# sinamalakouti/CDDMSL

Measured on AMD Instinct MI355X. Metric: images/sec (train step) VOC+Clipart RN50-C4, higher is better.
Workload: dtype bf16

## Files before the change

cddmsl_amd/csrc/elementwise.hip:

```cpp
#include "common.h"
#include <stdlib.h>

namespace {

template <typename T> struct Elt;
template <> struct Elt<__bf16> {
  static constexpr int ES = 2, VEC = 8;
  __device__ static __forceinline__ void unpack(const u32x4& v, float* f) {
#pragma unroll
    for (int j = 0; j < 4; ++j) { f[2 * j] = bf2f(v[j] & 0xffff); f[2 * j + 1] = bf2f(v[j] >> 16); }
  }
  __device__ static __forceinline__ u32x4 pack(const float* f) {
    u32x4 v;
#pragma unroll
    for (int j = 0; j < 4; ++j) v[j] = pack2bf(f[2 * j], f[2 * j + 1]);
    return v;
  }
  __device__ static __forceinline__ float ld(const char* p) { return bf2f(*(const unsigned short*)p); }
  __device__ static __forceinline__ void st(char* p, float v) { *(unsigned short*)p = f2bf(v); }
};
template <> struct Elt<float> {
  static constexpr int ES = 4, VEC = 4;
  __device__ static __forceinline__ void unpack(const u32x4& v, float* f) {
    const f32x4 x = __builtin_bit_cast(f32x4, v);
// ... 119 lines not shown
template <typename T>
__global__ void k_avgpool2_bwd(const char* dy, const char* mask, const char* add, char* dx, int N, int H, int W, int cch) {
  int Ho = H / 2, Wo = W / 2;
  long total = (long)N * H * W * cch;
  for (long i = (long)blockIdx.x * blockDim.x + threadIdx.x; i < total; i += (long)gridDim.x * blockDim.x) {
    int c = i % cch; long q = i / cch;
    int xx = q % W; q /= W;
    int yy = q % H; int n = q / H;
    float g[8], m[8], a[8], o[8];
    bool in = (yy >> 1) < Ho && (xx >> 1) < Wo;
    if (in) Elt<T>::unpack(((const u32x4*)dy)[(((long)n * Ho + (yy >> 1)) * Wo + (xx >> 1)) * cch + c], g);
    if (mask) Elt<T>::unpack(((const u32x4*)mask)[i], m);
    if (add) Elt<T>::unpack(((const u32x4*)add)[i], a);
#pragma unroll
    for (int j = 0; j < Elt<T>::VEC; ++j) {
      float v = in ? g[j] * 0.25f : 0.f;
      if (add) v += a[j];
      if (mask && !(m[j] > 0.f)) v = 0.f;
      o[j] = v;
    }
    ((u32x4*)dx)[i] = Elt<T>::pack(o);
  }
}

__global__ __launch_bounds__(256) void k_avgpool2_bwd_q8(const char* dy, const char* mask, const char* add, char* dx, int N, int H, int W, int cch,
                                                         char* y8, const float* q8, unsigned* amax8) {
  using T = __bf16;
  const int Ho = H / 2, Wo = W / 2;
  const long total = (long)N * H * W * cch;
  const float s = q8[0];
  unsigned mx = 0u;
  for (long i = (long)blockIdx.x * blockDim.x + threadIdx.x; i < total; i += (long)gridDim.x * blockDim.x) {
    int c = i % cch; long q = i / cch;
    int xx = q % W; q /= W;
    int yy = q % H; int n = q / H;
    float g[8], m[8], a[8], o[8];
    bool in = (yy >> 1) < Ho && (xx >> 1) < Wo;
    if (in) Elt<T>::unpack(((const u32x4*)dy)[(((long)n * Ho + (yy >> 1)) * Wo + (xx >> 1)) * cch + c], g);
    if (mask) Elt<T>::unpack(((const u32x4*)mask)[i], m);
    if (add) Elt<T>::unpack(((const u32x4*)add)[i], a);
#pragma unroll
    for (int j = 0; j < 8; ++j) {
      float v = in ? g[j] * 0.25f : 0.f;
      if (add) v += a[j];
      if (mask && !(m[j] > 0.f)) v = 0.f;
      o[j] = v;
      mx = absmax_bits(mx, v);
    }
    ((u32x4*)dx)[i] = Elt<T>::pack(o);
    const u32x2 o8 = {e4m3x4(o[0] * s, o[1] * s, o[2] * s, o[3] * s), e4m3x4(o[4] * s, o[5] * s, o[6] * s, o[7] * s)};
    ((u32x2*)y8)[i] = o8;
  }
  __shared__ unsigned sm[4];
  mx = wave_max_u(mx);
  if ((threadIdx.x & 63) == 0) sm[threadIdx.x >> 6] = mx;
  __syncthreads();
  if (threadIdx.x == 0) {
    const unsigned a = sm[0] > sm[1] ? sm[0] : sm[1], b = sm[2] > sm[3] ? sm[2] : sm[3];
    atomicMax(amax8 + (blockIdx.x & 63), a > b ? a : b);
  }
}

template <typename T>
__global__ void k_maxpool3s2(const char* x, char* y, int N, int H, int W, int Ho, int Wo, int cch) {
  long total = (long)N * Ho * Wo * cch;
  for (long i = (long)blockIdx.x * blockDim.x + threadIdx.x; i < total; i += (long)gridDim.x * blockDim.x) {
    int c = i % cch; long q = i / cch;
    int ox = q % Wo; q /= Wo;
    int oy = q % Ho; int n = q / Ho;
    float m[8], v[8];
#pragma unroll
    for (int j = 0; j < 8; ++j) m[j] = -INFINITY;
    for (int dy = 0; dy < 3; ++dy) {
      int iy = 2 * oy - 1 + dy;
      if (iy < 0 || iy >= H) continue;
      for (int dx = 0; dx < 3; ++dx) {
        int ix = 2 * ox - 1 + dx;
        if (ix < 0 || ix >= W) continue;
        Elt<T>::unpack(((const u32x4*)x)[(((long)n * H + iy) * W + ix) * cch + c], v);
#pragma unroll
        for (int j = 0; j < Elt<T>::VEC; ++j) m[j] = fmaxf(m[j], v[j]);
      }
    }
    ((u32x4*)y)[i] = Elt<T>::pack(m);
  }
}
template <typename T>
__global__ void k_upsample_zero2(const char* t, const char* mask, const char* add, char* dx, int N, int H, int W, int Ho, int Wo, int cch) {
  long total = (long)N * H * W * cch;
  for (long i = (long)blockIdx.x * blockDim.x + threadIdx.x; i < total; i += (long)gridDim.x * blockDim.x) {
    int c = i % cch; long q = i / cch;
    int xx = q % W; q /= W;
    int yy = q % H; int n = q / H;
    float g[8], m[8], a[8], o[8];
    bool in = !(yy & 1) && !(xx & 1) && (yy >> 1) < Ho && (xx >> 1) < Wo;
    if (in) Elt<T>::unpack(((const u32x4*)t)[(((long)n * Ho + (yy >> 1)) * Wo + (xx >> 1)) * cch + c], g);
    if (mask) Elt<T>::unpack(((const u32x4*)mask)[i], m);
    if (add) Elt<T>::unpack(((const u32x4*)add)[i], a);
#pragma unroll
    for (int j = 0; j < Elt<T>::VEC; ++j) {
      float v = in ? g[j] : 0.f;
      if (add) v += a[j];
      if (mask && !(m[j] > 0.f)) v = 0.f;
      o[j] = v;
    }
    ((u32x4*)dx)[i] = Elt<T>::pack(o);
  }
}
template <typename T>
__global__ void k_meanpool_fwd(const char* x, float* y, long K, int P, int C) {
  long i = (long)blockIdx.x * blockDim.x + threadIdx.x;
  if (i >= K * C) return;
  long k = i / C; int c = i % C;
  float s = 0.f;
  for (int p = 0; p < P; ++p) s += Elt<T>::ld(x + ((k * P + p) * C + c) * Elt<T>::ES);
  y[i] = s / (float)P;
}
template <typename T>
__global__ void k_meanpool_bwd(const float* dy, char* dx, long K, int P, int C) {
  long i = (long)blockIdx.x * blockDim.x + threadIdx.x;
  if (i >= K * P * C) return;
  int c = i % C; long k = i / ((long)P * C);
  Elt<T>::st(dx + i * Elt<T>::ES, dy[k * C + c] / (float)P);
}

template <typename T>
__global__ void k_attn_tokens_fwd(const char* x, const float* pos, char* tok, unsigned long long* mbits, int K, int P, int TP, int cch) {
  long total = (long)K * cch;
  for (long i = (long)blockIdx.x * blockDim.x + threadIdx.x; i < total; i += (long)gridDim.x * blockDim.x) {
    int c = i % cch; long k = i / cch;
    float s[8] = {0, 0, 0, 0, 0, 0, 0, 0}, v[8], o[8];
    unsigned long long mb[8] = {0, 0, 0, 0, 0, 0, 0, 0};
    const int VEC = Elt<T>::VEC;
    for (int p = 0; p < P; ++p) {
      Elt<T>::unpack(((const u32x4*)x)[(k * P + p) * cch + c], v);
      const float* pe = pos + (long)(p + 1) * cch * VEC + c * VEC;
#pragma unroll
      for (int j = 0; j < VEC; ++j) { s[j] += v[j]; o[j] = v[j] + pe[j]; mb[j] |= (unsigned long long)(v[j] > 0.f) << p; }
      ((u32x4*)tok)[(k * TP + p + 1) * cch + c] = Elt<T>::pack(o);
    }
    if (mbits) {
#pragma unroll
      for (int j = 0; j < VEC; ++j) mbits[(k * cch + c) * VEC + j] = mb[j];
    }
    const float* pe = pos + c * VEC;
#pragma unroll
    for (int j = 0; j < VEC; ++j) o[j] = s[j] / (float)P + pe[j];
    ((u32x4*)tok)[(k * TP) * cch + c] = Elt<T>::pack(o);
    const u32x4 z = {0u, 0u, 0u, 0u};
    for (int p = P + 1; p < TP; ++p) ((u32x4*)tok)[(k * TP + p) * cch + c] = z;
  }
}
template <typename T>
__global__ __launch_bounds__(256) void k_attn_tokens_bwd(const char* __restrict__ dtok, const char* __restrict__ relu_mask, char* __restrict__ dx, float* __restrict__ gpos, int K,
                                                         int P, int TP, int cch, int slab) {
  constexpr int V = Elt<T>::VEC;
  const int c = blockIdx.x * 256 + threadIdx.x;
  const int t = blockIdx.y;
  if (c >= cch || (t == 0 && !gpos)) return;
  const int k0 = blockIdx.z * slab, k1 = min(K, k0 + slab);
  float acc[V];
#pragma unroll
  for (int j = 0; j < V; ++j) acc[j] = 0.f;
  const u32x4* src = (const u32x4*)dtok;
#pragma unroll 4
  for (int k = k0; k < k1; ++k) {
    float a[8];
    Elt<T>::unpack(src[((long)k * TP + t) * cch + c], a);
#pragma unroll
    for (int j = 0; j < V; ++j) acc[j] += a[j];
    if (t > 0 && dx) {
      float b[8], m[8], o[8];
      const long oi = ((long)k * P + t - 1) * cch + c;
      Elt<T>::unpack(src[(long)k * TP * cch + c], b);
      if (relu_mask) Elt<T>::unpack(((const u32x4*)relu_mask)[oi], m);
#pragma unroll
      for (int j = 0; j < V; ++j) {
        o[j] = a[j] + b[j] / (float)P;
        if (relu_mask && !(m[j] > 0.f)) o[j] = 0.f;
      }
      ((u32x4*)dx)[oi] = Elt<T>::pack(o);
    }
  }
  if (gpos) {
#pragma unroll
    for (int j = 0; j < V; ++j) atomicAdd(gpos + (long)t * cch * V + (long)c * V + j, acc[j]);
  }
}

template <typename T>
__global__ void k_attnpool_softmax_fwd(const float* S, float* p, char* pT, long rows, int H, int P1, int TP, float scale) {
  const long r = (long)blockIdx.x * blockDim.x + threadIdx.x;
  if (r >= rows) return;
  const long k = r / H; const int h = (int)(r - k * H);
  const float* s = S + r * TP;
  float mx = -INFINITY;
  for (int t = 0; t < P1; ++t) mx = fmaxf(mx, s[t] * scale);
  float sum = 0.f;
  for (int t = 0; t < P1; ++t) sum += expf(s[t] * scale - mx);
  const float inv = 1.f / sum;
  for (int t = 0; t < TP; ++t) {
    float v = 0.f;
    if (t < P1) { v = expf(s[t] * scale - mx) * inv; p[r * P1 + t] = v; }
    Elt<T>::st(pT + ((k * TP + t) * H + h) * Elt<T>::ES, v);
  }
}
template <typename T>
__global__ void k_attnpool_softmax_bwd(const float* p, const float* dP, char* dsT, char* pds, long rows, int H, int P1, int TP,
                                       float scale) {
  const long r = (long)blockIdx.x * blockDim.x + threadIdx.x;
  if (r >= rows) return;
  const long k = r / H; const int h = (int)(r - k * H);
  const float* pr = p + r * P1;
  const float* dp = dP + r * TP;
  float dot = 0.f;
  for (int t = 0; t < P1; ++t) dot += pr[t] * dp[t];
  char* prow = pds + ((k * 2 * H + h) * TP) * Elt<T>::ES;
  char* drow = pds + ((k * 2 * H + H + h) * TP) * Elt<T>::ES;
  for (int t = 0; t < TP; ++t) {
    float pv = 0.f, ds = 0.f;
    if (t < P1) { pv = pr[t]; ds = pv * (dp[t] - dot) * scale; }
    Elt<T>::st(dsT + ((k * TP + t) * H + h) * Elt<T>::ES, ds);
    Elt<T>::st(prow + t * Elt<T>::ES, pv);
    Elt<T>::st(drow + t * Elt<T>::ES, ds);
  }
}

template <typename T>
__global__ __launch_bounds__(256) void k_attnpool_softmax_fwd_w(const float* __restrict__ S, float* __restrict__ p, char* __restrict__ pT,
                                                                long K, int H, int P1, int TP, float scale) {
  const long k = (long)blockIdx.x * 4 + (threadIdx.x >> 6);
  const int t = threadIdx.x & 63;
  if (k >= K) return;
  float v[32];
#pragma unroll
  for (int h = 0; h < 32; ++h) {
    v[h] = 0.f;
    if (h < H) {
      const bool in = t < P1;
      const float x = in ? S[(k * H + h) * TP + t] * scale : -INFINITY;
      const float mx = wave_max(x);
      const float e = in ? expf(x - mx) : 0.f;
      const float sum = wave_sum(e);
      v[h] = e * (1.f / sum);
      if (in) p[(k * H + h) * P1 + t] = v[h];
    }
  }
  if (t < TP) {
    char* dst = pT + ((k * TP + t) * H) * Elt<T>::ES;
    if (H % Elt<T>::VEC == 0) {
#pragma unroll
      for (int g = 0; g < 32 / Elt<T>::VEC; ++g)
        if (g * Elt<T>::VEC < H) ((u32x4*)dst)[g] = Elt<T>::pack(v + g * Elt<T>::VEC);
    } else {
#pragma unroll
      for (int h = 0; h < 32; ++h)
        if (h < H) Elt<T>::st(dst + h * Elt<T>::ES, v[h]);
    }
  }
}
template <typename T>
__global__ __launch_bounds__(256) void k_attnpool_softmax_bwd_w(const float* __restrict__ p, const float* __restrict__ dP,
                                                                char* __restrict__ dsT, char* __restrict__ pds, long K, int H, int P1,
                                                                int TP, float scale) {
  const long k = (long)blockIdx.x * 4 + (threadIdx.x >> 6);
  const int t = threadIdx.x & 63;
  if (k >= K) return;
  float dsv[32];
#pragma unroll
  for (int h = 0; h < 32; ++h) {
    dsv[h] = 0.f;
    if (h < H) {
      const bool in = t < P1;
      const float pv = in ? p[(k * H + h) * P1 + t] : 0.f;
      const float dp = in ? dP[(k * H + h) * TP + t] : 0.f;
      const float dot = wave_sum(pv * dp);
      dsv[h] = in ? pv * (dp - dot) * scale : 0.f;
      if (t < TP) {
        Elt<T>::st(pds + ((k * 2 * H + h) * TP + t) * Elt<T>::ES, pv);
        Elt<T>::st(pds + ((k * 2 * H + H + h) * TP + t) * Elt<T>::ES, dsv[h]);
      }
    }
  }
  if (t < TP) {
    char* dst = dsT + ((k * TP + t) * H) * Elt<T>::ES;
    if (H % Elt<T>::VEC == 0) {
#pragma unroll
      for (int g = 0; g < 32 / Elt<T>::VEC; ++g)
        if (g * Elt<T>::VEC < H) ((u32x4*)dst)[g] = Elt<T>::pack(dsv + g * Elt<T>::VEC);
    } else {
#pragma unroll
      for (int h = 0; h < 32; ++h)
        if (h < H) Elt<T>::st(dst + h * Elt<T>::ES, dsv[h]);
    }
  }
}

template <typename T>
__global__ void k_relu_bwd(const char* g, const char* y, char* dx, long nchunks, int g_f32) {
  for (long i = (long)blockIdx.x * blockDim.x + threadIdx.x; i < nchunks; i += (long)gridDim.x * blockDim.x) {
    float a[8], m[8], o[8];
    Elt<T>::unpack(((const u32x4*)y)[i], m);
    if (g_f32 && Elt<T>::VEC == 8) {
      Elt<float>::unpack(((const u32x4*)g)[2 * i], a);
      Elt<float>::unpack(((const u32x4*)g)[2 * i + 1], a + 4);
    } else Elt<T>::unpack(((const u32x4*)g)[i], a);
// ... 114 lines not shown
  return (unsigned)(g < 1 ? 1 : (g > cap ? cap : g));
}

}

#define DISPATCH(dtype, KERNEL, ...)                                   \
  do {                                                                 \
    if ((dtype) == 0) { KERNEL<__bf16> __VA_ARGS__; }                  \
    else if ((dtype) == 1) { KERNEL<float> __VA_ARGS__; }              \
    else return CDDMSL_ERR_ARG;                                        \
  } while (0)

extern "C" int cddmsl_preprocess(const unsigned char* img, void* out, int n, int h, int w, int Hp, int Wp, int Cp,
                                 const float* mean3, const float* std3, int div255, int dtype, void* stream) {
  if (h <= 0 || w <= 0 || h > Hp || w > Wp || Cp < 3) return CDDMSL_ERR_ARG;
  hipStream_t st = (hipStream_t)stream;
  long px = (long)Hp * Wp;
  DISPATCH(dtype, k_preprocess, <<<dim3((unsigned)((px + 255) / 256)), dim3(256), 0, st>>>(
      img, (char*)out, n, h, w, Hp, Wp, Cp, mean3[0], mean3[1], mean3[2], std3[0], std3[1], std3[2], div255 ? 255.0f : 1.0f));
  return launch_status();
}

extern "C" int cddmsl_preprocess224(const unsigned char* img, void* out, int n, int h, int w, int Hp, int Wp, int RH,
                                    int RW, int top, int left, int S, int Cp, const float* mean3, const float* std3,
                                    int dtype, void* stream) {
  if (h <= 0 || w <= 0 || h > Hp || w > Wp || Cp < 3 || S <= 0 || top < 0 || left < 0 || top + S > RH || left + S > RW)
    return CDDMSL_ERR_ARG;
  hipStream_t st = (hipStream_t)stream;
  DISPATCH(dtype, k_preprocess224, <<<dim3((unsigned)((S * S + 255) / 256)), dim3(256), 0, st>>>(
      img, (char*)out, n, h, w, Hp, Wp, RH, RW, top, left, S, Cp, mean3[0], mean3[1], mean3[2], std3[0], std3[1], std3[2]));
  return launch_status();
}

extern "C" int cddmsl_preprocess_batch(const unsigned char* const* imgs, const int* hs, const int* ws, int N, void* out, int Hp, int Wp,
                                       int Cp, const float* mean3, const float* std3, int div255, int dtype, void* stream) {
  if (N < 0 || Cp < 3 || !imgs || !hs || !ws) return CDDMSL_ERR_ARG;
  for (int j = 0; j < N; ++j) if (hs[j] <= 0 || ws[j] <= 0 || hs[j] > Hp || ws[j] > Wp || !imgs[j]) return CDDMSL_ERR_ARG;
  hipStream_t st = (hipStream_t)stream;
  const long px = (long)Hp * Wp;
  for (int n0 = 0; n0 < N; n0 += PRE_MAX) {
    const int c = N - n0 < PRE_MAX ? N - n0 : PRE_MAX;
    PreBatch b;
    for (int j = 0; j < PRE_MAX; ++j) { const int q = j < c ? j : 0; b.img[j] = imgs[n0 + q]; b.h[j] = hs[n0 + q]; b.w[j] = ws[n0 + q]; }
    DISPATCH(dtype, k_preprocess_batch, <<<dim3((unsigned)((px + 255) / 256), (unsigned)c), dim3(256), 0, st>>>(
        b, (char*)out, n0, Hp, Wp, Cp, mean3[0], mean3[1], mean3[2], std3[0], std3[1], std3[2], div255 ? 255.0f : 1.0f));
  }
  return launch_status();
}
extern "C" int cddmsl_preprocess224_batch(const unsigned char* const* imgs, const int* hs, const int* ws, int N, void* out, int Hp, int Wp,
                                          int RH, int RW, int top, int left, int S, int Cp, const float* mean3, const float* std3,
                                          int dtype, void* stream) {
  if (N < 0 || Cp < 3 || !imgs || !hs || !ws || S <= 0 || top < 0 || left < 0 || top + S > RH || left + S > RW) return CDDMSL_ERR_ARG;
  for (int j = 0; j < N; ++j) if (hs[j] <= 0 || ws[j] <= 0 || hs[j] > Hp || ws[j] > Wp || !imgs[j]) return CDDMSL_ERR_ARG;
  hipStream_t st = (hipStream_t)stream;
  for (int n0 = 0; n0 < N; n0 += PRE_MAX) {
    const int c = N - n0 < PRE_MAX ? N - n0 : PRE_MAX;
    PreBatch b;
    for (int j = 0; j < PRE_MAX; ++j) { const int q = j < c ? j : 0; b.img[j] = imgs[n0 + q]; b.h[j] = hs[n0 + q]; b.w[j] = ws[n0 + q]; }
    DISPATCH(dtype, k_preprocess224_batch, <<<dim3((unsigned)((S * S + 255) / 256), (unsigned)c), dim3(256), 0, st>>>(
        b, (char*)out, n0, Hp, Wp, RH, RW, top, left, S, Cp, mean3[0], mean3[1], mean3[2], std3[0], std3[1], std3[2]));
  }
  return launch_status();
}

extern "C" int cddmsl_avgpool2_fwd(const void* x, void* y, int N, int H, int W, int C, int dtype, void* stream) {
  int es = dtype == 0 ? 2 : 4;
  if ((C * es) % 16 || H < 2 || W < 2) return CDDMSL_ERR_ARG;
  int cch = C * es / 16;
  long total = (long)N * (H / 2) * (W / 2) * cch;
  if (total == 0) return CDDMSL_OK;
  DISPATCH(dtype, k_avgpool2_fwd, <<<dim3(gsz(total)), dim3(256), 0, (hipStream_t)stream>>>((const char*)x, (char*)y, N, H, W, cch));
  return launch_status();
}

extern "C" int cddmsl_avgpool2_bwd(const void* dy, const void* mask, const void* add, void* dx, int N, int H, int W,
                                   int C, int dtype, void* stream) {
  int es = dtype == 0 ? 2 : 4;
  if ((C * es) % 16 || H < 2 || W < 2) return CDDMSL_ERR_ARG;
  int cch = C * es / 16;
  long total = (long)N * H * W * cch;
  if (total == 0) return CDDMSL_OK;
  DISPATCH(dtype, k_avgpool2_bwd, <<<dim3(gsz(total)), dim3(256), 0, (hipStream_t)stream>>>(
      (const char*)dy, (const char*)mask, (const char*)add, (char*)dx, N, H, W, cch));
  return launch_status();
}

extern "C" int cddmsl_avgpool2_bwd_q8(const void* dy, const void* mask, const void* add, void* dx, int N, int H, int W, int C, void* y8,
                                      const float* q8, float* amax8, void* stream) {
  if ((C * 2) % 16 || !y8 || !q8 || !amax8) return CDDMSL_ERR_ARG;
  const int cch = C * 2 / 16;
  const long total = (long)N * H * W * cch;
  if (total == 0) return CDDMSL_OK;
  hipLaunchKernelGGL(k_avgpool2_bwd_q8, dim3(gsz(total, 256, 8192)), dim3(256), 0, (hipStream_t)stream, (const char*)dy, (const char*)mask, (const char*)add,
                     (char*)dx, N, H, W, cch, (char*)y8, q8, (unsigned*)amax8);
  return launch_status();
}

extern "C" int cddmsl_maxpool3s2_fwd(const void* x, void* y, int N, int H, int W, int C, int dtype, void* stream) {
  int es = dtype == 0 ? 2 : 4;
  if ((C * es) % 16 || H < 1 || W < 1) return CDDMSL_ERR_ARG;
  int cch = C * es / 16, Ho = (H - 1) / 2 + 1, Wo = (W - 1) / 2 + 1;
  long total = (long)N * Ho * Wo * cch;
  if (total == 0) return CDDMSL_OK;
  DISPATCH(dtype, k_maxpool3s2, <<<dim3(gsz(total)), dim3(256), 0, (hipStream_t)stream>>>((const char*)x, (char*)y, N, H, W, Ho, Wo, cch));
  return launch_status();
}
extern "C" int cddmsl_upsample_zero2(const void* t, const void* mask, const void* add, void* dx, int N, int H, int W, int C,
                                     int dtype, void* stream) {
  int es = dtype == 0 ? 2 : 4;
  if ((C * es) % 16 || H < 1 || W < 1) return CDDMSL_ERR_ARG;
  int cch = C * es / 16, Ho = (H - 1) / 2 + 1, Wo = (W - 1) / 2 + 1;
  long total = (long)N * H * W * cch;
  if (total == 0) return CDDMSL_OK;
  DISPATCH(dtype, k_upsample_zero2, <<<dim3(gsz(total)), dim3(256), 0, (hipStream_t)stream>>>(
      (const char*)t, (const char*)mask, (const char*)add, (char*)dx, N, H, W, Ho, Wo, cch));
  return launch_status();
}
extern "C" int cddmsl_meanpool_fwd(const void* x, float* y, long K, int P, int C, int dtype, void* stream) {
  if (K < 0 || P <= 0 || C <= 0) return CDDMSL_ERR_ARG;
  if (K == 0) return CDDMSL_OK;
  long n = K * C;
  DISPATCH(dtype, k_meanpool_fwd, <<<dim3((unsigned)((n + 255) / 256)), dim3(256), 0, (hipStream_t)stream>>>((const char*)x, y, K, P, C));
  return launch_status();
}
extern "C" int cddmsl_meanpool_bwd(const float* dy, void* dx, long K, int P, int C, int dtype, void* stream) {
  if (K < 0 || P <= 0 || C <= 0) return CDDMSL_ERR_ARG;
  if (K == 0) return CDDMSL_OK;
  long n = K * P * C;
  DISPATCH(dtype, k_meanpool_bwd, <<<dim3((unsigned)((n + 255) / 256)), dim3(256), 0, (hipStream_t)stream>>>(dy, (char*)dx, K, P, C));
  return launch_status();
}

extern "C" int cddmsl_attn_tokens_fwd(const void* x, const float* pos, void* tok, int K, int P, int TP, int C, int dtype, void* stream) {
  int es = dtype == 0 ? 2 : 4;
  if ((C * es) % 16 || P <= 0 || TP < P + 1) return CDDMSL_ERR_ARG;
  int cch = C * es / 16;
  long total = (long)K * cch;
  if (total == 0) return CDDMSL_OK;
  DISPATCH(dtype, k_attn_tokens_fwd, <<<dim3(gsz(total, 64)), dim3(64), 0, (hipStream_t)stream>>>((const char*)x, pos, (char*)tok, nullptr, K, P, TP, cch));
  return launch_status();
}

extern "C" int cddmsl_attn_tokens_fwd_mask(const void* x, const float* pos, void* tok, unsigned long long* mbits, int K, int P, int TP, int C,
                                           int dtype, void* stream) {
  int es = dtype == 0 ? 2 : 4;
  if ((C * es) % 16 || P <= 0 || P > 64 || TP < P + 1 || K < 0 || !mbits) return CDDMSL_ERR_ARG;
  int cch = C * es / 16;
  long total = (long)K * cch;
  if (total == 0) return CDDMSL_OK;
  DISPATCH(dtype, k_attn_tokens_fwd, <<<dim3(gsz(total, 64)), dim3(64), 0, (hipStream_t)stream>>>((const char*)x, pos, (char*)tok, mbits, K, P, TP, cch));
  return launch_status();
}

extern "C" int cddmsl_attn_tokens_bwd(const void* dtok, const void* relu_mask, void* dx, float* gpos, int K, int P, int TP, int C,
                                      int dtype, void* stream) {
  int es = dtype == 0 ? 2 : 4;
  if ((C * es) % 16 || P <= 0 || TP < P + 1 || K < 0 || (!dx && !gpos)) return CDDMSL_ERR_ARG;
  int cch = C * es / 16;
  if (K == 0) return CDDMSL_OK;
  int slab = 128;
  while ((K + slab - 1) / slab > 65535) slab *= 2;
  dim3 grid((unsigned)((cch + 255) / 256), (unsigned)(P + 1), (unsigned)((K + slab - 1) / slab));
  DISPATCH(dtype, k_attn_tokens_bwd, <<<grid, dim3(256), 0, (hipStream_t)stream>>>((const char*)dtok, (const char*)relu_mask, (char*)dx, gpos, K, P, TP, cch, slab));
  return launch_status();
}

extern "C" int cddmsl_attnpool_softmax_fwd(const float* S, float* p, void* pT, long K, int H, int P1, int TP, float scale, int dtype,
                                           void* stream) {
  if (K < 0 || H <= 0 || P1 <= 0 || TP < P1) return CDDMSL_ERR_ARG;
  const long rows = K * H;
  if (rows == 0) return CDDMSL_OK;
  if (H <= 32 && TP <= 64) {
    DISPATCH(dtype, k_attnpool_softmax_fwd_w, <<<dim3((unsigned)((K + 3) / 4)), dim3(256), 0, (hipStream_t)stream>>>(S, p, (char*)pT, K, H, P1, TP, scale));
    return launch_status();
  }
  DISPATCH(dtype, k_attnpool_softmax_fwd, <<<dim3((unsigned)((rows + 255) / 256)), dim3(256), 0, (hipStream_t)stream>>>(S, p, (char*)pT, rows, H, P1, TP, scale));
  return launch_status();
}
extern "C" int cddmsl_attnpool_softmax_bwd(const float* p, const float* dP, void* dsT, void* pds, long K, int H, int P1, int TP,
                                           float scale, int dtype, void* stream) {
  if (K < 0 || H <= 0 || P1 <= 0 || TP < P1) return CDDMSL_ERR_ARG;
  const long rows = K * H;
  if (rows == 0) return CDDMSL_OK;
  if (H <= 32 && TP <= 64) {
    DISPATCH(dtype, k_attnpool_softmax_bwd_w, <<<dim3((unsigned)((K + 3) / 4)), dim3(256), 0, (hipStream_t)stream>>>(p, dP, (char*)dsT, (char*)pds, K, H, P1, TP, scale));
    return launch_status();
  }
  DISPATCH(dtype, k_attnpool_softmax_bwd, <<<dim3((unsigned)((rows + 255) / 256)), dim3(256), 0, (hipStream_t)stream>>>(p, dP, (char*)dsT, (char*)pds, rows, H, P1, TP, scale));
  return launch_status();
}

extern "C" int cddmsl_relu_bwd(const void* g, const void* y, void* dx, long numel, int g_f32, int dtype, void* stream) {
  int vec = dtype == 0 ? 8 : 4;
  if (numel < 0 || numel % vec) return CDDMSL_ERR_ARG;
  if (numel == 0) return CDDMSL_OK;
  long nch = numel / vec;
  DISPATCH(dtype, k_relu_bwd, <<<dim3(gsz(nch)), dim3(256), 0, (hipStream_t)stream>>>((const char*)g, (const char*)y, (char*)dx, nch, g_f32));
  return launch_status();
}

extern "C" int cddmsl_colsum(const void* x, float* out, long rows, int cols, int period, int dtype, void* stream) {
  if (rows < 0 || cols <= 0 || period <= 0) return CDDMSL_ERR_ARG;
  if (rows == 0) return CDDMSL_OK;
  if (period > 65535) return CDDMSL_ERR_ARG;
  long nj = (rows + period - 1) / period;
  int slab = 256;
  while ((nj + slab - 1) / slab > 2048) slab *= 2;
  const int vec = dtype == 0 ? 8 : 4;
  if (cols % vec == 0) {
    dim3 gridv((unsigned)((cols / vec + 63) / 64), (unsigned)((nj + slab - 1) / slab), (unsigned)period);
    DISPATCH(dtype, k_colsum_vec, <<<gridv, dim3(256), 0, (hipStream_t)stream>>>((const char*)x, out, rows, cols, period, slab));
    return launch_status();
  }
  dim3 grid((unsigned)((cols + 63) / 64), (unsigned)((nj + slab - 1) / slab), (unsigned)period);
  DISPATCH(dtype, k_colsum, <<<grid, dim3(256), 0, (hipStream_t)stream>>>((const char*)x, out, rows, cols, period, slab));
  return launch_status();
}

extern "C" int cddmsl_sgd_clip_step(float** params, const float** grads, float** moms, const long* sizes, int count,
                                    float* norm_ws, float lr, float momentum, float wd, float clip, int first_step,
                                    void* stream) {
  hipStream_t st = (hipStream_t)stream;
  if (count < 0) return CDDMSL_ERR_ARG;
  for (int base = 0; base < count; base += SGD_MAX) {
    SgdBatch b;
    b.count = count - base < SGD_MAX ? count - base : SGD_MAX;
    long mx = 0;
    for (int i = 0; i < b.count; ++i) {
      b.it[i].p = params[base + i]; b.it[i].g = grads[base + i]; b.it[i].m = moms[base + i]; b.it[i].n = sizes[base + i];
      if (sizes[base + i] > mx) mx = sizes[base + i];
    }
    if (hipMemsetAsync(norm_ws + base, 0, sizeof(float) * b.count, st) != hipSuccess) return CDDMSL_ERR_LAUNCH;
    unsigned gx = gsz(mx, 256 * 8, 256);
    k_sqnorm<<<dim3(gx, b.count), dim3(256), 0, st>>>(b, norm_ws + base);
    k_sgd<<<dim3(gx, b.count), dim3(256), 0, st>>>(b, norm_ws + base, lr, momentum, wd, clip, first_step);
  }
  return launch_status();
}

extern "C" int cddmsl_abi_version() { return 3; }
```

cddmsl_amd/csrc/gemm_conv.hip:

```cpp
#include "common.h"
#include <cstdlib>
#include <type_traits>

namespace {

constexpr int BM = 128, BN = 128, KCH = 8;

struct FastDiv {
  unsigned mul, shr, d;
};
static inline FastDiv make_fastdiv(unsigned d) {
  FastDiv f;
  f.d = d;
  unsigned s = 0;
  while ((1ull << s) < d) ++s;
  f.shr = s;
  f.mul = (unsigned)(((1ull << 32) * ((1ull << s) - d)) / d + 1);
  return f;
}
__device__ __forceinline__ unsigned fdiv(unsigned n, const FastDiv& f) { return (__umulhi(n, f.mul) + n) >> f.shr; }

template <typename T> __device__ __forceinline__ float affine(float v, float sc, float bi) {
  return sizeof(T) <= 2 ? __builtin_fmaf(v, sc, bi) : v * sc + bi;
}

__device__ __forceinline__ unsigned pack4_e4m3(float a, float b, float c, float d) {
  a = __builtin_amdgcn_fmed3f(a, -448.f, 448.f); b = __builtin_amdgcn_fmed3f(b, -448.f, 448.f);
  c = __builtin_amdgcn_fmed3f(c, -448.f, 448.f); d = __builtin_amdgcn_fmed3f(d, -448.f, 448.f);
  int w = __builtin_amdgcn_cvt_pk_fp8_f32(a, b, 0, false);
  w = __builtin_amdgcn_cvt_pk_fp8_f32(c, d, w, true);
  return (unsigned)w;
}

#ifndef CDDMSL_STORE_AUX
#define CDDMSL_STORE_AUX 2
#endif
#ifndef CDDMSL_LOAD_AUX
#define CDDMSL_LOAD_AUX 0
#endif

struct ConvArgs {
  const char* x;
  const char* w;
  char* y;
  const float* scale;
  const float* bias;
  const char* residual;
  const char* relu_mask;
  int Nimg, Hi, Wi, Cin, Ho, Wo, Cout, KH, KW, stride, pad;
  int ldy, ldr, ldm;
  int relu, out_f32, pool;
  int res_f32;
  int res_pool;
  int M, Kc, cpp;
  FastDiv dWo, dHo, dcpp, dKW;
  int xrs, wrs;
  long bx, bw, by;
  char* y8 = nullptr;
  const float* q8 = nullptr;
  unsigned* amax8 = nullptr;
  float* partial = nullptr;
  int tile0 = 0, ksplits = 1, kper = 0, tile_limit = 0;
  int nt_out = 1;
#ifdef CDDMSL_STAMPS
  unsigned long long* stamps;
#endif
#ifdef CDDMSL_TILE_STAMPS
  unsigned long long* tstamps = nullptr;
#endif
};

template <typename T> struct Mma;
template <> struct Mma<__bf16> {
  static constexpr int ES = 2;
  __device__ static __forceinline__ void step(f32x16& acc, const u32x4& a, const u32x4& b) {
    acc = __builtin_amdgcn_mfma_f32_32x32x16_bf16(__builtin_bit_cast(bf16x8, a), __builtin_bit_cast(bf16x8, b), acc, 0, 0, 0);
  }
  __device__ static __forceinline__ float load(const char* p) { return bf2f(*(const unsigned short*)p); }
  __device__ static __forceinline__ void store(char* p, float v) { *(unsigned short*)p = f2bf(v); }
};
template <> struct Mma<float> {
  static constexpr int ES = 4;
  __device__ static __forceinline__ void step(f32x16& acc, const u32x4& a, const u32x4& b) {
    const f32x4 fa = __builtin_bit_cast(f32x4, a), fb = __builtin_bit_cast(f32x4, b);
    acc = __builtin_amdgcn_mfma_f32_32x32x2f32(fa[0], fb[0], acc, 0, 0, 0);
    acc = __builtin_amdgcn_mfma_f32_32x32x2f32(fa[1], fb[1], acc, 0, 0, 0);
    acc = __builtin_amdgcn_mfma_f32_32x32x2f32(fa[2], fb[2], acc, 0, 0, 0);
    acc = __builtin_amdgcn_mfma_f32_32x32x2f32(fa[3], fb[3], acc, 0, 0, 0);
  }
  __device__ static __forceinline__ float load(const char* p) { return *(const float*)p; }
  __device__ static __forceinline__ void store(char* p, float v) { *(float*)p = v; }
};

struct fp8e4 { unsigned char v; };
typedef __attribute__((ext_vector_type(8))) int i32x8;
template <> struct Mma<fp8e4> {
  static constexpr int ES = 2;
  __device__ static __forceinline__ void step2(f32x16& acc, const u32x4& a0, const u32x4& a1, const u32x4& b0, const u32x4& b1) {
    const i32x8 a = {(int)a0[0], (int)a0[1], (int)a0[2], (int)a0[3], (int)a1[0], (int)a1[1], (int)a1[2], (int)a1[3]};
    const i32x8 b = {(int)b0[0], (int)b0[1], (int)b0[2], (int)b0[3], (int)b1[0], (int)b1[1], (int)b1[2], (int)b1[3]};
    acc = __builtin_amdgcn_mfma_scale_f32_32x32x64_f8f6f4(a, b, acc, 0, 0, 0, 0x7f7f7f7f, 0, 0x7f7f7f7f);
  }
};
template <typename T> struct MmaQuad {
  __device__ static __forceinline__ void run(f32x16& c0, f32x16& c1, const u32x4 (*fa)[4], const u32x4* fb) {
#pragma unroll
    for (int ks = 0; ks < 4; ++ks) {
      Mma<T>::step(c0, fa[0][ks], fb[ks]);
      Mma<T>::step(c1, fa[1][ks], fb[ks]);
    }
  }
};
template <> struct MmaQuad<fp8e4> {
  __device__ static __forceinline__ void run(f32x16& c0, f32x16& c1, const u32x4 (*fa)[4], const u32x4* fb) {
#pragma unroll
    for (int s = 0; s < 2; ++s) {
      Mma<fp8e4>::step2(c0, fa[0][2 * s], fa[0][2 * s + 1], fb[2 * s], fb[2 * s + 1]);
      Mma<fp8e4>::step2(c1, fa[1][2 * s], fa[1][2 * s + 1], fb[2 * s], fb[2 * s + 1]);
    }
  }
};

template <typename T> __device__ __forceinline__ void load8(const char* p, float* f);
template <> __device__ __forceinline__ void load8<__bf16>(const char* p, float* f) {
  const u32x4 v = *(const u32x4*)p;
#pragma unroll
  for (int j = 0; j < 4; ++j) { f[2 * j] = bf2f(v[j] & 0xffff); f[2 * j + 1] = bf2f(v[j] >> 16); }
}
template <> __device__ __forceinline__ void load8<float>(const char* p, float* f) {
  const f32x4 a = ((const f32x4*)p)[0], b = ((const f32x4*)p)[1];
  f[0] = a[0]; f[1] = a[1]; f[2] = a[2]; f[3] = a[3]; f[4] = b[0]; f[5] = b[1]; f[6] = b[2]; f[7] = b[3];
}

__device__ __forceinline__ int xcd_remap(int bid, int nblk) {
  const int q = nblk >> 3, rem = nblk & 7, x = bid & 7, j = bid >> 3;
  return (x < rem ? x * (q + 1) : rem * (q + 1) + (x - rem) * q) + j;
}

__device__ __forceinline__ int swz(int row, int chunk) { return row * KCH + (chunk ^ ((row >> 1) & 7)); }

template <typename T> __device__ __forceinline__ u32x4 avg4(const u32x4& a, const u32x4& b, const u32x4& c, const u32x4& d);
template <> __device__ __forceinline__ u32x4 avg4<float>(const u32x4& a, const u32x4& b, const u32x4& c, const u32x4& d) {
  const f32x4 fa = __builtin_bit_cast(f32x4, a), fb = __builtin_bit_cast(f32x4, b);
  const f32x4 fc = __builtin_bit_cast(f32x4, c), fd = __builtin_bit_cast(f32x4, d);
  f32x4 r = ((fa + fb) + (fc + fd)) * 0.25f;
  return __builtin_bit_cast(u32x4, r);
}
template <> __device__ __forceinline__ u32x4 avg4<__bf16>(const u32x4& a, const u32x4& b, const u32x4& c, const u32x4& d) {
  u32x4 r;
#pragma unroll
  for (int j = 0; j < 4; ++j) {
    float lo = (bf2f(a[j] & 0xffff) + bf2f(b[j] & 0xffff)) + (bf2f(c[j] & 0xffff) + bf2f(d[j] & 0xffff));
    float hi = (bf2f(a[j] >> 16) + bf2f(b[j] >> 16)) + (bf2f(c[j] >> 16) + bf2f(d[j] >> 16));
    r[j] = pack2bf(lo * 0.25f, hi * 0.25f);
  }
  return r;
}

template <typename T>
__global__ __launch_bounds__(256, 2) void k_conv_fwd_reg(ConvArgs p) {
  __shared__ __attribute__((aligned(16))) u32x4 lds[2][BM * KCH];
  const int t = threadIdx.x;
  const int ntn = (p.Cout + BN - 1) / BN;
  const int tile_n = blockIdx.x % ntn, tile_m = blockIdx.x / ntn;
  const int m0 = tile_m * BM, n0 = tile_n * BN;
  const int cc = t & 7, rb = t >> 3;

  long pix[4];
  int iy0[4], ix0[4];
  bool vm[4];
#pragma unroll
  for (int i = 0; i < 4; ++i) {
    int m = m0 + rb + 32 * i;
    vm[i] = m < p.M;
    int mm = vm[i] ? m : 0;
    int ox = mm % p.Wo, tq = mm / p.Wo;
    int oy = tq % p.Ho, img = tq / p.Ho;
    int s = p.pool ? 2 * p.stride : p.stride;
    iy0[i] = oy * s - p.pad;
    ix0[i] = ox * s - p.pad;
    pix[i] = ((long)img * p.Hi + iy0[i]) * p.Wi + ix0[i];
  }
  const int nkt = (p.Kc + KCH - 1) / KCH;
  u32x4 ra[4], rbv[4];
  const u32x4 zero = {0u, 0u, 0u, 0u};

  auto gload = [&](int kt) {
    int kc = kt * KCH + cc;
    bool vk = kc < p.Kc;
    int pp = vk ? kc / p.cpp : 0;
    int coff = vk ? kc - pp * p.cpp : 0;
    int ky = pp / p.KW, kx = pp - ky * p.KW;
#pragma unroll
    for (int i = 0; i < 4; ++i) {
      int iy = iy0[i] + ky, ix = ix0[i] + kx;
      if (!p.pool) {
        bool ok = vk && vm[i] && iy >= 0 && iy < p.Hi && ix >= 0 && ix < p.Wi;
        const u32x4* src = (const u32x4*)(p.x + ((pix[i] + (long)ky * p.Wi + kx) * p.cpp + coff) * 16);
        ra[i] = ok ? *src : zero;
      } else {
        bool ok = vk && vm[i];
        if (ok) {
          const char* b0 = p.x + (pix[i] * p.cpp + coff) * 16;
          long rs = (long)p.Wi * p.cpp * 16, cs = (long)p.cpp * 16;
          ra[i] = avg4<T>(*(const u32x4*)b0, *(const u32x4*)(b0 + cs), *(const u32x4*)(b0 + rs), *(const u32x4*)(b0 + rs + cs));
        } else ra[i] = zero;
      }
      int n = n0 + rb + 32 * i;
      bool okb = vk && n < p.Cout;
      rbv[i] = okb ? *(const u32x4*)(p.w + ((long)n * p.Kc + kc) * 16) : zero;
    }
  };

  f32x16 acc[2][2];
#pragma unroll
  for (int a = 0; a < 2; ++a)
#pragma unroll
    for (int b = 0; b < 2; ++b)
#pragma unroll
      for (int r = 0; r < 16; ++r) acc[a][b][r] = 0.f;

  const int lane = t & 63, wv = t >> 6;
  const int wm = wv >> 1, wn = wv & 1;
  const int r = lane & 31, h = lane >> 5;

  gload(0);
  for (int kt = 0; kt < nkt; ++kt) {
#pragma unroll
    for (int i = 0; i < 4; ++i) {
      int row = rb + 32 * i;
      lds[0][swz(row, cc)] = ra[i];
      lds[1][swz(row, cc)] = rbv[i];
    }
    __syncthreads();
    if (kt + 1 < nkt) gload(kt + 1);
#pragma unroll
    for (int ks = 0; ks < KCH / 2; ++ks) {
      u32x4 fa[2], fb[2];
#pragma unroll
      for (int i = 0; i < 2; ++i) {
        fa[i] = lds[0][swz(wm * 64 + i * 32 + r, 2 * ks + h)];
        fb[i] = lds[1][swz(wn * 64 + i * 32 + r, 2 * ks + h)];
      }
#pragma unroll
      for (int a = 0; a < 2; ++a)
#pragma unroll
        for (int b = 0; b < 2; ++b) Mma<T>::step(acc[a][b], fa[a], fb[b]);
    }
    __syncthreads();
  }

  const bool vec_ok = (p.Cout % 8 == 0) && (p.ldy % 8 == 0) && (!p.residual || p.ldr % 8 == 0) && (!p.relu_mask || p.ldm % 8 == 0);
  if (vec_ok) {
    float* ep = (float*)&lds[0][0] + wv * 2048;
    const int cg = lane & 7, rr = lane >> 3;
    const int n = n0 + wn * 64 + cg * 8;
    float sc[8], bi[8];
#pragma unroll
    for (int j = 0; j < 8; ++j) {
      sc[j] = (p.scale && n + j < p.Cout) ? p.scale[n + j] : 1.f;
      bi[j] = (p.bias && n + j < p.Cout) ? p.bias[n + j] : 0.f;
    }
#pragma unroll
    for (int a = 0; a < 2; ++a) {
      __syncthreads();
#pragma unroll
      for (int b = 0; b < 2; ++b)
#pragma unroll
        for (int g = 0; g < 16; ++g) {
          int row = (g & 3) + 8 * (g >> 2) + 4 * h, col = b * 32 + r;
          ep[row * 64 + ((((col >> 3) ^ (row & 7)) << 3) | (col & 7))] = acc[a][b][g];
        }
      __syncthreads();
      if (n < p.Cout) {
#pragma unroll
        for (int i = 0; i < 4; ++i) {
          int row = rr + 8 * i;
          int m = m0 + wm * 64 + a * 32 + row;
          if (m >= p.M) continue;
          const f32x4* src = (const f32x4*)(ep + row * 64 + ((cg ^ (row & 7)) << 3));
          f32x4 v0 = src[0], v1 = src[1];
          float v[8] = {v0[0], v0[1], v0[2], v0[3], v1[0], v1[1], v1[2], v1[3]};
#pragma unroll
          for (int j = 0; j < 8; ++j) v[j] = affine<T>(v[j], sc[j], bi[j]);
          if (p.residual) {
            float rv[8];
            load8<T>(p.residual + ((long)m * p.ldr + n) * Mma<T>::ES, rv);
#pragma unroll
            for (int j = 0; j < 8; ++j) v[j] += rv[j];
          }
          if (p.relu) {
#pragma unroll
            for (int j = 0; j < 8; ++j) v[j] = fmaxf(v[j], 0.f);
          }
          if (p.relu_mask) {
            float mv[8];
            load8<T>(p.relu_mask + ((long)m * p.ldm + n) * Mma<T>::ES, mv);
#pragma unroll
            for (int j = 0; j < 8; ++j) if (!(mv[j] > 0.f)) v[j] = 0.f;
          }
          if (p.out_f32 || Mma<T>::ES == 4) {
            f32x4* dst = (f32x4*)(p.y + ((long)m * p.ldy + n) * 4);
            f32x4 o0 = {v[0], v[1], v[2], v[3]}, o1 = {v[4], v[5], v[6], v[7]};
            dst[0] = o0; dst[1] = o1;
          } else {
            u32x4 o = {pack2bf(v[0], v[1]), pack2bf(v[2], v[3]), pack2bf(v[4], v[5]), pack2bf(v[6], v[7])};
            *(u32x4*)(p.y + ((long)m * p.ldy + n) * 2) = o;
          }
        }
      }
    }
    return;
  }
#pragma unroll
  for (int b = 0; b < 2; ++b) {
    int n = n0 + wn * 64 + b * 32 + r;
    if (n >= p.Cout) continue;
    float sc = p.scale ? p.scale[n] : 1.f;
    float bi = p.bias ? p.bias[n] : 0.f;
#pragma unroll
    for (int a = 0; a < 2; ++a) {
#pragma unroll
      for (int g = 0; g < 16; ++g) {
        int m = m0 + wm * 64 + a * 32 + (g & 3) + 8 * (g >> 2) + 4 * h;
        if (m >= p.M) continue;
        float v = affine<T>(acc[a][b][g], sc, bi);
        if (p.residual) v += Mma<T>::load(p.residual + ((long)m * p.ldr + n) * Mma<T>::ES);
        if (p.relu) v = fmaxf(v, 0.f);
        if (p.relu_mask && !(Mma<T>::load(p.relu_mask + ((long)m * p.ldm + n) * Mma<T>::ES) > 0.f)) v = 0.f;
        if (p.out_f32) *(float*)(p.y + ((long)m * p.ldy + n) * 4) = v;
        else Mma<T>::store(p.y + ((long)m * p.ldy + n) * Mma<T>::ES, v);
      }
    }
  }
}

__device__ __attribute__((aligned(16))) unsigned int g_zero_page[4] = {0u, 0u, 0u, 0u};

__device__ __forceinline__ void glds16(const void* g, void* l) {
  __builtin_amdgcn_global_load_lds((const __attribute__((address_space(1))) void*)g,
                                   (__attribute__((address_space(3))) void*)l, 16, 0, 0);
}

__device__ __forceinline__ long pooled_row(const ConvArgs& p, int m) {
  const unsigned tq = fdiv((unsigned)m, p.dWo), ox = m - tq * p.Wo;
  const unsigned img = fdiv(tq, p.dHo), oy = tq - img * p.Ho;
  const unsigned hp = p.Ho >> 1, wp = p.Wo >> 1;
  return ((oy >> 1) < hp && (ox >> 1) < wp) ? ((long)img * hp + (oy >> 1)) * wp + (ox >> 1) : -1L;
}

template <typename T>
__global__ __launch_bounds__(256, 2) void k_conv_fwd(ConvArgs p) {
  __shared__ __attribute__((aligned(16))) u32x4 lds[2][2][BM * KCH];
  const int t = threadIdx.x;
  p.x += (long)blockIdx.y * p.bx; p.w += (long)blockIdx.y * p.bw; p.y += (long)blockIdx.y * p.by;
  const int wvu = __builtin_amdgcn_readfirstlane(t >> 6);
  const int ntn = (p.Cout + BN - 1) / BN;
  const int lbid = xcd_remap(blockIdx.x, gridDim.x);
  const int tile_n = lbid % ntn, tile_m = lbid / ntn;
  const int m0 = tile_m * BM, n0 = tile_n * BN;
  const int cc = t & 7, rb = t >> 3;
  const int cl = cc ^ ((rb >> 1) & 7);

  long rowoff[4], wrow[4];
  int iy0[4], ix0[4];
  bool vm[4], vn[4];
#pragma unroll
  for (int i = 0; i < 4; ++i) {
    int m = m0 + rb + 32 * i;
    vm[i] = m < p.M;
    unsigned mm = vm[i] ? m : 0;
    unsigned tq = fdiv(mm, p.dWo), ox = mm - tq * p.Wo;
    unsigned img = fdiv(tq, p.dHo), oy = tq - img * p.Ho;
    iy0[i] = (int)oy * p.stride - p.pad;
    ix0[i] = (int)ox * p.stride - p.pad;
    rowoff[i] = ((((long)img * p.Hi + iy0[i]) * p.Wi + ix0[i]) * p.xrs) * 16;
    int n = n0 + rb + 32 * i;
    vn[i] = n < p.Cout;
    wrow[i] = (long)(vn[i] ? n : 0) * p.wrs * 16;
  }
  const int nkt = (p.Kc + KCH - 1) / KCH;
  const char* zp = (const char*)g_zero_page;
  const bool taps = !(p.KH == 1 && p.KW == 1 && p.pad == 0);
  int kc = cl;
  int pp0 = (int)fdiv((unsigned)kc, p.dcpp);
  int coff = kc - pp0 * p.cpp;
  int ky = (int)fdiv((unsigned)pp0, p.dKW), kx = pp0 - ky * p.KW;

  const bool fast = (p.cpp & 7) == 0;
  const char* pa[4];
  const char* pb[4];
  int inca[4], incb[4];
  int tiles_left_in_tap = 0;
  auto retap = [&]() {
    const int delta = ((ky * p.Wi + kx) * p.xrs + coff) * 16;
#pragma unroll
    for (int i = 0; i < 4; ++i) {
      bool ok = vm[i];
      if (taps) {
        int iy = iy0[i] + ky, ix = ix0[i] + kx;
        ok = ok && iy >= 0 && iy < p.Hi && ix >= 0 && ix < p.Wi;
      }
      pa[i] = ok ? p.x + rowoff[i] + delta : zp;
      inca[i] = ok ? KCH * 16 : 0;
    }
  };
  if (fast) {
#pragma unroll
    for (int i = 0; i < 4; ++i) {
      pb[i] = vn[i] ? p.w + wrow[i] + (long)kc * 16 : zp;
      incb[i] = vn[i] ? KCH * 16 : 0;
    }
    retap();
    tiles_left_in_tap = p.cpp >> 3;
  }

  auto stage = [&](int buf) {
    if (fast) {
#pragma unroll
      for (int i = 0; i < 4; ++i) glds16(pa[i], &lds[buf][0][(8 * wvu + 32 * i) * KCH]);
#pragma unroll
      for (int i = 0; i < 4; ++i) glds16(pb[i], &lds[buf][1][(8 * wvu + 32 * i) * KCH]);
#pragma unroll
      for (int i = 0; i < 4; ++i) pb[i] += incb[i];
      if (--tiles_left_in_tap == 0) {
        tiles_left_in_tap = p.cpp >> 3;
        coff = cl;
        if (++kx == p.KW) { kx = 0; ++ky; }
        retap();
      } else {
#pragma unroll
        for (int i = 0; i < 4; ++i) pa[i] += inca[i];
      }
      return;
    }
    const bool vk = kc < p.Kc;
    const int delta = ((ky * p.Wi + kx) * p.xrs + coff) * 16;
#pragma unroll
    for (int i = 0; i < 4; ++i) {
      bool ok = vk && vm[i];
      if (taps) {
        int iy = iy0[i] + ky, ix = ix0[i] + kx;
        ok = ok && iy >= 0 && iy < p.Hi && ix >= 0 && ix < p.Wi;
      }
      const char* src = ok ? p.x + rowoff[i] + delta : zp;
      glds16(src, &lds[buf][0][(8 * wvu + 32 * i) * KCH]);
    }
#pragma unroll
    for (int i = 0; i < 4; ++i) {
      const char* src = (vk && vn[i]) ? p.w + wrow[i] + (long)kc * 16 : zp;
      glds16(src, &lds[buf][1][(8 * wvu + 32 * i) * KCH]);
    }
    kc += KCH;
    coff += KCH;
    while (coff >= p.cpp) {
      coff -= p.cpp;
      if (++kx == p.KW) { kx = 0; ++ky; }
    }
  };

  f32x16 acc[2][2];
#pragma unroll
  for (int a = 0; a < 2; ++a)
#pragma unroll
    for (int b = 0; b < 2; ++b)
#pragma unroll
      for (int r = 0; r < 16; ++r) acc[a][b][r] = 0.f;

  const int lane = t & 63, wv = t >> 6;
  const int wm = wv >> 1, wn = wv & 1;
  const int r = lane & 31, h = lane >> 5;

  const bool vec_ok = (p.Cout % 8 == 0) && (p.ldy % 8 == 0) && (!p.residual || p.ldr % 8 == 0) && (!p.relu_mask || p.ldm % 8 == 0);
  constexpr bool PRE = Mma<T>::ES == 2;
  u32x4 rres[2][4], rmsk[2][4];
  const bool rf32 = PRE && p.res_f32;
  if (PRE && vec_ok && ((p.residual && !rf32) || p.relu_mask)) {
    const int n = n0 + wn * 64 + (lane & 7) * 8;
#pragma unroll
    for (int a = 0; a < 2; ++a)
#pragma unroll
      for (int i = 0; i < 4; ++i) {
        int m = m0 + wm * 64 + a * 32 + (lane >> 3) + 8 * i;
        bool ok = m < p.M && n < p.Cout;
        const u32x4 z = {0u, 0u, 0u, 0u};
        if (p.res_pool) {
          const long po = pooled_row(p, m);
          rres[a][i] = (ok && po >= 0) ? *(const u32x4*)(p.residual + (po * p.ldr + n) * 2) : z;
        } else
        rres[a][i] = (ok && p.residual && !rf32) ? *(const u32x4*)(p.residual + ((long)m * p.ldr + n) * 2) : z;
        rmsk[a][i] = (ok && p.relu_mask) ? *(const u32x4*)(p.relu_mask + ((long)m * p.ldm + n) * 2) : z;
      }
  }

  stage(0);
  for (int kt = 0; kt < nkt; ++kt) {
    const int cur = kt & 1;
    if (kt + 1 < nkt) {
      stage(cur ^ 1);
      asm volatile("s_waitcnt vmcnt(8)" ::: "memory");
    } else {
      asm volatile("s_waitcnt vmcnt(0)" ::: "memory");
    }
    __builtin_amdgcn_s_barrier();
    u32x4 fa[2][2], fb[2][2];
#pragma unroll
    for (int i = 0; i < 2; ++i) {
      fa[0][i] = lds[cur][0][swz(wm * 64 + i * 32 + r, h)];
      fb[0][i] = lds[cur][1][swz(wn * 64 + i * 32 + r, h)];
    }
#pragma unroll
    for (int ks = 0; ks < KCH / 2; ++ks) {
      if (ks + 1 < KCH / 2) {
#pragma unroll
        for (int i = 0; i < 2; ++i) {
          fa[(ks + 1) & 1][i] = lds[cur][0][swz(wm * 64 + i * 32 + r, 2 * (ks + 1) + h)];
          fb[(ks + 1) & 1][i] = lds[cur][1][swz(wn * 64 + i * 32 + r, 2 * (ks + 1) + h)];
        }
      }
#pragma unroll
      for (int a = 0; a < 2; ++a)
#pragma unroll
        for (int b = 0; b < 2; ++b) Mma<T>::step(acc[a][b], fa[ks & 1][a], fb[ks & 1][b]);
    }
    asm volatile("s_waitcnt lgkmcnt(0)" ::: "memory");
    __builtin_amdgcn_s_barrier();
  }

  if (vec_ok) {
    float* ep = (float*)&lds[0][0][0] + wv * 2048;
    const int cg = lane & 7, rr = lane >> 3;
    const int n = n0 + wn * 64 + cg * 8;
    float sc[8], bi[8];
#pragma unroll
    for (int j = 0; j < 8; ++j) {
      sc[j] = (p.scale && n + j < p.Cout) ? p.scale[n + j] : 1.f;
      bi[j] = (p.bias && n + j < p.Cout) ? p.bias[n + j] : 0.f;
    }
#pragma unroll
    for (int a = 0; a < 2; ++a) {
      __syncthreads();
#pragma unroll
      for (int b = 0; b < 2; ++b)
#pragma unroll
        for (int g = 0; g < 16; ++g) {
          int row = (g & 3) + 8 * (g >> 2) + 4 * h, col = b * 32 + r;
          ep[row * 64 + ((((col >> 3) ^ (row & 7)) << 3) | (col & 7))] = acc[a][b][g];
        }
      __syncthreads();
      if (n < p.Cout) {
#pragma unroll
        for (int i = 0; i < 4; ++i) {
          int row = rr + 8 * i;
          int m = m0 + wm * 64 + a * 32 + row;
          if (m >= p.M) continue;
          const f32x4* src = (const f32x4*)(ep + row * 64 + ((cg ^ (row & 7)) << 3));
          f32x4 v0 = src[0], v1 = src[1];
          float v[8] = {v0[0], v0[1], v0[2], v0[3], v1[0], v1[1], v1[2], v1[3]};
#pragma unroll
          for (int j = 0; j < 8; ++j) v[j] = affine<T>(v[j], sc[j], bi[j]);
          if (p.residual) {
            float rv[8];
            if (rf32) load8<float>(p.residual + ((long)m * p.ldr + n) * 4, rv);
            else if (PRE) {
#pragma unroll
              for (int j = 0; j < 4; ++j) { rv[2 * j] = bf2f(rres[a][i][j] & 0xffff); rv[2 * j + 1] = bf2f(rres[a][i][j] >> 16); }
            } else if (p.res_pool) {
              const long po = pooled_row(p, m);
#pragma unroll
              for (int j = 0; j < 8; ++j) rv[j] = 0.f;
              if (po >= 0) load8<T>(p.residual + (po * p.ldr + n) * Mma<T>::ES, rv);
            } else load8<T>(p.residual + ((long)m * p.ldr + n) * Mma<T>::ES, rv);
            if (p.res_pool) {
#pragma unroll
              for (int j = 0; j < 8; ++j) rv[j] *= 0.25f;
            }
#pragma unroll
            for (int j = 0; j < 8; ++j) v[j] += rv[j];
          }
          if (p.relu) {
#pragma unroll
            for (int j = 0; j < 8; ++j) v[j] = fmaxf(v[j], 0.f);
          }
          if (p.relu_mask) {
            float mv[8];
            if (PRE) {
#pragma unroll
              for (int j = 0; j < 4; ++j) { mv[2 * j] = bf2f(rmsk[a][i][j] & 0xffff); mv[2 * j + 1] = bf2f(rmsk[a][i][j] >> 16); }
            } else load8<T>(p.relu_mask + ((long)m * p.ldm + n) * Mma<T>::ES, mv);
#pragma unroll
            for (int j = 0; j < 8; ++j) if (!(mv[j] > 0.f)) v[j] = 0.f;
          }
          if (p.out_f32 || Mma<T>::ES == 4) {
            f32x4* dst = (f32x4*)(p.y + ((long)m * p.ldy + n) * 4);
            f32x4 o0 = {v[0], v[1], v[2], v[3]}, o1 = {v[4], v[5], v[6], v[7]};
            dst[0] = o0; dst[1] = o1;
          } else {
            u32x4 o = {pack2bf(v[0], v[1]), pack2bf(v[2], v[3]), pack2bf(v[4], v[5]), pack2bf(v[6], v[7])};
            *(u32x4*)(p.y + ((long)m * p.ldy + n) * 2) = o;
          }
        }
      }
    }
    return;
  }
#pragma unroll
  for (int b = 0; b < 2; ++b) {
    int n = n0 + wn * 64 + b * 32 + r;
    if (n >= p.Cout) continue;
    float sc = p.scale ? p.scale[n] : 1.f;
    float bi = p.bias ? p.bias[n] : 0.f;
#pragma unroll
    for (int a = 0; a < 2; ++a) {
#pragma unroll
      for (int g = 0; g < 16; ++g) {
        int m = m0 + wm * 64 + a * 32 + (g & 3) + 8 * (g >> 2) + 4 * h;
        if (m >= p.M) continue;
        float v = affine<T>(acc[a][b][g], sc, bi);
        if (p.residual) v += Mma<T>::load(p.residual + ((long)m * p.ldr + n) * Mma<T>::ES);
        if (p.relu) v = fmaxf(v, 0.f);
        if (p.relu_mask && !(Mma<T>::load(p.relu_mask + ((long)m * p.ldm + n) * Mma<T>::ES) > 0.f)) v = 0.f;
        if (p.out_f32) *(float*)(p.y + ((long)m * p.ldy + n) * 4) = v;
        else Mma<T>::store(p.y + ((long)m * p.ldy + n) * Mma<T>::ES, v);
      }
    }
  }
}

struct WgradArgs {
  const char* x;
  const char* dy;
  float* dw;
  const float* scale;
  int Nimg, Hi, Wi, Cin, Ho, Wo, Cout, KH, KW, stride, pad, ldd, pool;
  int M, Kc, cpp, K, ncc;
  int mtiles_per_split;
  FastDiv dWo, dHo;
  int xrs;
  int ldo;
  int direct;
  long bx, bd, bo;
  const float* g0 = nullptr;
  const unsigned long long* mbits = nullptr;
  float* gpos = nullptr;
  float* ws = nullptr;
#ifdef CDDMSL_TILE_STAMPS
  unsigned long long* tstamps = nullptr;
#endif
};

constexpr int WM = 64;
constexpr int WROW = 16 + 4;

template <typename T> struct TrFrag;
template <> struct TrFrag<__bf16> {
  __device__ static __forceinline__ u32x4 read(const u32x4* base, int mrow0, int col0, int lane) {
    int g = lane >> 4, li = lane & 15, q = li >> 2, pp = li & 3;
    int hh = g >> 1;
    int col = col0 + 16 * (g & 1) + 4 * pp;
    const char* b = (const char*)base;
    const char* a0 = b + (long)(mrow0 + 8 * hh + q) * (WROW * 16) + col * 2;
    const char* a1 = a0 + 4 * (WROW * 16);
    i16x4 v0 = __builtin_amdgcn_ds_read_tr16_b64_v4i16((__attribute__((address_space(3))) i16x4*)a0);
    i16x4 v1 = __builtin_amdgcn_ds_read_tr16_b64_v4i16((__attribute__((address_space(3))) i16x4*)a1);
    u32x2 p0 = __builtin_bit_cast(u32x2, v0), p1 = __builtin_bit_cast(u32x2, v1);
    u32x4 r = {p0[0], p0[1], p1[0], p1[1]};
    return r;
  }
  static constexpr int MSTEP = 16;
};
template <> struct TrFrag<float> {
  __device__ static __forceinline__ u32x4 read(const u32x4* base, int mrow0, int col0, int lane) {
    int r = lane & 31, hh = lane >> 5;
    const char* b = (const char*)base;
    u32x4 v;
#pragma unroll
    for (int j = 0; j < 4; ++j) v[j] = *(const unsigned int*)(b + (long)(mrow0 + 4 * hh + j) * (WROW * 16) + (col0 + r) * 4);
    return v;
  }
  static constexpr int MSTEP = 8;
};

template <typename T>
__global__ __launch_bounds__(256, 2) void k_conv_wgrad(WgradArgs p) {
  constexpr int ES = Mma<T>::ES;
  constexpr int TC = 128 * ES / 16;
  constexpr int COLS = 256 / ES;
  __shared__ __attribute__((aligned(16))) u32x4 lds[2][WM * WROW];
  const int t = threadIdx.x, lane = t & 63, wv = t >> 6;
  const int ntn = (p.Cout + COLS - 1) / COLS, ntk = (p.K + COLS - 1) / COLS;
  int bid = xcd_remap(blockIdx.x, gridDim.x);
  const int tile_k = bid % ntk; bid /= ntk;
  const int tile_n = bid % ntn; bid /= ntn;
  const int split = bid;
  const int n0 = tile_n * COLS, k0 = tile_k * COLS;
  const int mt0 = split * p.mtiles_per_split;
  const int total_mt = (p.M + WM - 1) / WM;
  const int mt1 = min(mt0 + p.mtiles_per_split, total_mt);
  (void)TC;

  const int cc = t & 15, rb = t >> 4;
  const int kc = k0 * ES / 16 + cc;
  const bool vk = kc < p.Kc;
  const int pp = vk ? kc / p.cpp : 0, coff = vk ? kc - pp * p.cpp : 0;
  const int ky = pp / p.KW, kx = pp - ky * p.KW;
  const int nc = n0 * ES / 16 + cc;
  const bool vn = nc < p.ncc;
  const u32x4 zero = {0u, 0u, 0u, 0u};
  u32x4 rx[4], rd[4];

  auto gload = [&](int mt) {
#pragma unroll
    for (int i = 0; i < 4; ++i) {
      int m = mt * WM + rb + 16 * i;
      bool vmm = m < p.M;
      unsigned mm = vmm ? m : 0;
      unsigned tq = fdiv(mm, p.dWo);
      int ox = (int)(mm - tq * p.Wo);
      unsigned img = fdiv(tq, p.dHo);
      int oy = (int)(tq - img * p.Ho);
      if (!p.pool) {
        int iy = oy * p.stride - p.pad + ky, ix = ox * p.stride - p.pad + kx;
        bool ok = vmm && vk && iy >= 0 && iy < p.Hi && ix >= 0 && ix < p.Wi;
        rx[i] = ok ? *(const u32x4*)(p.x + ((((long)img * p.Hi + iy) * p.Wi + ix) * p.cpp + coff) * 16) : zero;
      } else {
        if (vmm && vk) {
          const char* b0 = p.x + ((((long)img * p.Hi + 2 * oy) * p.Wi + 2 * ox) * p.cpp + coff) * 16;
          long rs = (long)p.Wi * p.cpp * 16, cs = (long)p.cpp * 16;
          rx[i] = avg4<T>(*(const u32x4*)b0, *(const u32x4*)(b0 + cs), *(const u32x4*)(b0 + rs), *(const u32x4*)(b0 + rs + cs));
        } else rx[i] = zero;
      }
      rd[i] = (vmm && vn) ? *(const u32x4*)(p.dy + ((long)m * p.ldd) * ES + (long)nc * 16) : zero;
    }
  };

  constexpr int WT = COLS / 2;
  constexpr int NT = WT / 32;
  const int wn = wv >> 1, wk = wv & 1;
  f32x16 acc[NT][NT];
#pragma unroll
  for (int a = 0; a < NT; ++a)
#pragma unroll
    for (int b = 0; b < NT; ++b)
#pragma unroll
      for (int r = 0; r < 16; ++r) acc[a][b][r] = 0.f;

  if (mt0 < mt1) gload(mt0);
  for (int mt = mt0; mt < mt1; ++mt) {
#pragma unroll
    for (int i = 0; i < 4; ++i) {
      int row = rb + 16 * i;
      lds[0][row * WROW + cc] = rd[i];
      lds[1][row * WROW + cc] = rx[i];
    }
    __syncthreads();
    if (mt + 1 < mt1) gload(mt + 1);
#pragma unroll
    for (int ms = 0; ms < WM; ms += TrFrag<T>::MSTEP) {
      u32x4 fa[NT], fb[NT];
#pragma unroll
      for (int i = 0; i < NT; ++i) {
        fa[i] = TrFrag<T>::read(lds[0], ms, wn * WT + i * 32, lane);
        fb[i] = TrFrag<T>::read(lds[1], ms, wk * WT + i * 32, lane);
      }
#pragma unroll
      for (int a = 0; a < NT; ++a)
#pragma unroll
        for (int b = 0; b < NT; ++b) Mma<T>::step(acc[a][b], fa[a], fb[b]);
    }
    __syncthreads();
  }

  const int r = lane & 31, h = lane >> 5;
#pragma unroll
  for (int a = 0; a < NT; ++a)
#pragma unroll
    for (int b = 0; b < NT; ++b) {
      int k = k0 + wk * WT + b * 32 + r;
      if (k >= p.K) continue;
#pragma unroll
      for (int g = 0; g < 16; ++g) {
        int n = n0 + wn * WT + a * 32 + (g & 3) + 8 * (g >> 2) + 4 * h;
        if (n >= p.Cout) continue;
        float v = acc[a][b][g] * (p.scale ? p.scale[n] : 1.f);
        atomicAdd(p.dw + (long)n * p.K + k, v);
      }
    }
}

__device__ __forceinline__ int fsw(int row) { return ((row & 3) << 2) | ((row >> 2) & 3); }

template <typename T> struct TrFragS;
template <> struct TrFragS<__bf16> {
  struct Off { int o0, o1; };
  __device__ static __forceinline__ Off prep(int col0, int lane) {
    int g = lane >> 4, li = lane & 15, q = li >> 2, pp = li & 3;
    int hh = g >> 1;
// ... 34 lines not shown
    for (int j = 0; j < 4; ++j) {
      int off = o.o[j] + ms * 256;
      int row = off >> 8, ch = (off >> 4) & 15;
      v[j] = *(const unsigned int*)(b + (off & ~0xf0) + 16 * (ch ^ fsw(row)));
    }
    return v;
  }
  static constexpr int MSTEP = 8;
};

template <typename T>
__global__ __launch_bounds__(256, 2) void k_conv_wgrad_dma(WgradArgs p) {
  constexpr int ES = Mma<T>::ES;
  constexpr int COLS = 256 / ES;
  __shared__ __attribute__((aligned(16))) u32x4 lds[2][2][WM * 16];
  const int t = threadIdx.x, lane = t & 63, wv = t >> 6;
  p.x += (long)blockIdx.y * p.bx; p.dy += (long)blockIdx.y * p.bd;
  char* outp = (char*)p.dw + (long)blockIdx.y * p.bo;
  const int wvu = __builtin_amdgcn_readfirstlane(t >> 6);
  const int ntn = (p.Cout + COLS - 1) / COLS, ntk = (p.K + COLS - 1) / COLS;
  int bid = xcd_remap(blockIdx.x, gridDim.x);
  const int tile_k = bid % ntk; bid /= ntk;
  const int tile_n = bid % ntn; bid /= ntn;
  const int split = bid;
  const int n0 = tile_n * COLS, k0 = tile_k * COLS;
  const int mt0 = split * p.mtiles_per_split;
  const int total_mt = (p.M + WM - 1) / WM;
  const int mt1 = min(mt0 + p.mtiles_per_split, total_mt);

  const int cc = t & 15, rb = t >> 4;
  const int cl = cc ^ fsw(rb);
  const int kc = k0 * ES / 16 + cl;
  const bool vk = kc < p.Kc;
  const int pp = vk ? kc / p.cpp : 0, coff = vk ? kc - pp * p.cpp : 0;
  const int ky = pp / p.KW, kx = pp - ky * p.KW;
  const int nc = n0 * ES / 16 + cl;
  const bool vn = nc < p.ncc;
  const bool taps = !(p.KH == 1 && p.KW == 1);
  const char* zp = (const char*)g_zero_page;

  int m[4];
  const char* pd[4];
  const char* px[4];
#pragma unroll
  for (int i = 0; i < 4; ++i) {
    m[i] = mt0 * WM + rb + 16 * i;
    pd[i] = p.dy + ((long)m[i] * p.ldd) * ES + (long)nc * 16;
    px[i] = p.x + (((long)m[i] + (long)(ky - p.pad) * p.Wi + (kx - p.pad)) * p.xrs) * 16 + (long)coff * 16;
  }
  const long dstep = (long)WM * p.ldd * ES, xstep = (long)WM * p.xrs * 16;

  auto stage = [&](int buf) {
#pragma unroll
    for (int i = 0; i < 4; ++i) {
      bool vmm = m[i] < p.M;
      glds16((vmm && vn) ? pd[i] : zp, &lds[buf][0][(4 * wvu + 16 * i) * 16]);
    }
#pragma unroll
    for (int i = 0; i < 4; ++i) {
      bool ok = (m[i] < p.M) & vk;
      if (taps) {
        unsigned mm = min((unsigned)m[i], (unsigned)(p.M - 1));
        unsigned tq = fdiv(mm, p.dWo);
        unsigned ox = mm - tq * p.Wo;
        unsigned oy = tq - fdiv(tq, p.dHo) * p.Ho;
        ok = ok & ((unsigned)((int)oy - p.pad + ky) < (unsigned)p.Hi) & ((unsigned)((int)ox - p.pad + kx) < (unsigned)p.Wi);
      }
      glds16(ok ? px[i] : zp, &lds[buf][1][(4 * wvu + 16 * i) * 16]);
    }
#pragma unroll
    for (int i = 0; i < 4; ++i) { m[i] += WM; pd[i] += dstep; px[i] += xstep; }
  };

  constexpr int WT = COLS / 2;
  constexpr int NT = WT / 32;
  const int wn = wv >> 1, wk = wv & 1;
  f32x16 acc[NT][NT];
#pragma unroll
  for (int a = 0; a < NT; ++a)
#pragma unroll
    for (int b = 0; b < NT; ++b)
#pragma unroll
      for (int r = 0; r < 16; ++r) acc[a][b][r] = 0.f;

  typename TrFragS<T>::Off offa[NT], offb[NT];
#pragma unroll
  for (int i = 0; i < NT; ++i) {
    offa[i] = TrFragS<T>::prep(wn * WT + i * 32, lane);
    offb[i] = TrFragS<T>::prep(wk * WT + i * 32, lane);
  }

  if (mt0 < mt1) stage(0);
  for (int mt = mt0; mt < mt1; ++mt) {
    const int cur = (mt - mt0) & 1;
    if (mt + 1 < mt1) {
      stage(cur ^ 1);
      asm volatile("s_waitcnt vmcnt(8)" ::: "memory");
    } else {
      asm volatile("s_waitcnt vmcnt(0)" ::: "memory");
    }
    __builtin_amdgcn_s_barrier();
#pragma unroll
    for (int ms = 0; ms < WM; ms += TrFragS<T>::MSTEP) {
      u32x4 fa[NT], fb[NT];
#pragma unroll
      for (int i = 0; i < NT; ++i) {
        fa[i] = TrFragS<T>::read(lds[cur][0], ms, offa[i]);
        fb[i] = TrFragS<T>::read(lds[cur][1], ms, offb[i]);
      }
      asm volatile("s_waitcnt lgkmcnt(0)" ::: "memory");
      __builtin_amdgcn_sched_barrier(0);
#pragma unroll
      for (int a = 0; a < NT; ++a)
#pragma unroll
        for (int b = 0; b < NT; ++b) Mma<T>::step(acc[a][b], fa[a], fb[b]);
    }
    asm volatile("s_waitcnt lgkmcnt(0)" ::: "memory");
    __builtin_amdgcn_s_barrier();
  }

  const int r = lane & 31, h = lane >> 5;
  if (p.ws) {
    f32x4* dst = (f32x4*)p.ws + ((long)(split * ntn + tile_n) * ntk + tile_k) * (4 * NT * NT * 4 * 64) + (wv * NT * NT * 4) * 64 + lane;
#pragma unroll
    for (int a = 0; a < NT; ++a)
#pragma unroll
      for (int b = 0; b < NT; ++b)
#pragma unroll
        for (int g4 = 0; g4 < 4; ++g4) {
          const f32x4 v = {acc[a][b][4 * g4], acc[a][b][4 * g4 + 1], acc[a][b][4 * g4 + 2], acc[a][b][4 * g4 + 3]};
          dst[((a * NT + b) * 4 + g4) * 64] = v;
        }
    return;
  }
#pragma unroll
  for (int a = 0; a < NT; ++a)
#pragma unroll
    for (int b = 0; b < NT; ++b) {
      int k = k0 + wk * WT + b * 32 + r;
      if (k >= p.K) continue;
#pragma unroll
      for (int g = 0; g < 16; ++g) {
        int n = n0 + wn * WT + a * 32 + (g & 3) + 8 * (g >> 2) + 4 * h;
        if (n >= p.Cout) continue;
        float v = acc[a][b][g] * (p.scale ? p.scale[n] : 1.f);
        long o = (long)n * p.ldo + k;
        if (p.direct == 0) atomicAdd((float*)outp + o, v);
        else if (p.direct == 1) ((float*)outp)[o] = v;
        else Mma<T>::store(outp + o * ES, v);
      }
    }
}

template <typename T>
__global__ __launch_bounds__(256, 2) void k_gemm_tn_stream(WgradArgs p, int nbatch, int bpb) {
  constexpr int ES = Mma<T>::ES;
  constexpr int COLS = 256 / ES;
  __shared__ __attribute__((aligned(16))) u32x4 lds[2][2][WM * 16];
  const int t = threadIdx.x, lane = t & 63, wv = t >> 6;
  const int wvu = __builtin_amdgcn_readfirstlane(t >> 6);
  const int ntk = (p.K + COLS - 1) / COLS;
  const int tile_k = blockIdx.x % ntk, tile_n = blockIdx.x / ntk;
  const int n0 = tile_n * COLS, k0 = tile_k * COLS;
  const int b0 = blockIdx.y * bpb, nb = min(bpb, nbatch - b0);
  const int nmt = (p.M + WM - 1) / WM;
  const int nit = nb * nmt;

  const int cc = t & 15, rb = t >> 4;
  const int cl = cc ^ fsw(rb);
  const int kc = k0 * ES / 16 + cl, nc = n0 * ES / 16 + cl;
  const bool vk = kc < p.Kc, vn = nc < p.ncc;
  const char* zp = (const char*)g_zero_page;
  int sb = 0, smt = 0;
  auto stage = [&](int buf) {
    const char* db = p.dy + (long)(b0 + sb) * p.bd + (long)nc * 16;
    const char* xb = p.x + (long)(b0 + sb) * p.bx + (long)kc * 16;
#pragma unroll
    for (int i = 0; i < 4; ++i) {
      const int m = smt * WM + rb + 16 * i;
      const bool vm = m < p.M;
      glds16((vm && vn) ? db + ((long)m * p.ldd) * ES : zp, &lds[buf][0][(4 * wvu + 16 * i) * 16]);
    }
#pragma unroll
    for (int i = 0; i < 4; ++i) {
      const int m = smt * WM + rb + 16 * i;
      const bool vm = m < p.M;
      glds16((vm && vk) ? xb + ((long)m * p.xrs) * 16 : zp, &lds[buf][1][(4 * wvu + 16 * i) * 16]);
    }
    if (++smt == nmt) { smt = 0; ++sb; }
  };

  constexpr int WT = COLS / 2;
  constexpr int NT = WT / 32;
  const int wn = wv >> 1, wk = wv & 1;
  f32x16 acc[NT][NT];
#pragma unroll
  for (int a = 0; a < NT; ++a)
#pragma unroll
    for (int b = 0; b < NT; ++b)
#pragma unroll
      for (int r = 0; r < 16; ++r) acc[a][b][r] = 0.f;
  typename TrFragS<T>::Off offa[NT], offb[NT];
#pragma unroll
  for (int i = 0; i < NT; ++i) {
    offa[i] = TrFragS<T>::prep(wn * WT + i * 32, lane);
    offb[i] = TrFragS<T>::prep(wk * WT + i * 32, lane);
  }
  const int r = lane & 31, h = lane >> 5;

  if (nit > 0) stage(0);
  int cb = 0, cmt = 0;
  for (int it = 0; it < nit; ++it) {
    const int cur = it & 1;
    if (it + 1 < nit) {
      stage(cur ^ 1);
      asm volatile("s_waitcnt vmcnt(8)" ::: "memory");
    } else {
      asm volatile("s_waitcnt vmcnt(0)" ::: "memory");
    }
    __builtin_amdgcn_s_barrier();
#pragma unroll
    for (int ms = 0; ms < WM; ms += TrFragS<T>::MSTEP) {
      u32x4 fa[NT], fb[NT];
#pragma unroll
      for (int i = 0; i < NT; ++i) {
        fa[i] = TrFragS<T>::read(lds[cur][0], ms, offa[i]);
        fb[i] = TrFragS<T>::read(lds[cur][1], ms, offb[i]);
      }
      asm volatile("s_waitcnt lgkmcnt(0)" ::: "memory");
      __builtin_amdgcn_sched_barrier(0);
#pragma unroll
      for (int a = 0; a < NT; ++a)
#pragma unroll
        for (int b = 0; b < NT; ++b) Mma<T>::step(acc[a][b], fa[a], fb[b]);
    }
    asm volatile("s_waitcnt lgkmcnt(0)" ::: "memory");
    __builtin_amdgcn_s_barrier();
    if (++cmt == nmt) {
      char* outp = (char*)p.dw + (long)(b0 + cb) * p.bo;
#pragma unroll
      for (int a = 0; a < NT; ++a)
#pragma unroll
        for (int b = 0; b < NT; ++b) {
          const int k = k0 + wk * WT + b * 32 + r;
#pragma unroll
          for (int g = 0; g < 16; ++g) {
            const int n = n0 + wn * WT + a * 32 + (g & 3) + 8 * (g >> 2) + 4 * h;
            if (k < p.K && n < p.Cout) {
              const float v = acc[a][b][g];
              const long o = (long)n * p.ldo + k;
              if (p.direct == 0) atomicAdd((float*)outp + o, v);
              else if (p.direct == 1) ((float*)outp)[o] = v;
              else Mma<T>::store(outp + o * ES, v);
            }
            acc[a][b][g] = 0.f;
          }
        }
      cmt = 0; ++cb;
    }
  }
}

template <int N>
__device__ __forceinline__ void wait_vm() { asm volatile("s_waitcnt vmcnt(%0)" :: "n"(N) : "memory"); }

template <int NG, int P>
constexpr int tn_small_stores3() {
  int n = 0;
  for (int a = 0; a < (NG + 3) / 4; ++a)
    for (int g = 0; g < 16; ++g) {
      if (a * 4 + (g >> 2) >= NG) continue;
      const int n0 = a * 32 + (g & 3) + 8 * (g >> 2);
      if ((n0 >= 1 && n0 <= P) || (n0 + 4 >= 1 && n0 + 4 <= P)) ++n;
    }
  return n;
}
template <int NG, int MODE, int P = 0>
__global__ __launch_bounds__(256, 2) void k_gemm_tn_small(WgradArgs p, int nbatch, int bpb) {
  constexpr int NTN = (NG + 3) / 4, NSTORE = MODE == 3 ? tn_small_stores3<NG, P>() : 4 * NG, NML = MODE == 3 ? 2 : 0;
  constexpr int STAGE = 8192 + 16384, NST = 3;
  __shared__ __attribute__((aligned(16))) char lds[NST * STAGE];
  const int t = threadIdx.x, lane = t & 63;
  const int wvu = __builtin_amdgcn_readfirstlane(t >> 6);
  const int k0 = blockIdx.x * 128;
  const int b0 = blockIdx.y * bpb, nit = min(bpb, nbatch - b0);
  const char* zp = (const char*)g_zero_page;
  const int ar = t >> 3, ac = t & 7;
  const bool va = ac * 8 < p.Cout;
  const int xr = t >> 4, xc = (t & 15) ^ fsw(t >> 4);
  const int kc = (k0 >> 3) + xc;
  const bool vk = kc < p.Kc;
  int sb = 0;
  auto stage = [&](int slot) {
    char* base = lds + slot * STAGE;
    const char* db = p.dy + (long)(b0 + sb) * p.bd + ac * 16;
    const char* xb = p.x + (long)(b0 + sb) * p.bx + (long)kc * 16;
#pragma unroll
    for (int i = 0; i < 2; ++i) {
      const int m = ar + 32 * i;
      glds16((va && m < p.M) ? db + ((long)m * p.ldd) * 2 : zp, base + (i * 256 + wvu * 64) * 16);
    }
#pragma unroll
    for (int i = 0; i < 4; ++i) {
      const int m = xr + 16 * i;
      glds16((vk && m < p.M) ? xb + ((long)m * p.xrs) * 16 : zp, base + 8192 + (i * 256 + wvu * 64) * 16);
    }
    ++sb;
  };
  f32x16 acc[NTN];
#pragma unroll
  for (int a = 0; a < NTN; ++a)
#pragma unroll
    for (int r = 0; r < 16; ++r) acc[a][r] = 0.f;
  const unsigned lbase = (unsigned)(size_t)(__attribute__((address_space(3))) char*)lds;
  unsigned aoff[NTN][2], xoff[2];
  {
    const int g = lane >> 4, li = lane & 15, q = li >> 2, pp = li & 3, hh = g >> 1;
#pragma unroll
    for (int a = 0; a < NTN; ++a) {
      const int col = a * 32 + 16 * (g & 1) + 4 * pp;
      aoff[a][0] = (8 * hh + q) * 128 + col * 2;
      aoff[a][1] = aoff[a][0] + 4 * 128;
    }
    const TrFragS<__bf16>::Off o = TrFragS<__bf16>::prep(wvu * 32, lane);
    xoff[0] = 8192 + o.o0; xoff[1] = 8192 + o.o1;
  }
  const int r = lane & 31, h = lane >> 5;
  f32x16 gacc[MODE == 3 ? NTN : 1];
  if (MODE == 3) {
#pragma unroll
    for (int a = 0; a < NTN; ++a)
#pragma unroll
      for (int g = 0; g < 16; ++g) gacc[a][g] = 0.f;
  }
  if (nit > 0) stage(0);
  if (nit > 1) stage(1);
  auto item = [&](int it, auto KIND) {
    constexpr int kind = decltype(KIND)::value;
    const int slot = it % NST;
    float g0v = 0.f;
    u32x2 mbv = {~0u, ~0u};
    if (MODE == 3) {
      const long ci = (long)(b0 + it) * p.K + k0 + wvu * 32 + r;
      const char* gp = (const char*)(p.g0 + ci);
      const char* mp = (const char*)(p.mbits + ci);
      asm volatile("global_load_dword %0, %1, off" : "=v"(g0v) : "v"(gp) : "memory");
      asm volatile("global_load_dwordx2 %0, %1, off" : "=v"(mbv) : "v"(mp) : "memory");
    }
    if (kind == 2) {
      stage((it + 2) % NST);
      if (it) wait_vm<12 + NML + NSTORE>(); else wait_vm<12 + NML>();
    } else if (kind == 1) {
      if (it) wait_vm<6 + NML + NSTORE>(); else wait_vm<6 + NML>();
    } else {
      wait_vm<0>();
    }
    __builtin_amdgcn_s_barrier();
    const unsigned sbase = lbase + slot * STAGE;
#define CDDMSL_TRS(DST, A0, A1, IMM)                                                             \
  { u32x2 q0_, q1_;                                                                              \
    asm volatile("ds_read_b64_tr_b16 %0, %1 offset:%2" : "=v"(q0_) : "v"(A0), "i"(IMM));         \
    asm volatile("ds_read_b64_tr_b16 %0, %1 offset:%2" : "=v"(q1_) : "v"(A1), "i"(IMM));         \
    DST = u32x4{q0_[0], q0_[1], q1_[0], q1_[1]}; }
    u32x4 fa[NTN][4], fb[4];
    const unsigned x0 = sbase + xoff[0], x1 = sbase + xoff[1];
    CDDMSL_TRS(fb[0], x0, x1, 0) CDDMSL_TRS(fb[1], x0, x1, 4096) CDDMSL_TRS(fb[2], x0, x1, 8192) CDDMSL_TRS(fb[3], x0, x1, 12288)
#pragma unroll
    for (int a = 0; a < NTN; ++a) {
      const unsigned a0 = sbase + aoff[a][0], a1 = sbase + aoff[a][1];
      CDDMSL_TRS(fa[a][0], a0, a1, 0) CDDMSL_TRS(fa[a][1], a0, a1, 2048) CDDMSL_TRS(fa[a][2], a0, a1, 4096) CDDMSL_TRS(fa[a][3], a0, a1, 6144)
    }
#undef CDDMSL_TRS
    if (NTN == 1) asm volatile("s_waitcnt lgkmcnt(0)" : "+v"(fb[0]), "+v"(fb[1]), "+v"(fb[2]), "+v"(fb[3]), "+v"(fa[0][0]), "+v"(fa[0][1]),
                               "+v"(fa[0][2]), "+v"(fa[0][3]) :: "memory");
    else asm volatile("s_waitcnt lgkmcnt(0)" : "+v"(fb[0]), "+v"(fb[1]), "+v"(fb[2]), "+v"(fb[3]), "+v"(fa[0][0]), "+v"(fa[0][1]), "+v"(fa[0][2]),
                      "+v"(fa[0][3]), "+v"(fa[NTN - 1][0]), "+v"(fa[NTN - 1][1]), "+v"(fa[NTN - 1][2]), "+v"(fa[NTN - 1][3]) :: "memory");
    __builtin_amdgcn_sched_barrier(0);
#pragma unroll
    for (int ms = 0; ms < 4; ++ms)
#pragma unroll
      for (int a = 0; a < NTN; ++a) Mma<__bf16>::step(acc[a], fa[a][ms], fb[ms]);
    __builtin_amdgcn_s_barrier();
    char* outp = (char*)p.dw + (long)(b0 + it) * p.bo;
    const int k = k0 + wvu * 32 + r;
    if (MODE == 3) {
      if (kind == 2) asm volatile("s_waitcnt vmcnt(6)" : "+v"(g0v), "+v"(mbv) :: "memory");
      else asm volatile("s_waitcnt vmcnt(0)" : "+v"(g0v), "+v"(mbv) :: "memory");
      const unsigned a00 = __builtin_bit_cast(unsigned, acc[0][0]);
      const float t0 = __builtin_bit_cast(float, __builtin_amdgcn_permlane32_swap(a00, a00, false, false)[0]) + g0v;
      const float base = t0 * (1.0f / (float)(P > 0 ? P : 1));
      const unsigned mlo = mbv[0], mhi = mbv[1];
#pragma unroll
      for (int a = 0; a < NTN; ++a)
#pragma unroll
        for (int g = 0; g < 16; ++g) {
          const int n0 = a * 32 + (g & 3) + 8 * (g >> 2);
          const bool exists = a * 4 + (g >> 2) < NG;
          const bool lo_ok = n0 >= 1 && n0 <= P, hi_ok = n0 + 4 >= 1 && n0 + 4 <= P;
          if (exists) {
            const int n = n0 + 4 * h;
            const float v = acc[a][g];
            gacc[a][g] += (n == 0) ? t0 : v;
            if (lo_ok || hi_ok) {
              if (h ? hi_ok : lo_ok) {
                const unsigned word = (n - 1) < 32 ? mlo : mhi;
                const bool keep = (word >> ((n - 1) & 31)) & 1u;
                Mma<__bf16>::store(outp + ((long)(n - 1) * p.ldo + k) * 2, keep ? v + base : 0.f);
              }
            }
          }
          acc[a][g] = 0.f;
        }
      return;
    }
#pragma unroll
    for (int a = 0; a < NTN; ++a)
#pragma unroll
      for (int g = 0; g < 16; ++g) {
        if (a * 4 + (g >> 2) < NG) {
          const int n = a * 32 + (g & 3) + 8 * (g >> 2) + 4 * h;
          const float v = acc[a][g];
          const long o = (long)n * p.ldo + k;
          if (MODE == 0) atomicAdd((float*)outp + o, v);
          else if (MODE == 1) ((float*)outp)[o] = v;
          else Mma<__bf16>::store(outp + o * 2, v);
        }
        acc[a][g] = 0.f;
      }
  };
  {
    int it = 0;
    for (; it + 2 < nit; ++it) item(it, std::integral_constant<int, 2>{});
    if (it + 1 < nit) { item(it, std::integral_constant<int, 1>{}); ++it; }
    if (it < nit) item(it, std::integral_constant<int, 0>{});
  }
  if (MODE == 3 && p.gpos) {
    const int k = k0 + wvu * 32 + r;
#pragma unroll
    for (int a = 0; a < NTN; ++a)
#pragma unroll
      for (int g = 0; g < 16; ++g) {
        const int n = a * 32 + (g & 3) + 8 * (g >> 2) + 4 * h;
        if (a * 4 + (g >> 2) < NG && n <= P) atomicAdd(p.gpos + (long)n * p.K + k, gacc[a][g]);
      }
  }
}

__global__ __launch_bounds__(512) void k_wgrad256(WgradArgs p) {
  __shared__ __attribute__((aligned(16))) u32x4 lds[2 * 2 * 2 * 64 * 16];
  const int t = threadIdx.x, lane = t & 63;
#ifdef CDDMSL_TILE_STAMPS
  const unsigned long long ts_entry = __builtin_amdgcn_s_memrealtime();
  unsigned long long ts_loop = ts_entry;
#endif
  p.x += (long)blockIdx.y * p.bx; p.dy += (long)blockIdx.y * p.bd;
  char* outp = (char*)p.dw + (long)blockIdx.y * p.bo;
  const int wvu = __builtin_amdgcn_readfirstlane(t >> 6);
  const int wn = wvu >> 2, wk = wvu & 3;
  const int ntn = p.Cout >> 8, ntk = p.K >> 8;
  int bid = xcd_remap(blockIdx.x, gridDim.x);
  const int tile_k = bid % ntk; bid /= ntk;
  const int tile_n = bid % ntn; bid /= ntn;
  const int n0 = tile_n * 256, k0 = tile_k * 256;
  const int mt0 = bid * p.mtiles_per_split;
  const int nmt = min(p.mtiles_per_split, (p.M + WM - 1) / WM - mt0);
  const bool taps = !(p.KH == 1 && p.KW == 1);

  const int rb = t >> 4, cl = (t & 15) ^ fsw(rb);
  const int gd = (cl >> 3) * 16 + (cl & 7);
  const int gx = (cl >> 2) * 8 + (cl & 3);
  const int kc = (k0 >> 3) + gx;
  const int pp = kc / p.cpp, coff = kc - pp * p.cpp;
  const int ky = pp / p.KW, kx = pp - ky * p.KW;
  unsigned vd[2], vx[2];
#pragma unroll
  for (int i = 0; i < 2; ++i) {
    vd[i] = (unsigned)((i * 32 + rb) * p.ldd * 2 + gd * 16);
    vx[i] = (unsigned)((((i * 32 + rb) + ky * p.Wi + kx) * p.xrs + coff) * 16);
  }
  const __amdgpu_buffer_rsrc_t rd = __builtin_amdgcn_make_buffer_rsrc((void*)(p.dy + ((long)mt0 * WM * p.ldd + n0) * 2), 0, 0x80000000u, 0x00020000);
  const __amdgpu_buffer_rsrc_t rx = __builtin_amdgcn_make_buffer_rsrc((void*)(p.x + ((long)mt0 * WM - p.pad * p.Wi - p.pad) * p.xrs * 16), 0, 0x80000000u, 0x00020000);
  const unsigned dstep = (unsigned)(WM * p.ldd * 2), xstep = (unsigned)(WM * p.xrs * 16);
  const int mrow = mt0 * WM + rb;

  char* const L = (char*)lds;
  auto stageD = [&](auto H, int buf, int T) {
    constexpr int h = decltype(H)::value;
    char* dst = L + (buf << 16) + (h << 14) + wvu * 1024;
#pragma unroll
    for (int i = 0; i < 2; ++i) {
      const unsigned inv = (mrow + T * WM + i * 32 < p.M) ? 0u : 0x80000000u;
      __builtin_amdgcn_raw_ptr_buffer_load_lds(rd, (__attribute__((address_space(3))) void*)(dst + i * 8192 - h * 128), 16,
                                               (int)(vd[i] | inv), (int)(T * dstep), h * 128, 0);
    }
  };
  unsigned xinv[2];
  auto validX = [&](int T) {
#pragma unroll
    for (int i = 0; i < 2; ++i) {
      const int m = mrow + T * WM + i * 32;
      bool ok = m < p.M;
      if (taps) {
        const unsigned mm = min((unsigned)m, (unsigned)(p.M - 1));
        const unsigned tq = fdiv(mm, p.dWo);
        const unsigned ox = mm - tq * p.Wo;
        const unsigned oy = tq - fdiv(tq, p.dHo) * p.Ho;
        ok = ok & ((unsigned)((int)oy - p.pad + ky) < (unsigned)p.Hi) & ((unsigned)((int)ox - p.pad + kx) < (unsigned)p.Wi);
      }
      xinv[i] = ok ? 0u : 0x80000000u;
    }
  };
  auto stageX = [&](auto J, int buf, int T) {
    constexpr int j = decltype(J)::value;
    char* dst = L + (buf << 16) + (1 << 15) + (j << 14) + wvu * 1024;
#pragma unroll
    for (int i = 0; i < 2; ++i)
      __builtin_amdgcn_raw_ptr_buffer_load_lds(rx, (__attribute__((address_space(3))) void*)(dst + i * 8192 - j * 64), 16,
                                               (int)(vx[i] | xinv[i]), (int)(T * xstep), j * 64, 0);
  };
  using I0 = std::integral_constant<int, 0>;
  using I1 = std::integral_constant<int, 1>;

  f32x16 acc[4][2];
#pragma unroll
  for (int a = 0; a < 4; ++a)
#pragma unroll
    for (int b = 0; b < 2; ++b)
#pragma unroll
      for (int r = 0; r < 16; ++r) acc[a][b][r] = 0.f;

  const unsigned lbase = (unsigned)(size_t)(__attribute__((address_space(3))) char*)L;
  unsigned adA[2][2], adB[2];
  {
#pragma unroll
// ... 1573 lines not shown
      }
      hipLaunchKernelGGL(k_wgrad256, dim3((unsigned)(tiles2 * sp)), dim3(512), 0, (hipStream_t)stream, a);
      return launch_status();
    }
    a.mtiles_per_split = keep;
  }
  g_last_kernel = same ? 5 : 4;
  if (g_plan_only) return CDDMSL_OK;
  if (same && dtype == 0 && splits > 1 && use_workspace(grid, 16384)) {
    a.ws = (float*)g_ws;
    hipLaunchKernelGGL(k_conv_wgrad_dma<__bf16>, dim3((unsigned)grid), dim3(256), 0, (hipStream_t)stream, a);
    hipLaunchKernelGGL((k_wgrad_reduce<4, 16>), dim3((unsigned)(tiles * 16)), dim3(256), 0, (hipStream_t)stream, (const f32x4*)g_ws, dw, scale,
                       (Cout + 127) / 128, (a.K + 127) / 128, (int)splits, Cout, a.K, a.ldo);
  } else if (same) {
    if (dtype == 0) hipLaunchKernelGGL(k_conv_wgrad_dma<__bf16>, dim3((unsigned)grid), dim3(256), 0, (hipStream_t)stream, a);
    else hipLaunchKernelGGL(k_conv_wgrad_dma<float>, dim3((unsigned)grid), dim3(256), 0, (hipStream_t)stream, a);
  } else {
    if (dtype == 0) hipLaunchKernelGGL(k_conv_wgrad<__bf16>, dim3((unsigned)grid), dim3(256), 0, (hipStream_t)stream, a);
    else hipLaunchKernelGGL(k_conv_wgrad<float>, dim3((unsigned)grid), dim3(256), 0, (hipStream_t)stream, a);
  }
  return launch_status();
}

extern "C" int cddmsl_conv_wgrad_fp8_ok(int Cin, int Cout, int KH, int KW, int pad, int ldd) {
  return (Cin % 256 == 0 && Cout % 256 == 0 && KH == KW && (KH & 1) && 2 * pad == KH - 1 && ldd % 16 == 0) ? 1 : 0;
}
extern "C" int cddmsl_conv_wgrad_fp8(const void* x8, const void* dy8, float* dw, const float* scale, int Nimg, int Hi, int Wi, int Cin,
                                     int Cout, int KH, int KW, int pad, int ldd, void* stream) {
  if (Nimg < 0 || Hi <= 0 || Wi <= 0 || !cddmsl_conv_wgrad_fp8_ok(Cin, Cout, KH, KW, pad, ldd) || ldd < Cout) return CDDMSL_ERR_ARG;
  WgradArgs a;
  a.x = (const char*)x8; a.dy = (const char*)dy8; a.dw = dw; a.scale = scale;
  a.Nimg = Nimg; a.Hi = Hi; a.Wi = Wi; a.Cin = Cin; a.Cout = Cout; a.KH = KH; a.KW = KW; a.stride = 1; a.pad = pad;
  a.ldd = ldd; a.pool = 0; a.Ho = Hi; a.Wo = Wi;
  const long M = (long)Nimg * Hi * Wi;
  if (M > 0x7fffff00L) return CDDMSL_ERR_ARG;
  a.M = (int)M; a.cpp = Cin / 16; a.Kc = KH * KW * a.cpp; a.K = KH * KW * Cin; a.ncc = Cout / 16;
  a.dWo = make_fastdiv((unsigned)a.Wo); a.dHo = make_fastdiv((unsigned)a.Ho);
  a.xrs = a.cpp; a.ldo = a.K; a.direct = 0; a.bx = a.bd = a.bo = 0;
  if (a.M == 0) return CDDMSL_OK;
  const int total_mt = (a.M + WM - 1) / WM;
  const long tiles = (long)(Cout / 256) * (a.K / 256), maxs = (total_mt + 15) / 16;
  long sp = 1;
  double best = -1.0;
  for (int r = 1; r <= 6; ++r) {
    long c = (256L * r) / tiles;
    if (c < 1) continue;
    if (c > maxs) c = maxs;
    const long blocks = tiles * c, rounds = (blocks + 255) / 256;
    const double eff = (double)blocks / (256.0 * rounds);
    if (eff > best + 0.02) { best = eff; sp = c; }
    if (c == maxs) break;
  }
  a.mtiles_per_split = (int)((total_mt + sp - 1) / sp);
  sp = (total_mt + a.mtiles_per_split - 1) / a.mtiles_per_split;
  const long rowb = ldd > a.xrs * 16 ? ldd : a.xrs * 16;
  if (((long)a.mtiles_per_split * WM + WM + 2L * Wi + 2) * rowb + (1L << 20) >= (1L << 31)) return CDDMSL_ERR_ARG;
  g_last_kernel = 12;
  if (g_plan_only) return CDDMSL_OK;
  if (sp > 1 && use_workspace(tiles * sp, 65536)) {
    a.ws = (float*)g_ws;
    hipLaunchKernelGGL(k_wgrad256_f8, dim3((unsigned)(tiles * sp)), dim3(512), 0, (hipStream_t)stream, a);
    hipLaunchKernelGGL((k_wgrad_reduce<8, 32>), dim3((unsigned)(tiles * 64)), dim3(256), 0, (hipStream_t)stream, (const f32x4*)g_ws, dw, scale,
                       Cout / 256, a.K / 256, (int)sp, Cout, a.K, a.ldo);
    return launch_status();
  }
  hipLaunchKernelGGL(k_wgrad256_f8, dim3((unsigned)(tiles * sp)), dim3(512), 0, (hipStream_t)stream, a);
  return launch_status();
}

extern "C" int cddmsl_gemm_nt_batched(const void* a, const void* w, void* c, const float* bias, int M, int N, int K, int lda,
                                      int ldb, int ldc, int batch, long sa, long sw, long sc, int out_f32, int dtype, void* stream) {
  int es = dtype == 0 ? 2 : 4;
  if (dtype != 0 && dtype != 1) return CDDMSL_ERR_ARG;
  if (M < 0 || N <= 0 || K <= 0 || batch < 0 || batch > 65535) return CDDMSL_ERR_ARG;
  if ((K * es) % 16 || (lda * es) % 16 || (ldb * es) % 16 || (sa * es) % 16 || (sw * es) % 16) return CDDMSL_ERR_ARG;
  if (M == 0 || batch == 0) return CDDMSL_OK;
  ConvArgs p;
  p.x = (const char*)a; p.w = (const char*)w; p.y = (char*)c; p.scale = nullptr; p.bias = bias; p.residual = nullptr; p.relu_mask = nullptr;
  p.Nimg = 1; p.Hi = 1; p.Wi = M; p.Cin = K; p.Ho = 1; p.Wo = M; p.Cout = N; p.KH = 1; p.KW = 1; p.stride = 1; p.pad = 0;
  p.ldy = ldc; p.ldr = 0; p.ldm = 0; p.relu = 0; p.out_f32 = out_f32; p.pool = 0; p.res_f32 = 0; p.res_pool = 0;
  p.M = M; p.cpp = K * es / 16; p.Kc = p.cpp;
  p.dWo = make_fastdiv((unsigned)M); p.dHo = make_fastdiv(1u); p.dcpp = make_fastdiv((unsigned)p.cpp); p.dKW = make_fastdiv(1u);
  p.xrs = lda * es / 16; p.wrs = ldb * es / 16;
  p.bx = sa * es; p.bw = sw * es; p.by = sc * (out_f32 ? 4 : es);
  g_batch = batch;
  int st = dtype == 0 ? conv_fwd_launch<__bf16>(p, (hipStream_t)stream) : conv_fwd_launch<float>(p, (hipStream_t)stream);
  g_batch = 1;
  return st;
}

extern "C" int cddmsl_gemm_tn_batched(const void* a, const void* b, void* out, int M, int N, int K, int lda, int ldb, int ldo,
                                      int batch, long sa, long sb, long so, int mode, int dtype, void* stream) {
  int es = dtype == 0 ? 2 : 4;
  if (dtype != 0 && dtype != 1) return CDDMSL_ERR_ARG;
  if (M <= 0 || N <= 0 || K <= 0 || batch <= 0 || batch > 65535 || mode < 0 || mode > 2) return CDDMSL_ERR_ARG;
  if ((K * es) % 16 || (N * es) % 16 || (lda * es) % 16 || (ldb * es) % 16 || (sa * es) % 16 || (sb * es) % 16) return CDDMSL_ERR_ARG;
  WgradArgs p;
  p.x = (const char*)b; p.dy = (const char*)a; p.dw = (float*)out; p.scale = nullptr;
  p.Nimg = 1; p.Hi = 1; p.Wi = M; p.Cin = K; p.Ho = 1; p.Wo = M; p.Cout = N; p.KH = 1; p.KW = 1; p.stride = 1; p.pad = 0;
  p.ldd = lda; p.pool = 0; p.M = M; p.cpp = K * es / 16; p.Kc = p.cpp; p.K = K; p.ncc = N * es / 16;
  p.dWo = make_fastdiv((unsigned)M); p.dHo = make_fastdiv(1u);
  p.xrs = ldb * es / 16; p.ldo = ldo; p.direct = mode;
  p.bx = sb * es; p.bd = sa * es; p.bo = so * (mode == 2 ? es : 4);
  int cols = 256 / es;
  long tiles = (long)((N + cols - 1) / cols) * ((K + cols - 1) / cols);
  int total_mt = (M + WM - 1) / WM;
  long splits = 1;
  if (mode == 0) {
    long want = (2048 + tiles * batch - 1) / (tiles * batch);
    long maxs = (total_mt + 7) / 8;
    splits = want < 1 ? 1 : (want > maxs ? maxs : want);
    if (splits < 1) splits = 1;
  }
  if (dtype == 0 && total_mt == 1 && N <= 64 && batch >= 64 && K % 128 == 0 && N % 8 == 0) {
    const long kt = K / 128;
    long bpb = (kt * batch + 4095) / 4096;
    if (bpb < 8) bpb = 8;
    if (bpb > batch) bpb = batch;
    const unsigned gy = (unsigned)((batch + bpb - 1) / bpb);
    g_last_kernel = 9;
    if (g_plan_only) return CDDMSL_OK;
#define CDDMSL_TNS(NG)                                                                                                               \
  case NG:                                                                                                                           \
    if (mode == 0) hipLaunchKernelGGL((k_gemm_tn_small<NG, 0>), dim3((unsigned)kt, gy), dim3(256), 0, (hipStream_t)stream, p, batch, (int)bpb);      \
    else if (mode == 1) hipLaunchKernelGGL((k_gemm_tn_small<NG, 1>), dim3((unsigned)kt, gy), dim3(256), 0, (hipStream_t)stream, p, batch, (int)bpb); \
    else hipLaunchKernelGGL((k_gemm_tn_small<NG, 2>), dim3((unsigned)kt, gy), dim3(256), 0, (hipStream_t)stream, p, batch, (int)bpb);                \
    break;
    switch (N / 8) { CDDMSL_TNS(1) CDDMSL_TNS(2) CDDMSL_TNS(3) CDDMSL_TNS(4) CDDMSL_TNS(5) CDDMSL_TNS(6) CDDMSL_TNS(7) CDDMSL_TNS(8) }
#undef CDDMSL_TNS
    return launch_status();
  }
  if (total_mt <= 4 && batch >= 64) {
    long bpb = (tiles * batch + 4095) / 4096, minb = (8 + total_mt - 1) / total_mt;
    if (bpb < minb) bpb = minb;
    if (bpb > batch) bpb = batch;
    const unsigned gy = (unsigned)((batch + bpb - 1) / bpb);
    g_last_kernel = 7;
    if (g_plan_only) return CDDMSL_OK;
    if (dtype == 0) hipLaunchKernelGGL(k_gemm_tn_stream<__bf16>, dim3((unsigned)tiles, gy), dim3(256), 0, (hipStream_t)stream, p, batch, (int)bpb);
    else hipLaunchKernelGGL(k_gemm_tn_stream<float>, dim3((unsigned)tiles, gy), dim3(256), 0, (hipStream_t)stream, p, batch, (int)bpb);
    return launch_status();
  }
  p.mtiles_per_split = (int)((total_mt + splits - 1) / splits);
  splits = (total_mt + p.mtiles_per_split - 1) / p.mtiles_per_split;
  long grid = tiles * splits;
  if (grid > 0x7fffffffL) return CDDMSL_ERR_ARG;
  g_last_kernel = 5;
  if (g_plan_only) return CDDMSL_OK;
  if (dtype == 0) hipLaunchKernelGGL(k_conv_wgrad_dma<__bf16>, dim3((unsigned)grid, (unsigned)batch), dim3(256), 0, (hipStream_t)stream, p);
  else hipLaunchKernelGGL(k_conv_wgrad_dma<float>, dim3((unsigned)grid, (unsigned)batch), dim3(256), 0, (hipStream_t)stream, p);
  return launch_status();
}

extern "C" int cddmsl_attnpool_dx(const void* pds, const void* zu, const float* g0, const unsigned long long* mbits, void* dx, float* gpos,
                                  int K, int H2, int P, int TP, int C, int dtype, void* stream) {
  if (dtype != 0 || K < 0 || P != 49 || TP != 56 || H2 <= 0 || H2 > 64 || (H2 & 7) || C <= 0 || (C & 127) || !g0 || !mbits || !dx) return CDDMSL_ERR_ARG;
  if (K == 0) return CDDMSL_OK;
  if (K > 65535 * 8) return CDDMSL_ERR_ARG;
  WgradArgs p;
  p.x = (const char*)zu; p.dy = (const char*)pds; p.dw = (float*)dx; p.scale = nullptr;
  p.Nimg = 1; p.Hi = 1; p.Wi = H2; p.Cin = C; p.Ho = 1; p.Wo = H2; p.Cout = TP; p.KH = 1; p.KW = 1; p.stride = 1; p.pad = 0;
  p.ldd = TP; p.pool = 0; p.M = H2; p.cpp = C * 2 / 16; p.Kc = p.cpp; p.K = C; p.ncc = TP * 2 / 16;
  p.dWo = make_fastdiv((unsigned)H2); p.dHo = make_fastdiv(1u);
  p.xrs = C * 2 / 16; p.ldo = C; p.direct = 3;
  p.bx = (long)H2 * C * 2; p.bd = (long)H2 * TP * 2; p.bo = (long)P * C * 2;
  p.g0 = g0; p.mbits = mbits; p.gpos = gpos;
  const long kt = C / 128;
  long bpb = (kt * K + 4095) / 4096;
  if (bpb < 8) bpb = 8;
  if (bpb > K) bpb = K;
  const unsigned gy = (unsigned)((K + bpb - 1) / bpb);
  hipLaunchKernelGGL((k_gemm_tn_small<7, 3, 49>), dim3((unsigned)kt, gy), dim3(256), 0, (hipStream_t)stream, p, K, (int)bpb);
  return launch_status();
}

extern "C" int cddmsl_weight_prep_multi(const long long* table, int count, int dtype, void* stream) {
  if ((dtype != 0 && dtype != 1) || count < 0 || count > 65535) return CDDMSL_ERR_ARG;
  if (count == 0) return CDDMSL_OK;
  if (dtype == 0) hipLaunchKernelGGL(k_weight_prep_multi<__bf16>, dim3(256, (unsigned)count), dim3(256), 0, (hipStream_t)stream, table);
  else hipLaunchKernelGGL(k_weight_prep_multi<float>, dim3(256, (unsigned)count), dim3(256), 0, (hipStream_t)stream, table);
  return launch_status();
}

extern "C" int cddmsl_weight_prep(const float* w, const float* scale, void* w_fwd, void* w_dgrad, int Cout, int KH,
                                  int KW, int Cin, int dtype, void* stream) {
  if (dtype != 0 && dtype != 1) return CDDMSL_ERR_ARG;
  long n = (long)Cout * KH * KW * Cin;
  if (n <= 0) return n == 0 ? CDDMSL_OK : CDDMSL_ERR_ARG;
  const long tiles = (long)((Cout + 31) / 32) * KH * KW * ((Cin + 31) / 32);
  unsigned grid = (unsigned)(tiles > 4096 ? 4096 : tiles);
  if (dtype == 0) hipLaunchKernelGGL(k_weight_prep<__bf16>, dim3(grid), dim3(256), 0, (hipStream_t)stream, w, scale, (char*)w_fwd, (char*)w_dgrad, Cout, KH, KW, Cin);
  else hipLaunchKernelGGL(k_weight_prep<float>, dim3(grid), dim3(256), 0, (hipStream_t)stream, w, scale, (char*)w_fwd, (char*)w_dgrad, Cout, KH, KW, Cin);
  return launch_status();
}
```

cddmsl_amd/hip.py:

```python
import ctypes
import os
from ctypes import c_float, c_int, c_long, c_void_p

import torch

from ._lib import check, lib, ptr, require_cuda, stream_ptr

DT = {torch.bfloat16: 0, torch.float32: 1}

_sigs_done = False


def _L():
    global _sigs_done
    L = lib()
    if not _sigs_done:
        vp, ci, cf = c_void_p, c_int, c_float
        L.cddmsl_last_kernel.argtypes = []
        L.cddmsl_plan_only.argtypes = [ci]
        L.cddmsl_conv_fwd.argtypes = [vp] * 7 + [ci] * 16 + [vp]
        L.cddmsl_conv_wgrad.argtypes = [vp] * 4 + [ci] * 12 + [vp]
        L.cddmsl_set_workspace.argtypes = [vp, c_long]
        L.cddmsl_weight_prep.argtypes = [vp] * 4 + [ci] * 5 + [vp]
        L.cddmsl_weight_prep_multi.argtypes = [vp, ci, ci, vp]
        L.cddmsl_preprocess.argtypes = [vp, vp] + [ci] * 6 + [vp, vp, ci, ci, vp]
        L.cddmsl_maxpool3s2_fwd.argtypes = [vp, vp] + [ci] * 5 + [vp]
        L.cddmsl_upsample_zero2.argtypes = [vp] * 4 + [ci] * 5 + [vp]
        L.cddmsl_meanpool_fwd.argtypes = [vp, vp, c_long, ci, ci, ci, vp]
        L.cddmsl_meanpool_bwd.argtypes = [vp, vp, c_long, ci, ci, ci, vp]
        L.cddmsl_preprocess224.argtypes = [vp, vp] + [ci] * 11 + [vp, vp, ci, vp]
        L.cddmsl_preprocess_batch.argtypes = [vp, vp, vp, ci, vp, ci, ci, ci, vp, vp, ci, ci, vp]
        L.cddmsl_preprocess224_batch.argtypes = [vp, vp, vp, ci, vp] + [ci] * 8 + [vp, vp, ci, vp]
        L.cddmsl_avgpool2_fwd.argtypes = [vp, vp] + [ci] * 5 + [vp]
        L.cddmsl_avgpool2_bwd.argtypes = [vp] * 4 + [ci] * 5 + [vp]
        L.cddmsl_avgpool2_bwd_q8.argtypes = [vp] * 4 + [ci] * 4 + [vp] * 4
        L.cddmsl_attn_tokens_fwd.argtypes = [vp] * 3 + [ci] * 5 + [vp]
        L.cddmsl_attn_tokens_bwd.argtypes = [vp] * 4 + [ci] * 5 + [vp]
        L.cddmsl_attnpool_softmax_fwd.argtypes = [vp] * 3 + [c_long, ci, ci, ci, cf, ci, vp]
        L.cddmsl_attnpool_softmax_bwd.argtypes = [vp] * 4 + [c_long, ci, ci, ci, cf, ci, vp]
        L.cddmsl_gemm_nt_batched.argtypes = [vp] * 4 + [ci] * 7 + [c_long] * 3 + [ci, ci, vp]
        L.cddmsl_gemm_tn_batched.argtypes = [vp] * 3 + [ci] * 7 + [c_long] * 3 + [ci, ci, vp]
        L.cddmsl_relu_bwd.argtypes = [vp, vp, vp, c_long, ci, ci, vp]
        L.cddmsl_colsum.argtypes = [vp, vp, c_long, ci, ci, ci, vp]
        L.cddmsl_sgd_clip_step.argtypes = [vp] * 4 + [ci, vp] + [cf] * 4 + [ci, vp]
        L.cddmsl_roi_align_forward.argtypes = [vp] * 5 + [ci] * 7 + [cf, ci, ci, ci, vp]
        L.cddmsl_roi_align_backward.argtypes = [vp] * 7 + [ci] * 7 + [cf, ci, ci, ci, vp]
        L.cddmsl_nms_anyorder.argtypes = [vp] * 4 + [ci, cf, vp, vp, vp]
        L.cddmsl_roi_align_nchw_anyorder.argtypes = [vp] * 3 + [ci] * 7 + [cf, ci, ci, ci, vp, vp, vp]
        L.cddmsl_roi_align_backward_nchw_anyorder.argtypes = [vp] * 3 + [ci] * 7 + [cf, ci, ci, ci, vp, vp, vp]
        L.cddmsl_quantize_fp8.argtypes = [vp] * 4 + [c_long, ci, vp]
        L.cddmsl_conv_fwd_fp8.argtypes = [vp] * 7 + [ci] * 10 + [vp] * 4
        L.cddmsl_conv_wgrad_fp8_ok.argtypes = [ci] * 6
        L.cddmsl_conv_wgrad_fp8.argtypes = [vp] * 4 + [ci] * 9 + [vp]
        L.cddmsl_conv_fwd_q8.argtypes = [vp] * 7 + [ci] * 10 + [vp] * 4
        L.cddmsl_fp8_dot_nt.argtypes = [vp] * 4 + [ci] * 4 + [vp]
        L.cddmsl_roi_align_forward_affine.argtypes = [vp] * 6 + [ci] * 8 + [cf, ci, ci, ci] + [vp] * 4
        L.cddmsl_roi_align_backward_pooled.argtypes = [vp] * 7 + [ci] * 7 + [cf, ci, ci, ci, vp]
        L.cddmsl_anchors.argtypes = [vp, vp, ci, ci, ci, cf, cf, vp]
        L.cddmsl_sort_desc.argtypes = [vp] * 5 + [ci, ci, vp, vp, vp]
        L.cddmsl_rpn_decode.argtypes = [vp] * 6 + [ci] * 5 + [cf] * 8 + [vp]
        L.cddmsl_nms.argtypes = [vp] * 5 + [ci, ci, cf, ci, vp]
        L.cddmsl_iou_match.argtypes = [vp, ci, vp, ci, vp, vp, vp, ci, cf, cf, ci, ci, ci, ci, vp]
        L.cddmsl_iou_match_batched.argtypes = [vp] * 7 + [ci] * 5 + [cf, cf] + [ci] * 4 + [vp]
        L.cddmsl_l2norm_fwd.argtypes = [vp, vp, vp, c_long, ci, cf, vp]
        L.cddmsl_l2norm_bwd.argtypes = [vp, vp, vp, vp, c_long, ci, vp]
        L.cddmsl_cosine_logits_fwd.argtypes = [vp] * 4 + [c_long, ci, ci, cf, cf, vp]
        L.cddmsl_cosine_logits_bwd.argtypes = [vp] * 5 + [c_long, ci, ci, cf, ci, vp]
        L.cddmsl_layernorm_fwd.argtypes = [vp] * 6 + [c_long, ci, cf, ci, vp]
        L.cddmsl_layernorm_bwd.argtypes = [vp] * 6 + [c_long, ci, ci, ci, vp]
        L.cddmsl_focal_ce_fwd.argtypes = [vp] * 4 + [c_long, ci, cf, ci, cf, vp]
        L.cddmsl_focal_ce_bwd.argtypes = [vp] * 5 + [c_long, ci, cf, ci, cf, vp]
        L.cddmsl_attn_small_fwd.argtypes = [vp] * 4 + [ci] * 8 + [cf, ci, vp]
        L.cddmsl_attn_small_bwd.argtypes = [vp] * 7 + [ci] * 8 + [cf, ci, vp]
        L.cddmsl_attn_tokens_fwd_mask.argtypes = [vp] * 4 + [ci] * 5 + [vp]
        L.cddmsl_attnpool_dx.argtypes = [vp] * 6 + [ci] * 6 + [vp]
        L.cddmsl_rpn_losses.argtypes = [vp, vp, vp, ci, vp, ci, vp, vp, vp, vp, c_long, cf, cf, cf, cf, cf, vp, vp, vp, vp, vp]
        L.cddmsl_box_l1.argtypes = [vp, ci, vp, ci, vp, vp, vp, cf, cf, cf, cf, cf, vp, vp, vp, vp]
        L.cddmsl_attn_last_fwd.argtypes = [vp] * 4 + [ci] * 8 + [cf, ci, vp]
        L.cddmsl_attn_last_bwd.argtypes = [vp] * 6 + [ci] * 8 + [cf, ci, vp]
        L.cddmsl_contrastive_fwd.argtypes = [vp] * 4 + [ci, ci, vp]
        L.cddmsl_contrastive_bwd.argtypes = [vp] * 5 + [ci, ci, vp]
        L.cddmsl_instance_boxes.argtypes = [vp] + [ci] * 4 + [vp, ci, vp, vp, vp, vp]
        _sigs_done = True
    return L


class _Profiler:

    def __init__(self):
        self.on = False
        self.only = None
        self.events = []
        self.shapes = []

    def enable(self, only=None):
        self.on, self.only, self.events, self.shapes = True, (set(only) if only else None), [], []

    def begin(self, name=None, plan=None):
        if not self.on:
            return None
        if self.only is not None:
            if name is None and plan is not None:
                L = _L()
                L.cddmsl_plan_only(1)
                try:
                    plan()
                finally:
                    L.cddmsl_plan_only(0)
                name = _CONV_KERNEL.get(L.cddmsl_last_kernel())
            if name not in self.only:
                return None
        e = torch.cuda.Event(enable_timing=True)
        e.record()
        return e

    def end(self, e0, name, flops=0.0, shape=None, nbytes=0.0):
        if e0 is None:
            return
        e1 = torch.cuda.Event(enable_timing=True)
        e1.record()
        self.events.append((name, flops, e0, e1, nbytes))
        if shape is not None:
            self.shapes.append((name, shape, flops, e0, e1, nbytes))

    def by_shape(self):
        torch.cuda.synchronize()
        out = {}
        for name, shape, flops, e0, e1, nbytes in self.shapes:
            d = out.setdefault((name, shape), [0, 0.0, 0.0, 0.0])
            d[0] += 1
            d[1] += e0.elapsed_time(e1)
            d[2] += flops
            d[3] += nbytes
        return out

    def collect(self):
        torch.cuda.synchronize()
        out = {}
        for name, flops, e0, e1, nbytes in self.events:
            d = out.setdefault(name, {"flops": 0.0, "ms": 0.0, "launches": 0, "bytes": 0.0})
            d["flops"] += flops
            d["bytes"] += nbytes
            d["ms"] += e0.elapsed_time(e1)
            d["launches"] += 1
        self.on, self.only, self.events = False, None, []
        return out


PROFILE = _Profiler()
_CONV_KERNEL = {10: "k_conv_fwd256_fp8", 11: "k_conv_fwd2", 1: "k_conv_fwd", 2: "k_conv_fwd_reg", 3: "k_conv_fwd256", 4: "k_conv_wgrad", 5: "k_conv_wgrad_dma", 6: "k_wgrad256", 7: "k_gemm_tn_stream", 8: "k_conv3x3_small", 9: "k_gemm_tn_small", 12: "k_wgrad256_fp8"}


def _timed(name):
    def deco(fn):
        def wrapper(*a, **k):
            e0 = PROFILE.begin(name)
            r = fn(*a, **k)
            PROFILE.end(e0, name)
            return r
        wrapper.__name__, wrapper.__doc__ = fn.__name__, fn.__doc__
        return wrapper
    return deco


def _dt(t):
    if t.dtype not in DT:
        raise TypeError(f"unsupported dtype {t.dtype}: the kernels compute in bf16 or f32")
    return DT[t.dtype]


def _conv_input_pixels(N, H, W, Ho, Wo, KH, KW, stride, pool):
    if pool:
        return N * min(H, 2 * Ho) * min(W, 2 * Wo)
    rows = min(H, Ho * min(KH, stride) if stride > KH else (Ho - 1) * stride + KH)
    cols = min(W, Wo * min(KW, stride) if stride > KW else (Wo - 1) * stride + KW)
    return N * rows * cols


class OutSpec:

    def __init__(self):
        self.full, self.used = None, 0


def conv_fwd(x, w, scale=None, bias=None, residual=None, relu=False, relu_mask=None, stride=1, pad=0,
             pool=False, out_f32=False, residual_pooled=False, emit8=None, out_spec=None):
    require_cuda(x, w, scale, bias, residual, relu_mask)
    ensure_workspace(x.device)
    assert x.dim() == 4 and w.dim() == 4 and x.is_contiguous() and w.is_contiguous()
    assert x.dtype == w.dtype
    N, H, W, Cin = x.shape
    Cout, KH, KW, Cin2 = w.shape
    assert Cin == Cin2, (x.shape, w.shape)
    if pool:
# ... 151 lines not shown
        return _L().cddmsl_conv_wgrad(ptr(x), ptr(dy), ptr(out), ptr(scale), N, H, W, Cin, Cout, KH, KW, stride, pad,
                                      int(pool), Cout, _dt(x), stream_ptr())
    e0 = PROFILE.begin(plan=launch) if PROFILE.on else None
    st = launch()
    check(st, "cddmsl_conv_wgrad")
    PROFILE.end(e0, _CONV_KERNEL.get(_L().cddmsl_last_kernel(), "conv_wgrad") if e0 is not None else "conv_wgrad",
                2.0 * (dy.numel() // Cout) * Cout * KH * KW * Cin,
                (dy.numel() // Cout, Cout, KH * KW * Cin, KH, int(pool), stride),
                nbytes=float(_conv_input_pixels(N, H, W, (H // 2) if pool else (H + 2 * pad - KH) // stride + 1,
                                                 (W // 2) if pool else (W + 2 * pad - KW) // stride + 1, KH, KW, stride, bool(pool)) * Cin * x.element_size()
                             + dy.numel() * dy.element_size() + out.numel() * 4))
    return out


def conv_wgrad_fp8_ok(M, Cin, Cout, KH, KW, pad, min_m=None, taps_only=True):
    min_m = int(os.environ.get("CDDMSL_FP8_WGRAD_MIN_M", "300000" if min_m is None else str(min_m)))
    return os.environ.get("CDDMSL_FP8_WGRAD", "1") != "0" and (KH * KW > 1 or not taps_only) and M >= min_m \
        and bool(_L().cddmsl_conv_wgrad_fp8_ok(Cin, Cout, KH, KW, pad, Cout))


def conv_wgrad_fp8(x8, dy8, w_shape, scale, pad=0, out=None):
    require_cuda(x8, dy8, scale, out)
    Cout, KH, KW, Cin = w_shape
    N, H, W, Cin2 = x8.shape
    assert Cin == Cin2 and x8.dtype == torch.uint8 and dy8.dtype == torch.uint8 and x8.is_contiguous() and dy8.is_contiguous()
    assert dy8.shape[-1] == Cout and dy8.numel() // Cout == N * H * W and 2 * pad == KH - 1
    assert scale is not None and scale.dtype == torch.float32 and scale.numel() == Cout and scale.is_contiguous()
    if out is None:
        out = torch.zeros(w_shape, device=x8.device, dtype=torch.float32)
    assert out.dtype == torch.float32 and out.is_contiguous() and tuple(out.shape) == tuple(w_shape)
    ensure_workspace(x8.device)
    def launch():
        return _L().cddmsl_conv_wgrad_fp8(ptr(x8), ptr(dy8), ptr(out), ptr(scale), N, H, W, Cin, Cout, KH, KW, pad, Cout, stream_ptr())
    e0 = PROFILE.begin(name="k_wgrad256_fp8") if PROFILE.on else None
    check(launch(), "cddmsl_conv_wgrad_fp8")
    PROFILE.end(e0, "k_wgrad256_fp8", 2.0 * (N * H * W) * Cout * KH * KW * Cin, (N * H * W, Cout, KH * KW * Cin, KH, 0, 1),
                nbytes=float(x8.numel() + dy8.numel() + out.numel() * 4))
    return out


@_timed("weight_prep")
def weight_prep(w_master, scale, dtype, want_fwd=True, want_dgrad=True):
    require_cuda(w_master, scale)
    assert w_master.dtype == torch.float32 and w_master.is_contiguous() and w_master.dim() == 4
    Cout, KH, KW, Cin = w_master.shape
    wf = torch.empty((Cout, KH, KW, Cin), device=w_master.device, dtype=dtype) if want_fwd else None
    wd = torch.empty((Cin, KH, KW, Cout), device=w_master.device, dtype=dtype) if want_dgrad else None
    st = _L().cddmsl_weight_prep(ptr(w_master), ptr(scale), ptr(wf), ptr(wd), Cout, KH, KW, Cin, DT[dtype], stream_ptr())
    check(st, "cddmsl_weight_prep")
    return wf, wd


@_timed("weight_prep")
def weight_prep_multi(table, count, dtype):
    require_cuda(table)
    assert table.dtype == torch.int64 and table.is_contiguous() and table.shape == (count, 8)
    check(_L().cddmsl_weight_prep_multi(ptr(table), count, DT[dtype], stream_ptr()), "cddmsl_weight_prep_multi")


def _f3(v):
    return (c_float * 3)(*[float(x) for x in v])


def _image_table(images_u8):
    import ctypes
    n = len(images_u8)
    ptrs = (ctypes.c_void_p * n)(*[im.data_ptr() for im in images_u8])
    hs = (ctypes.c_int * n)(*[int(im.shape[1]) for im in images_u8])
    ws = (ctypes.c_int * n)(*[int(im.shape[2]) for im in images_u8])
    return ptrs, hs, ws


@_timed("preprocess")
def preprocess(images_u8, Hp, Wp, mean, std, dtype, Cp=None, div255=True):
    require_cuda(*images_u8)
    Cp = Cp or (8 if dtype == torch.bfloat16 else 4)
    out = torch.empty((len(images_u8), Hp, Wp, Cp), device=images_u8[0].device, dtype=dtype)
    m, s = _f3(mean), _f3(std)
    for im in images_u8:
        assert im.dtype == torch.uint8 and im.dim() == 3 and im.shape[0] == 3 and im.is_contiguous()
    ptrs, hs, ws = _image_table(images_u8)
    check(_L().cddmsl_preprocess_batch(ptrs, hs, ws, len(images_u8), ptr(out), Hp, Wp, Cp, m, s, int(div255), DT[dtype], stream_ptr()),
          "cddmsl_preprocess_batch")
    return out


@_timed("preprocess224")
def preprocess224(images_u8, Hp, Wp, mean, std, dtype, size=224, Cp=None):
    require_cuda(*images_u8)
    Cp = Cp or (8 if dtype == torch.bfloat16 else 4)
    if Wp <= Hp:
        RW, RH = size, int(size * Hp / Wp)
    else:
        RH, RW = size, int(size * Wp / Hp)
    top, left = int(round((RH - size) / 2.0)), int(round((RW - size) / 2.0))
    out = torch.empty((len(images_u8), size, size, Cp), device=images_u8[0].device, dtype=dtype)
    m, s = _f3(mean), _f3(std)
    for im in images_u8:
        assert im.dtype == torch.uint8 and im.dim() == 3 and im.is_contiguous()
    ptrs, hs, ws = _image_table(images_u8)
    check(_L().cddmsl_preprocess224_batch(ptrs, hs, ws, len(images_u8), ptr(out), Hp, Wp, RH, RW, top, left, size, Cp,
                                           m, s, DT[dtype], stream_ptr()), "cddmsl_preprocess224_batch")
    return out


@_timed("avgpool2_fwd")
def avgpool2_fwd(x):
    require_cuda(x)
    N, H, W, C = x.shape
    y = torch.empty((N, H // 2, W // 2, C), device=x.device, dtype=x.dtype)
    check(_L().cddmsl_avgpool2_fwd(ptr(x), ptr(y), N, H, W, C, _dt(x), stream_ptr()), "cddmsl_avgpool2_fwd")
    return y


@_timed("avgpool2_bwd")
def avgpool2_bwd(dy, in_shape, mask=None, add=None, emit8=None):
    require_cuda(dy, mask, add)
    N, H, W, C = in_shape
    assert dy.is_contiguous() and tuple(dy.shape) == (N, H // 2, W // 2, C)
    dx = torch.empty(in_shape, device=dy.device, dtype=dy.dtype)
    if emit8 is not None and dy.dtype == torch.bfloat16:
        y8 = torch.empty(in_shape, device=dy.device, dtype=torch.uint8)
        check(_L().cddmsl_avgpool2_bwd_q8(ptr(dy), ptr(mask), ptr(add), ptr(dx), N, H, W, C, ptr(y8), ptr(emit8[0]), ptr(emit8[1]), stream_ptr()),
              "cddmsl_avgpool2_bwd_q8")
        dx._fp8 = (y8, emit8[0].data_ptr())
        return dx
    check(_L().cddmsl_avgpool2_bwd(ptr(dy), ptr(mask), ptr(add), ptr(dx), N, H, W, C, _dt(dy), stream_ptr()), "cddmsl_avgpool2_bwd")
    return dx


@_timed("attn_tokens_fwd")
def attn_tokens_fwd(x, pos, tp=None):
    require_cuda(x, pos)
    K, P, C = x.shape
    tp = tp or P + 1
    assert pos.dtype == torch.float32 and tuple(pos.shape) == (P + 1, C) and x.is_contiguous() and pos.is_contiguous()
    tok = torch.empty((K, tp, C), device=x.device, dtype=x.dtype)
    check(_L().cddmsl_attn_tokens_fwd(ptr(x), ptr(pos), ptr(tok), K, P, tp, C, _dt(x), stream_ptr()), "cddmsl_attn_tokens_fwd")
    return tok


@_timed("attn_tokens_fwd")
def attn_tokens_fwd_mask(x, pos, tp=None):
    require_cuda(x, pos)
    K, P, C = x.shape
    tp = tp or P + 1
    assert pos.dtype == torch.float32 and tuple(pos.shape) == (P + 1, C) and x.is_contiguous() and pos.is_contiguous() and P <= 64
    tok = torch.empty((K, tp, C), device=x.device, dtype=x.dtype)
    mbits = torch.empty((K, C), device=x.device, dtype=torch.int64)
    check(_L().cddmsl_attn_tokens_fwd_mask(ptr(x), ptr(pos), ptr(tok), ptr(mbits), K, P, tp, C, _dt(x), stream_ptr()), "cddmsl_attn_tokens_fwd_mask")
    return tok, mbits


def rpn_losses(logits, deltas, pos, neg, midx, gt, gt_off, anchors, weights, inv_norm, gout=None):
    require_cuda(logits, deltas, pos, neg, midx, gt, gt_off, anchors)
    for t in (logits, deltas, gt, anchors):
        assert t.dtype == torch.float32 and t.is_contiguous()
    for t in (pos, neg, midx, gt_off):
        assert t.dtype == torch.int64 and t.is_contiguous()
    A = anchors.shape[0]
    assert deltas.numel() == 4 * logits.numel() and midx.numel() == logits.numel()
    args = (ptr(logits), ptr(deltas), ptr(pos), pos.numel(), ptr(neg), neg.numel(), ptr(midx), ptr(gt), ptr(gt_off), ptr(anchors), A,
            *[float(w) for w in weights], float(inv_norm))
    if gout is None:
        out = torch.empty(2, device=logits.device, dtype=torch.float32)
        check(_L().cddmsl_rpn_losses(*args, ptr(out), None, None, None, stream_ptr()), "cddmsl_rpn_losses")
        return out
    dl, dd = torch.zeros_like(logits), torch.zeros_like(deltas)
    g = gout.contiguous().float()
    check(_L().cddmsl_rpn_losses(*args, None, ptr(g), ptr(dl), ptr(dd), stream_ptr()), "cddmsl_rpn_losses(backward)")
    return dl, dd


def box_l1(deltas, fg, cls, src, tgt, weights, inv_norm, gout=None):
    require_cuda(deltas, fg, src, tgt)
    assert deltas.dtype == torch.float32 and deltas.dim() == 2 and deltas.is_contiguous() and fg.dtype == torch.int64 and fg.is_contiguous()
    assert src.dtype == tgt.dtype == torch.float32 and src.is_contiguous() and tgt.is_contiguous() and (cls is None or (cls.dtype == torch.int64 and cls.is_contiguous()))
    args = (ptr(deltas), deltas.shape[1], ptr(fg), fg.numel(), ptr(cls), ptr(src), ptr(tgt), *[float(w) for w in weights], float(inv_norm))
    if gout is None:
        out = torch.empty(1, device=deltas.device, dtype=torch.float32)
        check(_L().cddmsl_box_l1(*args, ptr(out), None, None, stream_ptr()), "cddmsl_box_l1")
        return out
    dd = torch.zeros_like(deltas)
    g = gout.contiguous().float().view(1)
    check(_L().cddmsl_box_l1(*args, None, ptr(g), ptr(dd), stream_ptr()), "cddmsl_box_l1(backward)")
    return dd


def attnpool_dx_ok(K, H, P, TP, C, dtype):
    return dtype == torch.bfloat16 and P == 49 and TP == 56 and 2 * H <= 64 and (2 * H) % 8 == 0 and C % 128 == 0 and 0 < K <= 65535 * 8


@_timed("attnpool_dx")
def attnpool_dx(pds, zu, g0, mbits, P, gpos=None):
    require_cuda(pds, zu, g0, mbits)
    K, H2, TP = pds.shape
    C = zu.shape[2]
    assert pds.dtype == zu.dtype == torch.bfloat16 and g0.dtype == torch.float32 and mbits.dtype == torch.int64
    assert pds.is_contiguous() and zu.is_contiguous() and g0.is_contiguous() and mbits.is_contiguous() and tuple(zu.shape) == (K, H2, C)
    assert tuple(g0.shape) == (K, C) and tuple(mbits.shape) == (K, C) and (gpos is None or (gpos.dtype == torch.float32 and tuple(gpos.shape) == (P + 1, C) and gpos.is_contiguous()))
    dx = torch.empty((K, P, C), device=pds.device, dtype=pds.dtype)
    check(_L().cddmsl_attnpool_dx(ptr(pds), ptr(zu), ptr(g0), ptr(mbits), ptr(dx), ptr(gpos), K, H2, P, TP, C, 0, stream_ptr()), "cddmsl_attnpool_dx")
    return dx


@_timed("attn_tokens_bwd")
def attn_tokens_bwd(dtok, P, relu_mask=None, gpos=None, want_dx=True):
    require_cuda(dtok, relu_mask, gpos)
    K, TP, C = dtok.shape
    assert dtok.is_contiguous()
    assert relu_mask is None or (relu_mask.is_contiguous() and relu_mask.dtype == dtok.dtype and relu_mask.numel() == K * P * C)
    assert gpos is None or (gpos.is_contiguous() and gpos.dtype == torch.float32 and tuple(gpos.shape) == (P + 1, C))
    assert want_dx or gpos is not None
    dx = torch.empty((K, P, C), device=dtok.device, dtype=dtok.dtype) if want_dx else None
    check(_L().cddmsl_attn_tokens_bwd(ptr(dtok), ptr(relu_mask), ptr(dx), ptr(gpos), K, P, TP, C, _dt(dtok), stream_ptr()), "cddmsl_attn_tokens_bwd")
    return dx


@_timed("attnpool_softmax")
def attnpool_softmax_fwd(S, P1, scale, dtype):
    require_cuda(S)
    K, H, TP = S.shape
    assert S.dtype == torch.float32 and S.is_contiguous() and P1 <= TP
    p = torch.empty((K, H, P1), device=S.device, dtype=torch.float32)
    pT = torch.empty((K, TP, H), device=S.device, dtype=dtype)
    check(_L().cddmsl_attnpool_softmax_fwd(ptr(S), ptr(p), ptr(pT), K, H, P1, TP, float(scale), DT[dtype], stream_ptr()), "cddmsl_attnpool_softmax_fwd")
    return p, pT


@_timed("attnpool_softmax")
def attnpool_softmax_bwd(p, dP, scale, dtype):
    require_cuda(p, dP)
    K, H, P1 = p.shape
    TP = dP.shape[2]
    assert p.dtype == dP.dtype == torch.float32 and p.is_contiguous() and dP.is_contiguous() and dP.shape[:2] == (K, H)
    dsT = torch.empty((K, TP, H), device=p.device, dtype=dtype)
    pds = torch.empty((K, 2 * H, TP), device=p.device, dtype=dtype)
    check(_L().cddmsl_attnpool_softmax_bwd(ptr(p), ptr(dP), ptr(dsT), ptr(pds), K, H, P1, TP, float(scale), DT[dtype], stream_ptr()), "cddmsl_attnpool_softmax_bwd")
    return dsT, pds


def _eptr(t, elem_offset=0):
    return ctypes.c_void_p(t.data_ptr() + elem_offset * t.element_size())


@_timed("gemm_nt_batched")
def gemm_nt_batched(a, w, c, M, N, K, lda, ldb, ldc, batch, sa, sw, sc, a_off=0, w_off=0, c_off=0, bias=None):
    require_cuda(a, w, c, bias)
    assert a.dtype == w.dtype and c.dtype in (a.dtype, torch.float32)
    out_f32 = int(c.dtype == torch.float32 and a.dtype != torch.float32)
    check(_L().cddmsl_gemm_nt_batched(_eptr(a, a_off), _eptr(w, w_off), _eptr(c, c_off), ptr(bias), M, N, K, lda, ldb, ldc, batch,
                                      sa, sw, sc, out_f32, _dt(a), stream_ptr()), "cddmsl_gemm_nt_batched")


@_timed("gemm_tn_batched")
def gemm_tn_batched(a, b, out, M, N, K, lda, ldb, ldo, batch, sa, sb, so, a_off=0, b_off=0, o_off=0, accumulate=False):
    require_cuda(a, b, out)
    assert a.dtype == b.dtype
    if accumulate:
        assert out.dtype == torch.float32
        mode = 0
    else:
        mode = 1 if (out.dtype == torch.float32 and a.dtype != torch.float32) else (1 if out.dtype == torch.float32 else 2)
        assert out.dtype in (a.dtype, torch.float32)
    check(_L().cddmsl_gemm_tn_batched(_eptr(a, a_off), _eptr(b, b_off), _eptr(out, o_off), M, N, K, lda, ldb, ldo, batch, sa, sb, so,
                                      mode, _dt(a), stream_ptr()), "cddmsl_gemm_tn_batched")


@_timed("relu_bwd")
def relu_bwd(g, y):
    require_cuda(g, y)
    assert g.is_contiguous() and y.is_contiguous() and g.numel() == y.numel()
    g_f32 = int(g.dtype == torch.float32 and y.dtype != torch.float32)
    assert g_f32 or g.dtype == y.dtype
    dx = torch.empty_like(y)
    check(_L().cddmsl_relu_bwd(ptr(g), ptr(y), ptr(dx), y.numel(), g_f32, _dt(y), stream_ptr()), "cddmsl_relu_bwd")
    return dx


@_timed("colsum")
def colsum(x2d, period=1, out=None):
    require_cuda(x2d, out)
    rows, cols = x2d.shape
    assert x2d.is_contiguous()
    if out is None:
        out = torch.zeros((period, cols) if period > 1 else (cols,), device=x2d.device, dtype=torch.float32)
    check(_L().cddmsl_colsum(ptr(x2d), ptr(out), rows, cols, period, _dt(x2d), stream_ptr()), "cddmsl_colsum")
    return out


def same_layout(a, b):
    return a.shape == b.shape and all(sa == sb for sa, sb, n in zip(a.stride(), b.stride(), a.shape) if n > 1)


@_timed("sgd_clip_step")
def sgd_clip_step(params, grads, moms, norm_ws, lr, momentum, wd, clip, first_step):
    n = len(params)
    if n == 0:
        return
    require_cuda(*params, *grads, *moms)
    for p, g, m in zip(params, grads, moms):
        assert p.dtype == g.dtype == m.dtype == torch.float32
        assert same_layout(p, g) and same_layout(p, m), "param/grad/momentum must share a memory layout"
    P = (c_void_p * n)(*[p.data_ptr() for p in params])
    G = (c_void_p * n)(*[g.data_ptr() for g in grads])
    M = (c_void_p * n)(*[m.data_ptr() for m in moms])
# ... 474 lines not shown
```

cddmsl_amd/layers.py:

```python
import os
import weakref

import torch

from . import hip

_STEP = [0]


def bump_weight_version():
    _STEP[0] += 1


_LOAD_GEN = [0]


def note_weights_loaded(*_):
    _LOAD_GEN[0] += 1
    _STEP[0] += 1


def load_generation():
    return _LOAD_GEN[0]

# ... 579 lines not shown
        o1[K:].copy_(hip.conv_fwd(extra, w1, s1, b1, relu=True))
        px[K:].copy_(hip.avgpool2_fwd(extra))
    o2 = conv_fwd_auto(o1, bp.pw[1], s2, b2, f8, relu=True, pad=1)
    p2 = hip.avgpool2_fwd(o2)
    idn = conv_fwd_auto(px, bp.pw[3], bnd[0], bnd[1], f8)
    out_shape = (p2.shape[0], p2.shape[1], p2.shape[2], _ohwi(bp.w[2]).shape[0])
    out = conv_fwd_auto(p2, bp.pw[2], s3, b3, f8, emit8=fp8_emit_for(next_pw, out_shape, 0, f8), residual=idn, relu=True)
    return o1, o2, p2, px, out, (_fp8_made_for(o1, bp.pw[1]) if f8 else None)


class RoIStageFn(torch.autograd.Function):

    @staticmethod
    def forward(ctx, feat, anchor, rois, roi_start, blocks, out_size, scale, sr, out_grad_premasked, extra):
        feat = feat.contiguous()
        nxt = lambda i: blocks[i + 1].pw[0] if i + 1 < len(blocks) else None
        o1, o2, p2, px, cur, o1_8 = _roi_block0_forward(feat, rois, blocks[0], out_size, scale, sr, extra, nxt(0))
        saved, o1_8s = [feat, rois, roi_start, extra, o1, o2, p2, px, cur], [None, o1_8, None]
        for bi, bp in enumerate(blocks[1:], start=1):
            cur, mids = _block_forward(cur, bp, True, None, nxt(bi))
            saved += [mids[0], mids[1], mids[2], mids[3], cur]
            o1_8s += list(mids[4])
        ctx.blocks, ctx.meta = blocks, (out_size, scale, sr, out_grad_premasked)
        ctx.save_for_backward(*saved, *o1_8s)
        return cur

    @staticmethod
    def backward(ctx, g):
        blocks = ctx.blocks
        saved, o1_8s = ctx.saved_tensors[:-3 * len(blocks)], ctx.saved_tensors[-3 * len(blocks):]
        out_size, scale, sr, premasked = ctx.meta
        feat, rois, roi_start, extra = saved[:4]
        st = saved[4:]
        gs = g.contiguous() if premasked else hip.relu_bwd(g.contiguous(), st[-1])
        for i in range(len(blocks) - 1, 0, -1):
            o1, o2, p2, px = st[5 * i: 5 * i + 4]
            gs = _block_backward(gs, st[5 * i - 1], o1, o2, p2, px, blocks[i], True, mask_x=True, prev_bp=blocks[i - 1], c8=tuple(o1_8s[3 * i: 3 * i + 3]))
        bp = blocks[0]
        o1, o2, p2, px = st[0:4]
        T = o1.dtype
        (s1, _), (s2, _), (s3, _), bnd = bp.bn
        w1p, w2p, w3p, wdp = bp.w
        shp = lambda w: _ohwi(w).shape
        K, E = rois.shape[0], (0 if extra is None else extra.shape[0])
        f8 = bp.fp8 and T == torch.bfloat16
        gs_slot = fp8_slot_of(bp, "_fp8_gs") if f8 else None
        d2_slot = fp8_slot_of(bp.pw[1], "_fp8_g") if f8 else None
        hip.conv_wgrad(p2, gs, shp(w3p), s3, out=_ohwi(_grad_buf(w3p)))
        e8 = d2_slot.emit() if f8 and _fp8_dgrad_wanted(bp.pw[1], o2.shape, 1, f8) else None
        dpre2 = hip.avgpool2_bwd(dgrad_auto(gs, bp.pw[2], f8, gs_slot), tuple(o2.shape), mask=o2, emit8=e8)
        dpre1 = dgrad_auto(dpre2, bp.pw[1], f8, d2_slot, pad=1, relu_mask=o1)
        wgrad_auto(o1, dpre2, bp.pw[1], s2, 1, _ohwi(_grad_buf(w2p)), f8, o1_8s[1], d2_slot)
        hip.conv_wgrad(px, gs, shp(wdp), bnd[0], out=_ohwi(_grad_buf(wdp)))
        dxb = dgrad_auto(gs, bp.pw[3], f8, gs_slot)
        N, H, W, C = feat.shape
        dz = hip.roi_align_backward(dpre1[:K], rois, roi_start, (N, H, W, dpre1.shape[-1]), scale, sr, True)
        hip.conv_wgrad(feat, dz, shp(w1p), s1, out=_ohwi(_grad_buf(w1p)))
        _, w1d = bp.pw[0].get(T, True)
        dfeat = dextra = None
        if E:
            hip.conv_wgrad(extra, dpre1[K:], shp(w1p), s1, out=_ohwi(_grad_buf(w1p)))
            if ctx.needs_input_grad[9]:
                dextra = hip.conv_fwd(dpre1[K:], w1d, residual=hip.avgpool2_bwd(dxb[K:].contiguous(), tuple(extra.shape)))
        if ctx.needs_input_grad[0]:
            r = hip.roi_align_backward(dxb[:K], rois, roi_start, (N, H, W, C), scale, sr, True, pooled=True)
            dfeat = hip.conv_fwd(dz, w1d, residual=r)
        return dfeat, None, None, None, None, None, None, None, None, dextra


def roi_stage_supported(blocks):
    bp = blocks[0]
    return bp.stride == 2 and bp.w[3] is not None and tuple(bp.w[0].shape[2:]) == (1, 1) and tuple(bp.w[3].shape[2:]) == (1, 1)


def roi_stage(feat, rois, roi_start, blocks, frozen, out_size, scale, sr, extra=None, out_grad_premasked=False):
    assert rois.dim() == 2 and rois.size(1) == 5 and out_size % 2 == 0
    assert extra is None or tuple(extra.shape[1:]) == (out_size, out_size, feat.shape[3])
    if frozen or not torch.is_grad_enabled():
        nxt = lambda i: blocks[i + 1].pw[0] if i + 1 < len(blocks) else None
        cur = _roi_block0_forward(feat.contiguous(), rois, blocks[0], out_size, scale, sr, extra, nxt(0))[4]
        for bi, bp in enumerate(blocks[1:], start=1):
            cur, _ = _block_forward(cur, bp, False, None, nxt(bi))
        return cur
    return RoIStageFn.apply(feat, blocks[0].w[0], rois, roi_start, blocks, out_size, scale, sr, out_grad_premasked, extra)


def roi_stage_attnpool(feat, rois, roi_start, blocks, frozen, ap, out_size, scale, sr, extra=None):
    fuse = not frozen and torch.is_grad_enabled()
    y = roi_stage(feat, rois, roi_start, blocks, frozen, out_size, scale, sr, extra, out_grad_premasked=fuse)
    return AttnPoolFn.apply(y, None if ap.frozen else ap.q_w, ap, fuse)


class RoIAlignFn(torch.autograd.Function):
    @staticmethod
    def forward(ctx, x, rois, roi_start, out_size, scale, sampling_ratio, aligned, with_pooled=False, extra=None):
        K, E = rois.shape[0], (0 if extra is None else extra.shape[0])
        out = hip.roi_align_forward(x, rois, out_size, out_size, scale, sampling_ratio, aligned, with_pooled=with_pooled, extra_rows=E)
        ctx.save_for_backward(rois, roi_start)
        ctx.meta = (tuple(x.shape), scale, sampling_ratio, aligned, K)
        y = out[0] if with_pooled else out
        if E:
            y[K:].copy_(extra)
            if with_pooled:
                out[1][K:].copy_(hip.avgpool2_fwd(extra.contiguous()))
        if with_pooled:
            ctx.mark_non_differentiable(out[1])
        return out

    @staticmethod
    def backward(ctx, dy, *unused):
        rois, roi_start = ctx.saved_tensors
        shape, scale, sr, aligned, K = ctx.meta
        dy = dy.contiguous()
        dx = hip.roi_align_backward(dy[:K], rois, roi_start, shape, scale, sr, aligned)
        dextra = dy[K:] if (dy.shape[0] > K and ctx.needs_input_grad[8]) else None
        return dx, None, None, None, None, None, None, None, dextra


def roi_align(x, rois, roi_start, out_size, scale, sampling_ratio, aligned=True, with_pooled=False, extra=None):
    assert rois.dim() == 2 and rois.size(1) == 5
    assert extra is None or tuple(extra.shape[1:]) == (out_size, out_size, x.shape[3])
    if with_pooled and out_size % 2 == 0:
        y, yp = RoIAlignFn.apply(x, rois, roi_start, out_size, scale, sampling_ratio, aligned, True, extra)
        y._pooled2 = yp
        return y
    return RoIAlignFn.apply(x, rois, roi_start, out_size, scale, sampling_ratio, aligned, False, extra)


class AttnPoolParams:
    def __init__(self, pos, q_w, q_b, k_w, k_b, v_w, v_b, c_w, c_b, heads, frozen=False):
        self.pos, self.heads, self.frozen = pos, heads, frozen
        self.q_w, self.q_b, self.k_w, self.k_b, self.v_w, self.v_b, self.c_w, self.c_b = q_w, q_b, k_w, k_b, v_w, v_b, c_w, c_b
        self.pq = PreparedWeight(q_w, None, frozen)
        self.pk = PreparedWeight(k_w, None, frozen)
        self.pv = PreparedWeight(v_w, None, frozen)
        self.pc = PreparedWeight(c_w, None, frozen)


class AttnPoolFn(torch.autograd.Function):

    TP = 56

    @staticmethod
    def forward(ctx, x, anchor, ap, premask_input_grad=False):
        ctx.relu_src = x if premask_input_grad else None
        T = x.dtype
        K, h, w, C = x.shape
        P, TP, H = h * w, AttnPoolFn.TP, ap.heads
        D = C // H
        assert ap.pos.shape[0] == P + 1 <= TP, "attention pool needs a 7x7 map (clip_backbone.py:86)"
        dev = x.device
        fused_dx = hip.attnpool_dx_ok(K, H, P, TP, C, T) and bool(ctx.needs_input_grad[0]) and os.environ.get("CDDMSL_ATTNPOOL_DX", "1") != "0"
        mbits = None
        if fused_dx and premask_input_grad:
            tok, mbits = hip.attn_tokens_fwd_mask(x.view(K, P, C), ap.pos.detach(), TP)
        else:
            tok = hip.attn_tokens_fwd(x.view(K, P, C), ap.pos.detach(), TP)
        wq, _ = ap.pq.get(T, False)
        wk, wkT = ap.pk.get(T, True)
        wv, wvT = ap.pv.get(T, True)
        wc, _ = ap.pc.get(T, False)
        q0 = hip.conv_fwd(tok.view(K, 1, TP, C), wq, None, ap.q_b.detach(), stride=TP).view(K, C)
        zu = torch.empty((K, 2 * H, C), device=dev, dtype=T)
        hip.gemm_nt_batched(q0, wkT, zu, K, C, D, C, C, 2 * H * C, H, D, D, C, c_off=H * C)
        S = torch.empty((K, H, TP), device=dev, dtype=torch.float32)
        hip.gemm_nt_batched(zu, tok, S, H, TP, C, C, C, TP, K, 2 * H * C, TP * C, H * TP, a_off=H * C)
        p, pT = hip.attnpool_softmax_fwd(S, P + 1, D ** -0.5, T)
        z = torch.empty((K, H, C), device=dev, dtype=T)
        hip.gemm_tn_batched(pT, tok, z, TP, H, C, H, C, C, K, TP * H, TP * C, H * C)
        o = torch.empty((K, C), device=dev, dtype=T)
        hip.gemm_nt_batched(z, wv, o, K, D, C, H * C, C, C, H, C, D * C, D)
        o = o + ap.v_b.detach().to(T)
        out = hip.conv_fwd(o.view(1, 1, K, C), wc, None, ap.c_b.detach(), out_f32=True).view(K, -1)
        ctx.ap = ap
        ctx.fused_dx = fused_dx
        ctx.save_for_backward(tok, q0, zu, p, z, o, mbits)
        ctx.shape = (K, h, w, C)
        return out

    @staticmethod
    def backward(ctx, dout):
        ap = ctx.ap
        tok, q0, zu, p, z, o, mbits = ctx.saved_tensors
        K, h, w, C = ctx.shape
        P, TP, H = h * w, AttnPoolFn.TP, ap.heads
        D = C // H
        T = tok.dtype
        dev = tok.device
        train = not ap.frozen
        dout_t = dout.contiguous().to(T)
        if train:
            hip.conv_wgrad(o.view(1, 1, K, C), dout_t.view(1, 1, K, -1), _ohwi(ap.c_w).shape, out=_ohwi(_grad_buf(ap.c_w)))
            hip.colsum(dout_t, out=_grad_buf(ap.c_b))
        _, wcd = ap.pc.get(T, True)
        wk, wkT = ap.pk.get(T, True)
        wv, wvT = ap.pv.get(T, True)
        do = hip.conv_fwd(dout_t.view(1, 1, K, -1), wcd).view(K, C)
        if train:
            hip.colsum(do, out=_grad_buf(ap.v_b))
            hip.gemm_tn_batched(do, z, _grad_buf(ap.v_w), K, D, C, C, H * C, C, H, D, C, D * C, accumulate=True)
        hip.gemm_nt_batched(do, wvT, zu, K, C, D, C, C, 2 * H * C, H, D, D, C)
        dP = torch.empty((K, H, TP), device=dev, dtype=torch.float32)
        hip.gemm_nt_batched(zu, tok, dP, H, TP, C, C, C, TP, K, 2 * H * C, TP * C, H * TP)
        dsT, pds = hip.attnpool_softmax_bwd(p, dP, D ** -0.5, T)
        du = torch.empty((K, H, C), device=dev, dtype=T)
        hip.gemm_tn_batched(dsT, tok, du, TP, H, C, H, C, C, K, TP * H, TP * C, H * C)
        dq0 = torch.empty((K, C), device=dev, dtype=T)
        hip.gemm_nt_batched(du, wk, dq0, K, D, C, H * C, C, C, H, C, D * C, D)
        if train:
            hip.gemm_tn_batched(q0, du, _grad_buf(ap.k_w), K, D, C, C, H * C, C, H, D, C, D * C, accumulate=True)
            _grad_buf(ap.k_b)
            hip.conv_wgrad(tok.view(K, 1, TP, C), dq0.view(K, 1, 1, C), _ohwi(ap.q_w).shape, stride=TP, out=_ohwi(_grad_buf(ap.q_w)))
            hip.colsum(dq0, out=_grad_buf(ap.q_b))
        _, wqd = ap.pq.get(T, True)
        gpos = _grad_buf(ap.pos) if train else None
        want_dx = ctx.needs_input_grad[0]
        if ctx.fused_dx and want_dx:
            g0 = hip.conv_fwd(dq0.view(1, 1, K, C), wqd, out_f32=True).view(K, C)
            if mbits is None:
                mbits = torch.full((K, C), -1, device=dev, dtype=torch.int64)
            dx = hip.attnpool_dx(pds, zu, g0, mbits, P, gpos)
            return dx.view(K, h, w, C), None, None, None
        dtok = torch.empty((K, TP, C), device=dev, dtype=T)
        hip.gemm_tn_batched(pds, zu, dtok, 2 * H, TP, C, TP, C, C, K, 2 * H * TP, 2 * H * C, TP * C)
        dtok[:, 0, :] += hip.conv_fwd(dq0.view(1, 1, K, C), wqd).view(K, C)
        dx = None
        if want_dx or train:
            dx = hip.attn_tokens_bwd(dtok, P, ctx.relu_src if want_dx else None, gpos, want_dx)
        return (dx.view(K, h, w, C) if want_dx else None), None, None, None


def attnpool(x, ap):
    return AttnPoolFn.apply(x, None if ap.frozen else ap.q_w, ap)


_FP8_CONST = {}


def _fp8_const(value, device):
    k = (float(value), str(device))
    if k not in _FP8_CONST:
        _FP8_CONST[k] = torch.tensor([float(value)], device=device, dtype=torch.float32)
    return _FP8_CONST[k]


def fp8_unit_rows(wn):
    return hip.quantize_fp8(wn.contiguous(), _fp8_const(hip.FP8_MAX, wn.device))


class CosineLogitsFn(torch.autograd.Function):
    @staticmethod
    def forward(ctx, x, wn, temperature, fp8=False, wn8=None):
        x = x.contiguous()
        if fp8 and x.shape[1] % 64 == 0 and wn.shape[0] <= 32:
            xn, inv = hip.l2norm_fwd(x, 1e-12)
            unit = _fp8_const(hip.FP8_MAX, x.device)
            if wn8 is None:
                wn8 = fp8_unit_rows(wn)
            dot = hip.fp8_dot_nt(hip.quantize_fp8(xn, unit), wn8, _fp8_const(1.0 / (hip.FP8_MAX * hip.FP8_MAX * temperature), x.device))
            scores = torch.cat([dot, torch.zeros(x.shape[0], 1, device=x.device, dtype=torch.float32)], dim=1)
        else:
            scores, inv = hip.cosine_logits_fwd(x, wn, temperature)
        ctx.save_for_backward(x, wn, inv)
        ctx.t = temperature
        return scores

    @staticmethod
    def backward(ctx, ds):
        x, wn, inv = ctx.saved_tensors
        return hip.cosine_logits_bwd(ds, x.contiguous(), wn, inv, ctx.t), None, None, None, None


def cosine_logits(x, wn, temperature, fp8=False, wn8=None):
    return CosineLogitsFn.apply(x, wn, temperature, fp8, wn8)


class ContrastiveFn(torch.autograd.Function):

    @staticmethod
    def forward(ctx, a, b):
        an, ia = hip.l2norm_fwd(a.contiguous(), 0.0)
        bn, ib = hip.l2norm_fwd(b.contiguous(), 0.0)
        S = hip.linear_fwd(an, bn)
        loss, rl, cl = hip.contrastive_fwd(S)
        ctx.save_for_backward(an, ia, bn, ib, S, rl, cl)
        return loss.view(())

    @staticmethod
    def backward(ctx, g):
        an, ia, bn, ib, S, rl, cl = ctx.saved_tensors
        dS = hip.contrastive_bwd(S, rl, cl, g)
        n = dS.shape[0]
        pad = (-n) % 4
        P = (lambda t: torch.nn.functional.pad(t, (0, pad))) if pad else (lambda t: t)
        dan = hip.linear_fwd(P(dS).contiguous(), P(bn.t()).contiguous())
        dbn = hip.linear_fwd(P(dS.t()).contiguous(), P(an.t()).contiguous())
        return hip.l2norm_bwd(dan, an, ia), hip.l2norm_bwd(dbn, bn, ib)


def contrastive_loss(a, b):
    return ContrastiveFn.apply(a, b)


class LayerNormFn(torch.autograd.Function):

    @staticmethod
    def forward(ctx, x, gamma, beta, out_dtype):
        y, mean, rstd = hip.layernorm_fwd(x.contiguous(), gamma, beta, out_dtype)
        ctx.save_for_backward(x, gamma, mean, rstd)
        return y

    @staticmethod
    def backward(ctx, dy):
        x, gamma, mean, rstd = ctx.saved_tensors
        return hip.layernorm_bwd(dy, x.contiguous(), gamma, mean, rstd), None, None, None


def layer_norm(x2d, gamma, beta, out_dtype):
    return LayerNormFn.apply(x2d, gamma.detach(), beta.detach(), out_dtype)


class LayerNormSkipFn(torch.autograd.Function):

    @staticmethod
    def forward(ctx, x, gamma, beta, out_dtype):
        x = x.contiguous()
        y, mean, rstd = hip.layernorm_fwd(x, gamma, beta, out_dtype)
        ctx.save_for_backward(x, gamma, mean, rstd)
        return y, x.view_as(x)

    @staticmethod
    def backward(ctx, dy, dskip):
        x, gamma, mean, rstd = ctx.saved_tensors
        if dskip is None:
            return hip.layernorm_bwd(dy, x, gamma, mean, rstd), None, None, None
        acc = dskip.contiguous()
        if dy is None:
            return acc, None, None, None
        return hip.layernorm_bwd(dy, x, gamma, mean, rstd, accumulate_into=acc), None, None, None


def layer_norm_skip(x2d, gamma, beta, out_dtype):
    return LayerNormSkipFn.apply(x2d, gamma.detach(), beta.detach(), out_dtype)


class FocalCEFn(torch.autograd.Function):

    @staticmethod
    def forward(ctx, logits, target, gamma, bg_class, bg_weight):
        logits = logits.contiguous()
        row, probs = hip.focal_ce_fwd(logits, target, gamma, bg_class, bg_weight)
        ctx.save_for_backward(logits, target, probs)
        ctx.meta = (gamma, bg_class, bg_weight)
        return row.mean()

    @staticmethod
    def backward(ctx, g):
        logits, target, probs = ctx.saved_tensors
        gamma, bg_class, bg_weight = ctx.meta
        return hip.focal_ce_bwd(logits, target, probs, g / logits.shape[0], gamma, bg_class, bg_weight), None, None, None, None


def focal_cross_entropy(logits, target, gamma, bg_class, bg_weight):
    return FocalCEFn.apply(logits, target, float(gamma or 0.0), int(bg_class), float(1.0 if bg_weight is None else bg_weight))

# ... 117 lines not shown
```

include/cddmsl_hip.h:

```cpp
#ifndef CDDMSL_HIP_H
#define CDDMSL_HIP_H
#include <stddef.h>

#ifdef __cplusplus
extern "C" {
#endif

int cddmsl_abi_version(void);

int cddmsl_conv_fwd(const void* x, const void* w, void* y, const float* scale, const float* bias, const void* residual,
                    const void* relu_mask, int Nimg, int Hi, int Wi, int Cin, int Cout, int KH, int KW, int stride, int pad,
                    int pool, int ldy, int ldr, int ldm, int relu, int out_f32, int dtype, void* stream);
int cddmsl_set_workspace(void* ptr, long bytes);
int cddmsl_conv_wgrad(const void* x, const void* dy, float* dw, const float* scale, int Nimg, int Hi, int Wi, int Cin,
                      int Cout, int KH, int KW, int stride, int pad, int pool, int ldd, int dtype, void* stream);
int cddmsl_gemm_nt_batched(const void* a, const void* w, void* c, const float* bias, int M, int N, int K, int lda, int ldb, int ldc,
                           int batch, long sa, long sw, long sc, int out_f32, int dtype, void* stream);
int cddmsl_gemm_tn_batched(const void* a, const void* b, void* out, int M, int N, int K, int lda, int ldb, int ldo, int batch, long sa,
                           long sb, long so, int mode, int dtype, void* stream);
int cddmsl_last_kernel(void);
int cddmsl_plan_only(int on);
int cddmsl_weight_prep(const float* w, const float* scale, void* w_fwd, void* w_dgrad, int Cout, int KH, int KW, int Cin,
                       int dtype, void* stream);
int cddmsl_weight_prep_multi(const long long* table, int count, int dtype, void* stream);

int cddmsl_quantize_fp8(const void* x, void* y, const float* scale, float* amax, long numel, int src_dtype, void* stream);
int cddmsl_conv_fwd_fp8(const void* x, const void* w, void* y, const float* scale, const float* bias, const void* residual,
                        const void* relu_mask, int Nimg, int Hi, int Wi, int Cin, int Cout, int KH, int KW, int pad, int relu,
                        int out_f32, void* y8, const float* q8, float* amax8, void* stream);
int cddmsl_conv_fwd_q8(const void* x, const void* w, void* y, const float* scale, const float* bias, const void* residual,
                       const void* relu_mask, int Nimg, int Hi, int Wi, int Cin, int Cout, int KH, int KW, int stride, int pad,
                       int relu, void* y8, const float* q8, float* amax8, void* stream);
int cddmsl_fp8_dot_nt(const void* a, const void* b, float* c, const float* alpha, int R, int N, int K, int ldc, void* stream);
int cddmsl_conv_wgrad_fp8_ok(int Cin, int Cout, int KH, int KW, int pad, int ldd);
int cddmsl_conv_wgrad_fp8(const void* x8, const void* dy8, float* dw, const float* scale, int Nimg, int Hi, int Wi, int Cin, int Cout,
                          int KH, int KW, int pad, int ldd, void* stream);

int cddmsl_roi_align_forward(const void* x, const float* rois, void* y, void* y_pooled, int* dbg_grid, int N, int C, int H, int W,
                             int K, int ph, int pw, float spatial_scale, int sampling_ratio, int aligned, int dtype, void* stream);
int cddmsl_roi_align_backward(const void* dy, const float* rois, const int* roi_start, void* dx, float* ws_ay, float* ws_ax,
                              int* ws_fp, int N, int C, int H, int W, int K, int ph, int pw, float spatial_scale,
                              int sampling_ratio, int aligned, int dtype, void* stream);
int cddmsl_roi_align_forward_affine(const void* x, const float* rois, void* y, void* y_pooled, const float* scale,
                                    const float* bias, int relu, int N, int C, int H, int W, int K, int ph, int pw,
                                    float spatial_scale, int sampling_ratio, int aligned, int dtype, void* y8, const float* q8,
                                    float* amax8, void* stream);
int cddmsl_roi_align_backward_pooled(const void* dy, const float* rois, const int* roi_start, void* dx, float* ws_ay,
                                     float* ws_ax, int* ws_fp, int N, int C, int H, int W, int K, int ph, int pw,
                                     float spatial_scale, int sampling_ratio, int aligned, int dtype, void* stream);
int cddmsl_roi_align_nchw_anyorder(const void* input, const float* rois, void* output, int N, int C, int H, int W, int K, int ph, int pw,
                                   float spatial_scale, int sampling_ratio, int aligned, int dtype, void* temp, size_t* temp_bytes,
                                   void* stream);
int cddmsl_roi_align_backward_nchw_anyorder(const void* grad, const float* rois, void* grad_input, int N, int C, int H, int W, int K,
                                            int ph, int pw, float spatial_scale, int sampling_ratio, int aligned, int dtype, void* temp,
                                            size_t* temp_bytes, void* stream);

int cddmsl_anchors(const float* cell, float* out, int Hf, int Wf, int A, float stride, float offset, void* stream);
int cddmsl_sort_desc(const float* keys_in, float* keys_out, int* idx_scratch, int* order_out, const int* offsets, int N,
                     int total, void* temp, size_t* temp_bytes, void* stream);
int cddmsl_rpn_decode(const int* order, const float* deltas, const float* cell, const int* img_hw, float* boxes,
                      unsigned char* valid, int N, int Hf, int Wf, int A, int topk, float stride, float offset, float wx,
                      float wy, float ww, float wh, float scale_clamp, float min_size, void* stream);
int cddmsl_nms(const float* boxes, const unsigned char* valid, unsigned long long* mask_ws, int* keep, int* nkeep, int N,
               int n, float thr, int max_keep, void* stream);
int cddmsl_nms_anyorder(const float* boxes, const float* scores, long* keep, int* nkeep, int K, float iou_threshold, void* temp,
                        size_t* temp_bytes, void* stream);
int cddmsl_iou_match(const float* gt, int G, const float* preds, int P, long* matches, signed char* labels,
                     unsigned int* best_ws, int nthr, float t0, float t1, int l0, int l1, int l2, int allow_low_quality,
                     void* stream);

int cddmsl_iou_match_batched(const float* gt, const int* gt_off, const float* preds, const int* pred_off, long* matches,
                             signed char* labels, unsigned int* best_ws, int N, int P, int maxG, int totalG, int nthr, float t0,
                             float t1, int l0, int l1, int l2, int allow_low_quality, void* stream);

int cddmsl_attn_tokens_fwd(const void* x, const float* pos, void* tok, int K, int P, int TP, int C, int dtype, void* stream);
int cddmsl_attn_tokens_fwd_mask(const void* x, const float* pos, void* tok, unsigned long long* mbits, int K, int P, int TP, int C,
                                int dtype, void* stream);
int cddmsl_attnpool_dx(const void* pds, const void* zu, const float* g0, const unsigned long long* mbits, void* dx, float* gpos, int K,
                       int H2, int P, int TP, int C, int dtype, void* stream);
int cddmsl_attn_tokens_bwd(const void* dtok, const void* relu_mask, void* dx, float* gpos, int K, int P, int TP, int C, int dtype,
                           void* stream);
int cddmsl_attnpool_softmax_fwd(const float* S, float* p, void* pT, long K, int H, int P1, int TP, float scale, int dtype, void* stream);
int cddmsl_attnpool_softmax_bwd(const float* p, const float* dP, void* dsT, void* pds, long K, int H, int P1, int TP, float scale,
                                int dtype, void* stream);

int cddmsl_attn_small_fwd(const void* q, const void* k, const void* v, void* o, int nseq, int t, int heads, int dh, int ldq,
                          int ldk, int ldv, int ldo, float scale, int dtype, void* stream);
int cddmsl_attn_small_bwd(const void* q, const void* k, const void* v, const void* dout, void* dq, void* dk, void* dv, int nseq,
                          int t, int heads, int dh, int ldq, int ldk, int ldv, int ldo, float scale, int dtype, void* stream);
int cddmsl_attn_last_fwd(const void* q, const void* kv, void* o, float* p, int n, int t, int heads, int dh, int ldq, int ldkv, int voff,
                         int ldo, float scale, int dtype, void* stream);
int cddmsl_attn_last_bwd(const void* q, const void* kv, const void* dout, const float* p, void* dq, void* dkv, int n, int t, int heads,
                         int dh, int ldq, int ldkv, int voff, int ldo, float scale, int dtype, void* stream);

int cddmsl_l2norm_fwd(const float* x, float* y, float* inv, long R, int D, float eps, void* stream);
int cddmsl_l2norm_bwd(const float* dy, const float* y, const float* inv, float* dx, long R, int D, void* stream);
int cddmsl_cosine_logits_fwd(const float* x, const float* wn, float* scores, float* inv, long R, int D, int Kc,
                             float temperature, float eps, void* stream);
int cddmsl_cosine_logits_bwd(const float* ds, const float* x, const float* wn, const float* inv, float* dx, long R, int D,
                             int Kc, float temperature, int accumulate, void* stream);
int cddmsl_layernorm_fwd(const float* x, const float* gamma, const float* beta, void* y, float* mean, float* rstd, long R, int D,
                         float eps, int dtype, void* stream);
int cddmsl_layernorm_bwd(const void* dy, const float* x, const float* gamma, const float* mean, const float* rstd, float* dx,
                         long R, int D, int accumulate, int dtype, void* stream);
int cddmsl_focal_ce_fwd(const float* logits, const long* target, float* row_loss, float* probs, long R, int C, float gamma,
                        int bg_class, float bg_weight, void* stream);
int cddmsl_focal_ce_bwd(const float* logits, const long* target, const float* probs, const float* gscale, float* dlogits, long R,
                        int C, float gamma, int bg_class, float bg_weight, void* stream);
int cddmsl_contrastive_fwd(const float* S, float* rlse, float* clse, float* loss, int n, int ld, void* stream);
int cddmsl_contrastive_bwd(const float* S, const float* rlse, const float* clse, const float* gloss, float* dS, int n, int ld,
                           void* stream);
int cddmsl_rpn_losses(const float* logits, const float* deltas, const long* pos, int npos, const long* neg, int nneg, const long* midx,
                      const float* gt, const long* gt_off, const float* anchors, long A, float wx, float wy, float ww, float wh, float inv_norm,
                      float* out2, const float* gout2, float* dlogits, float* ddeltas, void* stream);
int cddmsl_box_l1(const float* deltas, int ld, const long* fg, int nfg, const long* cls, const float* src, const float* tgt, float wx, float wy,
                  float ww, float wh, float inv_norm, float* out1, const float* gout1, float* ddeltas, void* stream);

int cddmsl_preprocess(const unsigned char* img, void* out, int n, int h, int w, int Hp, int Wp, int Cp, const float* mean3,
                      const float* std3, int div255, int dtype, void* stream);
int cddmsl_preprocess224(const unsigned char* img, void* out, int n, int h, int w, int Hp, int Wp, int RH, int RW, int top,
                         int left, int S, int Cp, const float* mean3, const float* std3, int dtype, void* stream);
int cddmsl_preprocess_batch(const unsigned char* const* imgs, const int* hs, const int* ws, int N, void* out, int Hp, int Wp, int Cp,
                            const float* mean3, const float* std3, int div255, int dtype, void* stream);
int cddmsl_preprocess224_batch(const unsigned char* const* imgs, const int* hs, const int* ws, int N, void* out, int Hp, int Wp, int RH,
                               int RW, int top, int left, int S, int Cp, const float* mean3, const float* std3, int dtype, void* stream);
int cddmsl_avgpool2_fwd(const void* x, void* y, int N, int H, int W, int C, int dtype, void* stream);
int cddmsl_avgpool2_bwd(const void* dy, const void* mask, const void* add, void* dx, int N, int H, int W, int C, int dtype,
                        void* stream);
int cddmsl_avgpool2_bwd_q8(const void* dy, const void* mask, const void* add, void* dx, int N, int H, int W, int C, void* y8,
                           const float* q8, float* amax8, void* stream);
int cddmsl_maxpool3s2_fwd(const void* x, void* y, int N, int H, int W, int C, int dtype, void* stream);
int cddmsl_upsample_zero2(const void* t, const void* mask, const void* add, void* dx, int N, int H, int W, int C, int dtype,
                          void* stream);
int cddmsl_meanpool_fwd(const void* x, float* y, long K, int P, int C, int dtype, void* stream);
int cddmsl_meanpool_bwd(const float* dy, void* dx, long K, int P, int C, int dtype, void* stream);
int cddmsl_relu_bwd(const void* g, const void* y, void* dx, long numel, int g_f32, int dtype, void* stream);
int cddmsl_colsum(const void* x, float* out, long rows, int cols, int period, int dtype, void* stream);
int cddmsl_sgd_clip_step(float** params, const float** grads, float** moms, const long* sizes, int count, float* norm_ws,
                         float lr, float momentum, float wd, float clip, int first_step, void* stream);

int cddmsl_instance_boxes(const void* maps, int B, int H, int W, int dtype, int* records, int max_records, int* counts, void* ws,
                          size_t* ws_bytes, void* stream);

#ifdef __cplusplus
}
#endif
#endif
```

Measured before the change: 158.6.

## Avoid materializing attention-pool token tensor; read x, token0 and pos directly in GEMMs

Replaces the materialized (K, TP, C) token tensor (x + pos, mean token, padding) with a small token-0 tensor plus a bf16 copy of the positional embedding. The NT and TN batched GEMMs in the attention pool read rows straight from x, t0 and pos and add the positional term inside the kernel: an extra LDS read in the conv epilogue, and extra MFMA steps against preloaded pos fragments in the TN kernel. This is meant to cut the write and repeated reads of a large intermediate in both forward and backward. The cost is more complex address selection and extra MFMA work, and it is on by default via an env flag.

```diff
diff --git a/cddmsl_amd/csrc/elementwise.hip b/cddmsl_amd/csrc/elementwise.hip
--- a/cddmsl_amd/csrc/elementwise.hip
+++ b/cddmsl_amd/csrc/elementwise.hip
@@ -295,6 +295,36 @@
   }
 }
 template <typename T>
+__global__ void k_attn_token0(const char* x, const float* pos, char* t0, char* posT, unsigned long long* mbits, int K, int P, int cch) {
+  const int VEC = Elt<T>::VEC;
+  const long total = (long)K * cch, npos = posT ? (long)(P + 1) * cch : 0;
+  for (long i = (long)blockIdx.x * blockDim.x + threadIdx.x; i < total || i < npos; i += (long)gridDim.x * blockDim.x) {
+    if (i < npos) {
+      float o[8];
+#pragma unroll
+      for (int j = 0; j < VEC; ++j) o[j] = pos[i * VEC + j];
+      ((u32x4*)posT)[i] = Elt<T>::pack(o);
+    }
+    if (i >= total) continue;
+    int c = i % cch; long k = i / cch;
+    float s[8] = {0, 0, 0, 0, 0, 0, 0, 0}, v[8], o[8];
+    unsigned long long mb[8] = {0, 0, 0, 0, 0, 0, 0, 0};
+    for (int p = 0; p < P; ++p) {
+      Elt<T>::unpack(((const u32x4*)x)[(k * P + p) * cch + c], v);
+#pragma unroll
+      for (int j = 0; j < VEC; ++j) { s[j] += v[j]; mb[j] |= (unsigned long long)(v[j] > 0.f) << p; }
+    }
+    if (mbits) {
+#pragma unroll
+      for (int j = 0; j < VEC; ++j) mbits[(k * cch + c) * VEC + j] = mb[j];
+    }
+    const float* pe = pos + c * VEC;
+#pragma unroll
+    for (int j = 0; j < VEC; ++j) o[j] = s[j] / (float)P + pe[j];
+    ((u32x4*)t0)[k * cch + c] = Elt<T>::pack(o);
+  }
+}
+template <typename T>
 __global__ __launch_bounds__(256) void k_attn_tokens_bwd(const char* __restrict__ dtok, const char* __restrict__ relu_mask, char* __restrict__ dx, float* __restrict__ gpos, int K,
                                                          int P, int TP, int cch, int slab) {
   constexpr int V = Elt<T>::VEC;
@@ -715,6 +745,18 @@
   return launch_status();
 }
 
+extern "C" int cddmsl_attn_token0(const void* x, const float* pos, void* t0, void* posT, unsigned long long* mbits, int K, int P, int C,
+                                  int dtype, void* stream) {
+  int es = dtype == 0 ? 2 : 4;
+  if ((dtype != 0 && dtype != 1) || C <= 0 || (C * es) % 16 || P <= 0 || K < 0 || (K && !t0) || (mbits && P > 64)) return CDDMSL_ERR_ARG;
+  int cch = C * es / 16;
+  long total = (long)K * cch, npos = posT ? (long)(P + 1) * cch : 0;
+  if (npos > total) total = npos;
+  if (total == 0) return CDDMSL_OK;
+  DISPATCH(dtype, k_attn_token0, <<<dim3(gsz(total, 64)), dim3(64), 0, (hipStream_t)stream>>>((const char*)x, pos, (char*)t0, (char*)posT, mbits, K, P, cch));
+  return launch_status();
+}
+
 extern "C" int cddmsl_attn_tokens_bwd(const void* dtok, const void* relu_mask, void* dx, float* gpos, int K, int P, int TP, int C,
                                       int dtype, void* stream) {
   int es = dtype == 0 ? 2 : 4;
diff --git a/cddmsl_amd/csrc/gemm_conv.hip b/cddmsl_amd/csrc/gemm_conv.hip
--- a/cddmsl_amd/csrc/gemm_conv.hip
+++ b/cddmsl_amd/csrc/gemm_conv.hip
@@ -62,6 +62,10 @@
   float* partial = nullptr;
   int tile0 = 0, ksplits = 1, kper = 0, tile_limit = 0;
   int nt_out = 1;
+  const char* vt0 = nullptr;
+  const char* vpos = nullptr;
+  long bvt0 = 0;
+  int vtP = 0;
 #ifdef CDDMSL_STAMPS
   unsigned long long* stamps;
 #endif
@@ -349,7 +353,7 @@
   return ((oy >> 1) < hp && (ox >> 1) < wp) ? ((long)img * hp + (oy >> 1)) * wp + (ox >> 1) : -1L;
 }
 
-template <typename T>
+template <typename T, bool VT = false>
 __global__ __launch_bounds__(256, 2) void k_conv_fwd(ConvArgs p) {
   __shared__ __attribute__((aligned(16))) u32x4 lds[2][2][BM * KCH];
   const int t = threadIdx.x;
@@ -362,7 +366,8 @@
   const int cc = t & 7, rb = t >> 3;
   const int cl = cc ^ ((rb >> 1) & 7);
 
-  long rowoff[4], wrow[4];
+  long rowoff[4];
+  const char* wrow[4];
   int iy0[4], ix0[4];
   bool vm[4], vn[4];
 #pragma unroll
@@ -376,8 +381,15 @@
     ix0[i] = (int)ox * p.stride - p.pad;
     rowoff[i] = ((((long)img * p.Hi + iy0[i]) * p.Wi + ix0[i]) * p.xrs) * 16;
     int n = n0 + rb + 32 * i;
-    vn[i] = n < p.Cout;
-    wrow[i] = (long)(vn[i] ? n : 0) * p.wrs * 16;
+    if (VT) {
+      const int tk = n & 63;
+      vn[i] = tk >= (n >> 6) && tk <= p.vtP;
+      wrow[i] = n >= 64 ? p.vpos + (long)tk * p.wrs * 16
+                        : (tk == 0 ? p.vt0 + (long)blockIdx.y * p.bvt0 : p.w + (long)(tk > 0 ? tk - 1 : 0) * p.wrs * 16);
+    } else {
+      vn[i] = n < p.Cout;
+      wrow[i] = p.w + (long)(vn[i] ? n : 0) * p.wrs * 16;
+    }
   }
   const int nkt = (p.Kc + KCH - 1) / KCH;
   const char* zp = (const char*)g_zero_page;
@@ -408,7 +420,7 @@
   if (fast) {
 #pragma unroll
     for (int i = 0; i < 4; ++i) {
-      pb[i] = vn[i] ? p.w + wrow[i] + (long)kc * 16 : zp;
+      pb[i] = vn[i] ? wrow[i] + (long)kc * 16 : zp;
       incb[i] = vn[i] ? KCH * 16 : 0;
     }
     retap();
@@ -448,7 +460,7 @@
     }
 #pragma unroll
     for (int i = 0; i < 4; ++i) {
-      const char* src = (vk && vn[i]) ? p.w + wrow[i] + (long)kc * 16 : zp;
+      const char* src = (vk && vn[i]) ? wrow[i] + (long)kc * 16 : zp;
       glds16(src, &lds[buf][1][(8 * wvu + 32 * i) * KCH]);
     }
     kc += KCH;
@@ -556,6 +568,7 @@
           if (m >= p.M) continue;
           const f32x4* src = (const f32x4*)(ep + row * 64 + ((cg ^ (row & 7)) << 3));
           f32x4 v0 = src[0], v1 = src[1];
+          if (VT) { v0 += src[512]; v1 += src[513]; }
           float v[8] = {v0[0], v0[1], v0[2], v0[3], v1[0], v1[1], v1[2], v1[3]};
 #pragma unroll
           for (int j = 0; j < 8; ++j) v[j] = affine<T>(v[j], sc[j], bi[j]);
@@ -643,6 +656,10 @@
   const float* g0 = nullptr;
   const unsigned long long* mbits = nullptr;
   float* gpos = nullptr;
+  const char* vt0 = nullptr;
+  const char* vpos = nullptr;
+  long bvt0 = 0;
+  int vtP = 0;
   float* ws = nullptr;
 #ifdef CDDMSL_TILE_STAMPS
   unsigned long long* tstamps = nullptr;
@@ -983,7 +1000,7 @@
     }
 }
 
-template <typename T>
+template <typename T, bool VT = false>
 __global__ __launch_bounds__(256, 2) void k_gemm_tn_stream(WgradArgs p, int nbatch, int bpb) {
   constexpr int ES = Mma<T>::ES;
   constexpr int COLS = 256 / ES;
@@ -994,7 +1011,7 @@
   const int tile_k = blockIdx.x % ntk, tile_n = blockIdx.x / ntk;
   const int n0 = tile_n * COLS, k0 = tile_k * COLS;
   const int b0 = blockIdx.y * bpb, nb = min(bpb, nbatch - b0);
-  const int nmt = (p.M + WM - 1) / WM;
+  const int nmt = VT ? 2 : (p.M + WM - 1) / WM;
   const int nit = nb * nmt;
 
   const int cc = t & 15, rb = t >> 4;
@@ -1008,15 +1025,23 @@
     const char* xb = p.x + (long)(b0 + sb) * p.bx + (long)kc * 16;
 #pragma unroll
     for (int i = 0; i < 4; ++i) {
-      const int m = smt * WM + rb + 16 * i;
+      const int m = (VT ? 0 : smt * WM) + rb + 16 * i;
       const bool vm = m < p.M;
       glds16((vm && vn) ? db + ((long)m * p.ldd) * ES : zp, &lds[buf][0][(4 * wvu + 16 * i) * 16]);
     }
 #pragma unroll
     for (int i = 0; i < 4; ++i) {
-      const int m = smt * WM + rb + 16 * i;
-      const bool vm = m < p.M;
-      glds16((vm && vk) ? xb + ((long)m * p.xrs) * 16 : zp, &lds[buf][1][(4 * wvu + 16 * i) * 16]);
+      const int m = (VT ? 0 : smt * WM) + rb + 16 * i;
+      const char* src = zp;
+      if (VT) {
+        if (vk && m <= p.vtP) {
+          if (smt) src = m > 0 ? p.vpos + ((long)m * p.xrs + kc) * 16 : zp;
+          else src = m > 0 ? xb + ((long)(m - 1) * p.xrs) * 16 : p.vt0 + (long)(b0 + sb) * p.bvt0 + (long)kc * 16;
+        }
+      } else if (m < p.M && vk) {
+        src = xb + ((long)m * p.xrs) * 16;
+      }
+      glds16(src, &lds[buf][1][(4 * wvu + 16 * i) * 16]);
     }
     if (++smt == nmt) { smt = 0; ++sb; }
   };
@@ -1106,7 +1131,7 @@
     }
   return n;
 }
-template <int NG, int MODE, int P = 0>
+template <int NG, int MODE, int P = 0, bool VT = false>
 __global__ __launch_bounds__(256, 2) void k_gemm_tn_small(WgradArgs p, int nbatch, int bpb) {
   constexpr int NTN = (NG + 3) / 4, NSTORE = MODE == 3 ? tn_small_stores3<NG, P>() : 4 * NG, NML = MODE == 3 ? 2 : 0;
   constexpr int STAGE = 8192 + 16384, NST = 3;
@@ -1134,7 +1159,13 @@
 #pragma unroll
     for (int i = 0; i < 4; ++i) {
       const int m = xr + 16 * i;
-      glds16((vk && m < p.M) ? xb + ((long)m * p.xrs) * 16 : zp, base + 8192 + (i * 256 + wvu * 64) * 16);
+      const char* src = zp;
+      if (VT) {
+        if (vk && m <= p.vtP) src = m > 0 ? xb + ((long)(m - 1) * p.xrs) * 16 : p.vt0 + (long)(b0 + sb) * p.bvt0 + (long)kc * 16;
+      } else if (vk && m < p.M) {
+        src = xb + ((long)m * p.xrs) * 16;
+      }
+      glds16(src, base + 8192 + (i * 256 + wvu * 64) * 16);
     }
     ++sb;
   };
@@ -1163,6 +1194,27 @@
     for (int a = 0; a < NTN; ++a)
 #pragma unroll
       for (int g = 0; g < 16; ++g) gacc[a][g] = 0.f;
+  }
+  u32x4 fpos[4];
+  if (VT) {
+    char* base = lds + 2 * STAGE + 8192;
+#pragma unroll
+    for (int i = 0; i < 4; ++i) {
+      const int m = xr + 16 * i;
+      glds16((vk && m >= 1 && m <= p.vtP) ? p.vpos + ((long)m * p.xrs + kc) * 16 : zp, base + (i * 256 + wvu * 64) * 16);
+    }
+    wait_vm<0>();
+    __builtin_amdgcn_s_barrier();
+    const unsigned x0 = lbase + 2 * STAGE + xoff[0], x1 = lbase + 2 * STAGE + xoff[1];
+#define CDDMSL_TRP(DST, IMM)                                                                     \
+  { u32x2 q0_, q1_;                                                                              \
+    asm volatile("ds_read_b64_tr_b16 %0, %1 offset:%2" : "=v"(q0_) : "v"(x0), "i"(IMM));         \
+    asm volatile("ds_read_b64_tr_b16 %0, %1 offset:%2" : "=v"(q1_) : "v"(x1), "i"(IMM));         \
+    DST = u32x4{q0_[0], q0_[1], q1_[0], q1_[1]}; }
+    CDDMSL_TRP(fpos[0], 0) CDDMSL_TRP(fpos[1], 4096) CDDMSL_TRP(fpos[2], 8192) CDDMSL_TRP(fpos[3], 12288)
+#undef CDDMSL_TRP
+    asm volatile("s_waitcnt lgkmcnt(0)" : "+v"(fpos[0]), "+v"(fpos[1]), "+v"(fpos[2]), "+v"(fpos[3]) :: "memory");
+    __builtin_amdgcn_s_barrier();
   }
   if (nit > 0) stage(0);
   if (nit > 1) stage(1);
@@ -1211,6 +1263,12 @@
     for (int ms = 0; ms < 4; ++ms)
 #pragma unroll
       for (int a = 0; a < NTN; ++a) Mma<__bf16>::step(acc[a], fa[a][ms], fb[ms]);
+    if (VT) {
+#pragma unroll
+      for (int ms = 0; ms < 4; ++ms)
+#pragma unroll
+        for (int a = 0; a < NTN; ++a) Mma<__bf16>::step(acc[a], fa[a][ms], fpos[ms]);
+    }
     __builtin_amdgcn_s_barrier();
     char* outp = (char*)p.dw + (long)(b0 + it) * p.bo;
     const int k = k0 + wvu * 32 + r;
@@ -3090,6 +3148,76 @@
   return launch_status();
 }
 
+extern "C" int cddmsl_attnpool_nt_tok(const void* a, const void* t0, const void* x, const void* pos, void* c, int M, int TP, int P, int C,
+                                      int lda, int ldc, int batch, long sa, long sc, int out_f32, int dtype, void* stream) {
+  const int es = dtype == 0 ? 2 : 4;
+  if (dtype != 0 && dtype != 1) return CDDMSL_ERR_ARG;
+  if (M < 0 || batch < 0 || batch > 65535 || P <= 0 || P >= TP || TP > 64 || (TP & 7) || C <= 0 || (C * es) % 128 || (ldc & 7) || ldc < TP) return CDDMSL_ERR_ARG;
+  if ((lda * es) % 16 || (sa * es) % 16 || !t0 || !x || !pos) return CDDMSL_ERR_ARG;
+  if (M == 0 || batch == 0) return CDDMSL_OK;
+  ConvArgs p;
+  p.x = (const char*)a; p.w = (const char*)x; p.y = (char*)c; p.scale = nullptr; p.bias = nullptr; p.residual = nullptr; p.relu_mask = nullptr;
+  p.Nimg = 1; p.Hi = 1; p.Wi = M; p.Cin = C; p.Ho = 1; p.Wo = M; p.Cout = TP; p.KH = 1; p.KW = 1; p.stride = 1; p.pad = 0;
+  p.ldy = ldc; p.ldr = 0; p.ldm = 0; p.relu = 0; p.out_f32 = out_f32; p.pool = 0; p.res_f32 = 0; p.res_pool = 0;
+  p.M = M; p.cpp = C * es / 16; p.Kc = p.cpp;
+  p.dWo = make_fastdiv((unsigned)M); p.dHo = make_fastdiv(1u); p.dcpp = make_fastdiv((unsigned)p.cpp); p.dKW = make_fastdiv(1u);
+  p.xrs = lda * es / 16; p.wrs = p.cpp;
+  p.bx = sa * es; p.bw = (long)P * C * es; p.by = sc * (out_f32 ? 4 : es);
+  p.vt0 = (const char*)t0; p.bvt0 = (long)C * es; p.vpos = (const char*)pos; p.vtP = P;
+  const long ntm = (M + BM - 1) / BM;
+  g_last_kernel = 1;
+  if (g_plan_only) return CDDMSL_OK;
+  if (dtype == 0) hipLaunchKernelGGL((k_conv_fwd<__bf16, true>), dim3((unsigned)ntm, (unsigned)batch), dim3(256), 0, (hipStream_t)stream, p);
+  else hipLaunchKernelGGL((k_conv_fwd<float, true>), dim3((unsigned)ntm, (unsigned)batch), dim3(256), 0, (hipStream_t)stream, p);
+  return launch_status();
+}
+
+extern "C" int cddmsl_attnpool_tn_tok(const void* a, const void* t0, const void* x, const void* pos, void* out, int TP, int N, int P, int C,
+                                      int lda, int ldo, int batch, long sa, long so, int mode, int dtype, void* stream) {
+  const int es = dtype == 0 ? 2 : 4;
+  if (dtype != 0 && dtype != 1) return CDDMSL_ERR_ARG;
+  if (N <= 0 || C <= 0 || batch <= 0 || batch > 65535 || mode < 0 || mode > 2 || P <= 0 || P >= TP || TP > WM) return CDDMSL_ERR_ARG;
+  if ((C * es) % 16 || (N * es) % 16 || (lda * es) % 16 || (sa * es) % 16 || !t0 || !x || !pos) return CDDMSL_ERR_ARG;
+  WgradArgs p;
+  p.x = (const char*)x; p.dy = (const char*)a; p.dw = (float*)out; p.scale = nullptr;
+  p.Nimg = 1; p.Hi = 1; p.Wi = TP; p.Cin = C; p.Ho = 1; p.Wo = TP; p.Cout = N; p.KH = 1; p.KW = 1; p.stride = 1; p.pad = 0;
+  p.ldd = lda; p.pool = 0; p.M = TP; p.cpp = C * es / 16; p.Kc = p.cpp; p.K = C; p.ncc = N * es / 16;
+  p.dWo = make_fastdiv((unsigned)TP); p.dHo = make_fastdiv(1u);
+  p.xrs = C * es / 16; p.ldo = ldo; p.direct = mode;
+  p.bx = (long)P * C * es; p.bd = sa * es; p.bo = so * (mode == 2 ? es : 4);
+  p.vt0 = (const char*)t0; p.bvt0 = (long)C * es; p.vpos = (const char*)pos; p.vtP = P;
+  if (dtype == 0 && N <= 64 && N % 8 == 0 && C % 128 == 0 && batch >= 64) {
+    const long kt = C / 128;
+    long bpb = (kt * batch + 4095) / 4096;
+    if (bpb < 8) bpb = 8;
+    if (bpb > batch) bpb = batch;
+    const unsigned gy = (unsigned)((batch + bpb - 1) / bpb);
+    g_last_kernel = 9;
+    if (g_plan_only) return CDDMSL_OK;
+#define CDDMSL_TNV(NG)                                                                                                                    \
+  case NG:                                                                                                                                \
+    if (mode == 0) hipLaunchKernelGGL((k_gemm_tn_small<NG, 0, 0, true>), dim3((unsigned)kt, gy), dim3(256), 0, (hipStream_t)stream, p, batch, (int)bpb);      \
+    else if (mode == 1) hipLaunchKernelGGL((k_gemm_tn_small<NG, 1, 0, true>), dim3((unsigned)kt, gy), dim3(256), 0, (hipStream_t)stream, p, batch, (int)bpb); \
+    else hipLaunchKernelGGL((k_gemm_tn_small<NG, 2, 0, true>), dim3((unsigned)kt, gy), dim3(256), 0, (hipStream_t)stream, p, batch, (int)bpb);                \
+    break;
+    switch (N / 8) { CDDMSL_TNV(1) CDDMSL_TNV(2) CDDMSL_TNV(3) CDDMSL_TNV(4) CDDMSL_TNV(5) CDDMSL_TNV(6) CDDMSL_TNV(7) CDDMSL_TNV(8) }
+#undef CDDMSL_TNV
+    return launch_status();
+  }
+  const int cols = 256 / es;
+  const long tiles = (long)((N + cols - 1) / cols) * ((C + cols - 1) / cols);
+  long bpb = (tiles * batch + 4095) / 4096;
+  if (bpb < 4) bpb = 4;
+  if (bpb > batch) bpb = batch;
+  const long gy = (batch + bpb - 1) / bpb;
+  if (tiles > 0x7fffffffL) return CDDMSL_ERR_ARG;
+  g_last_kernel = 7;
+  if (g_plan_only) return CDDMSL_OK;
+  if (dtype == 0) hipLaunchKernelGGL((k_gemm_tn_stream<__bf16, true>), dim3((unsigned)tiles, (unsigned)gy), dim3(256), 0, (hipStream_t)stream, p, batch, (int)bpb);
+  else hipLaunchKernelGGL((k_gemm_tn_stream<float, true>), dim3((unsigned)tiles, (unsigned)gy), dim3(256), 0, (hipStream_t)stream, p, batch, (int)bpb);
+  return launch_status();
+}
+
 extern "C" int cddmsl_attnpool_dx(const void* pds, const void* zu, const float* g0, const unsigned long long* mbits, void* dx, float* gpos,
                                   int K, int H2, int P, int TP, int C, int dtype, void* stream) {
   if (dtype != 0 || K < 0 || P != 49 || TP != 56 || H2 <= 0 || H2 > 64 || (H2 & 7) || C <= 0 || (C & 127) || !g0 || !mbits || !dx) return CDDMSL_ERR_ARG;
diff --git a/cddmsl_amd/hip.py b/cddmsl_amd/hip.py
--- a/cddmsl_amd/hip.py
+++ b/cddmsl_amd/hip.py
@@ -40,6 +40,9 @@
         L.cddmsl_attnpool_softmax_bwd.argtypes = [vp] * 4 + [c_long, ci, ci, ci, cf, ci, vp]
         L.cddmsl_gemm_nt_batched.argtypes = [vp] * 4 + [ci] * 7 + [c_long] * 3 + [ci, ci, vp]
         L.cddmsl_gemm_tn_batched.argtypes = [vp] * 3 + [ci] * 7 + [c_long] * 3 + [ci, ci, vp]
+        L.cddmsl_attn_token0.argtypes = [vp] * 5 + [ci] * 4 + [vp]
+        L.cddmsl_attnpool_nt_tok.argtypes = [vp] * 5 + [ci] * 7 + [c_long] * 2 + [ci, ci, vp]
+        L.cddmsl_attnpool_tn_tok.argtypes = [vp] * 5 + [ci] * 7 + [c_long] * 2 + [ci, ci, vp]
         L.cddmsl_relu_bwd.argtypes = [vp, vp, vp, c_long, ci, ci, vp]
         L.cddmsl_colsum.argtypes = [vp, vp, c_long, ci, ci, ci, vp]
         L.cddmsl_sgd_clip_step.argtypes = [vp] * 4 + [ci, vp] + [cf] * 4 + [ci, vp]
@@ -497,6 +500,51 @@
     return tok, mbits
 
 
+@_timed("attn_token0")
+def attn_token0(x, pos, want_mask=False):
+    require_cuda(x, pos)
+    K, P, C = x.shape
+    assert pos.dtype == torch.float32 and tuple(pos.shape) == (P + 1, C) and x.is_contiguous() and pos.is_contiguous()
+    assert not want_mask or P <= 64
+    t0 = torch.empty((K, C), device=x.device, dtype=x.dtype)
+    posT = torch.empty((P + 1, C), device=x.device, dtype=x.dtype)
+    mbits = torch.empty((K, C), device=x.device, dtype=torch.int64) if want_mask else None
+    check(_L().cddmsl_attn_token0(ptr(x), ptr(pos), ptr(t0), ptr(posT), ptr(mbits), K, P, C, _dt(x), stream_ptr()), "cddmsl_attn_token0")
+    return t0, posT, mbits
+
+
+def _tok_operands(t0, x, posT, TP):
+    K, P, C = x.shape
+    assert t0.dtype == x.dtype == posT.dtype and t0.is_contiguous() and x.is_contiguous() and posT.is_contiguous()
+    assert tuple(t0.shape) == (K, C) and tuple(posT.shape) == (P + 1, C) and P < TP
+    return K, P, C
+
+
+@_timed("attnpool_nt_tok")
+def attnpool_nt_tok(a, t0, x, posT, c, M, TP, lda, sa, sc, a_off=0, c_off=0):
+    require_cuda(a, t0, x, posT, c)
+    K, P, C = _tok_operands(t0, x, posT, TP)
+    assert a.dtype == x.dtype and c.dtype in (a.dtype, torch.float32)
+    out_f32 = int(c.dtype == torch.float32 and a.dtype != torch.float32)
+    check(_L().cddmsl_attnpool_nt_tok(_eptr(a, a_off), ptr(t0), ptr(x), ptr(posT), _eptr(c, c_off), M, TP, P, C, lda, TP, K, sa, sc,
+                                      out_f32, _dt(a), stream_ptr()), "cddmsl_attnpool_nt_tok")
+
+
+@_timed("attnpool_tn_tok")
+def attnpool_tn_tok(a, t0, x, posT, out, N, TP, lda, ldo, sa, so, accumulate=False):
+    require_cuda(a, t0, x, posT, out)
+    K, P, C = _tok_operands(t0, x, posT, TP)
+    assert a.dtype == x.dtype
+    if accumulate:
+        assert out.dtype == torch.float32
+        mode = 0
+    else:
+        assert out.dtype in (a.dtype, torch.float32)
+        mode = 1 if out.dtype == torch.float32 else 2
+    check(_L().cddmsl_attnpool_tn_tok(ptr(a), ptr(t0), ptr(x), ptr(posT), ptr(out), TP, N, P, C, lda, ldo, K, sa, so, mode, _dt(a),
+                                      stream_ptr()), "cddmsl_attnpool_tn_tok")
+
+
 def rpn_losses(logits, deltas, pos, neg, midx, gt, gt_off, anchors, weights, inv_norm, gout=None):
     require_cuda(logits, deltas, pos, neg, midx, gt, gt_off, anchors)
     for t in (logits, deltas, gt, anchors):
diff --git a/cddmsl_amd/layers.py b/cddmsl_amd/layers.py
--- a/cddmsl_amd/layers.py
+++ b/cddmsl_amd/layers.py
@@ -755,41 +755,77 @@
         dev = x.device
         fused_dx = hip.attnpool_dx_ok(K, H, P, TP, C, T) and bool(ctx.needs_input_grad[0]) and os.environ.get("CDDMSL_ATTNPOOL_DX", "1") != "0"
         mbits = None
-        if fused_dx and premask_input_grad:
-            tok, mbits = hip.attn_tokens_fwd_mask(x.view(K, P, C), ap.pos.detach(), TP)
+        xv = x.view(K, P, C)
+        want_mask = fused_dx and premask_input_grad
+        if AttnPoolFn.token_free():
+            t0, posT, mbits = hip.attn_token0(xv, ap.pos.detach(), want_mask)
+            toks = (t0, xv, posT)
+        elif want_mask:
+            tok, mbits = hip.attn_tokens_fwd_mask(xv, ap.pos.detach(), TP)
+            toks = (tok,)
         else:
-            tok = hip.attn_tokens_fwd(x.view(K, P, C), ap.pos.detach(), TP)
+            toks = (hip.attn_tokens_fwd(xv, ap.pos.detach(), TP),)
         wq, _ = ap.pq.get(T, False)
         wk, wkT = ap.pk.get(T, True)
         wv, wvT = ap.pv.get(T, True)
         wc, _ = ap.pc.get(T, False)
-        q0 = hip.conv_fwd(tok.view(K, 1, TP, C), wq, None, ap.q_b.detach(), stride=TP).view(K, C)
+        q0 = hip.conv_fwd(AttnPoolFn._tok0(toks, K, C), wq, None, ap.q_b.detach(), stride=AttnPoolFn._tok0_stride(toks)).view(K, C)
         zu = torch.empty((K, 2 * H, C), device=dev, dtype=T)
         hip.gemm_nt_batched(q0, wkT, zu, K, C, D, C, C, 2 * H * C, H, D, D, C, c_off=H * C)
         S = torch.empty((K, H, TP), device=dev, dtype=torch.float32)
-        hip.gemm_nt_batched(zu, tok, S, H, TP, C, C, C, TP, K, 2 * H * C, TP * C, H * TP, a_off=H * C)
+        AttnPoolFn._nt(zu, toks, S, H, K, C, H * C)
         p, pT = hip.attnpool_softmax_fwd(S, P + 1, D ** -0.5, T)
         z = torch.empty((K, H, C), device=dev, dtype=T)
-        hip.gemm_tn_batched(pT, tok, z, TP, H, C, H, C, C, K, TP * H, TP * C, H * C)
+        AttnPoolFn._tn(pT, toks, z, H, K, C)
         o = torch.empty((K, C), device=dev, dtype=T)
         hip.gemm_nt_batched(z, wv, o, K, D, C, H * C, C, C, H, C, D * C, D)
         o = o + ap.v_b.detach().to(T)
         out = hip.conv_fwd(o.view(1, 1, K, C), wc, None, ap.c_b.detach(), out_f32=True).view(K, -1)
         ctx.ap = ap
         ctx.fused_dx = fused_dx
-        ctx.save_for_backward(tok, q0, zu, p, z, o, mbits)
+        ctx.ntok = len(toks)
+        ctx.save_for_backward(*toks, q0, zu, p, z, o, mbits)
         ctx.shape = (K, h, w, C)
         return out
 
     @staticmethod
+    def token_free():
+        return os.environ.get("CDDMSL_ATTNPOOL_TOKENS", "0") == "0"
+
+    @staticmethod
+    def _tok0(toks, K, C):
+        return toks[0].view(K, 1, 1, C) if len(toks) == 3 else toks[0].view(K, 1, AttnPoolFn.TP, C)
+
+    @staticmethod
+    def _tok0_stride(toks):
+        return 1 if len(toks) == 3 else AttnPoolFn.TP
+
+    @staticmethod
+    def _nt(zu, toks, out, H, K, C, a_off):
+        TP = AttnPoolFn.TP
+        if len(toks) == 3:
+            hip.attnpool_nt_tok(zu, *toks, out, H, TP, C, 2 * H * C, H * TP, a_off=a_off)
+        else:
+            hip.gemm_nt_batched(zu, toks[0], out, H, TP, C, C, C, TP, K, 2 * H * C, TP * C, H * TP, a_off=a_off)
+
+    @staticmethod
+    def _tn(aT, toks, out, H, K, C):
+        TP = AttnPoolFn.TP
+        if len(toks) == 3:
+            hip.attnpool_tn_tok(aT, *toks, out, H, TP, H, C, TP * H, H * C)
+        else:
+            hip.gemm_tn_batched(aT, toks[0], out, TP, H, C, H, C, C, K, TP * H, TP * C, H * C)
+
+    @staticmethod
     def backward(ctx, dout):
         ap = ctx.ap
-        tok, q0, zu, p, z, o, mbits = ctx.saved_tensors
+        saved = ctx.saved_tensors
+        toks, (q0, zu, p, z, o, mbits) = saved[:ctx.ntok], saved[ctx.ntok:]
         K, h, w, C = ctx.shape
         P, TP, H = h * w, AttnPoolFn.TP, ap.heads
         D = C // H
-        T = tok.dtype
-        dev = tok.device
+        T = q0.dtype
+        dev = q0.device
         train = not ap.frozen
         dout_t = dout.contiguous().to(T)
         if train:
@@ -804,16 +840,17 @@
             hip.gemm_tn_batched(do, z, _grad_buf(ap.v_w), K, D, C, C, H * C, C, H, D, C, D * C, accumulate=True)
         hip.gemm_nt_batched(do, wvT, zu, K, C, D, C, C, 2 * H * C, H, D, D, C)
         dP = torch.empty((K, H, TP), device=dev, dtype=torch.float32)
-        hip.gemm_nt_batched(zu, tok, dP, H, TP, C, C, C, TP, K, 2 * H * C, TP * C, H * TP)
+        AttnPoolFn._nt(zu, toks, dP, H, K, C, 0)
         dsT, pds = hip.attnpool_softmax_bwd(p, dP, D ** -0.5, T)
         du = torch.empty((K, H, C), device=dev, dtype=T)
-        hip.gemm_tn_batched(dsT, tok, du, TP, H, C, H, C, C, K, TP * H, TP * C, H * C)
+        AttnPoolFn._tn(dsT, toks, du, H, K, C)
         dq0 = torch.empty((K, C), device=dev, dtype=T)
         hip.gemm_nt_batched(du, wk, dq0, K, D, C, H * C, C, C, H, C, D * C, D)
         if train:
             hip.gemm_tn_batched(q0, du, _grad_buf(ap.k_w), K, D, C, C, H * C, C, H, D, C, D * C, accumulate=True)
             _grad_buf(ap.k_b)
-            hip.conv_wgrad(tok.view(K, 1, TP, C), dq0.view(K, 1, 1, C), _ohwi(ap.q_w).shape, stride=TP, out=_ohwi(_grad_buf(ap.q_w)))
+            hip.conv_wgrad(AttnPoolFn._tok0(toks, K, C), dq0.view(K, 1, 1, C), _ohwi(ap.q_w).shape, stride=AttnPoolFn._tok0_stride(toks),
+                           out=_ohwi(_grad_buf(ap.q_w)))
             hip.colsum(dq0, out=_grad_buf(ap.q_b))
         _, wqd = ap.pq.get(T, True)
         gpos = _grad_buf(ap.pos) if train else None
diff --git a/include/cddmsl_hip.h b/include/cddmsl_hip.h
--- a/include/cddmsl_hip.h
+++ b/include/cddmsl_hip.h
@@ -76,6 +76,12 @@
 int cddmsl_attn_tokens_fwd(const void* x, const float* pos, void* tok, int K, int P, int TP, int C, int dtype, void* stream);
 int cddmsl_attn_tokens_fwd_mask(const void* x, const float* pos, void* tok, unsigned long long* mbits, int K, int P, int TP, int C,
                                 int dtype, void* stream);
+int cddmsl_attn_token0(const void* x, const float* pos, void* t0, void* posT, unsigned long long* mbits, int K, int P, int C, int dtype,
+                       void* stream);
+int cddmsl_attnpool_nt_tok(const void* a, const void* t0, const void* x, const void* pos, void* c, int M, int TP, int P, int C, int lda,
+                           int ldc, int batch, long sa, long sc, int out_f32, int dtype, void* stream);
+int cddmsl_attnpool_tn_tok(const void* a, const void* t0, const void* x, const void* pos, void* out, int TP, int N, int P, int C, int lda,
+                           int ldo, int batch, long sa, long so, int mode, int dtype, void* stream);
 int cddmsl_attnpool_dx(const void* pds, const void* zu, const float* g0, const unsigned long long* mbits, void* dx, float* gpos, int K,
                        int H2, int P, int TP, int C, int dtype, void* stream);
 int cddmsl_attn_tokens_bwd(const void* dtok, const void* relu_mask, void* dx, float* gpos, int K, int P, int TP, int C, int dtype,
```

New measurement: 159.7 (median of 6 runs). No clear change (+0.7%).
